# ayutaz/F5-TTS

Hardware: AMD Instinct MI355X
Metric: mel-frames/s (RTF alongside), F5TTS_v1_Base NFE=16 CFM.sample (higher is better)
Workload: dtype bf16; 1 GPU; C2: F5TTS_v1_Base CFM.sample, NFE 16 EPSS + sway -1, CFG 2.0, 1 utterance per GPU, 938 prompt + 938 generated frames (1876), 300 tokens; batch_per_gpu=1, frames=1876, gen_frames_per_gpu=938, nfe=16, parallelism=dp1

## Files before the change

### f5-tts_amd/csrc/elementwise.hip

```cpp
#include "common.h"
#include "kernels.h"
#include "lnrow.h"

#include <algorithm>

namespace f5h {

static inline unsigned nblk(int64_t n, int t) { return (unsigned)((n + t - 1) / t); }

struct TVals {
  float t[513];
};
__global__ void time_sinus_kernel(TVals tv, int n, float* out) {
  int i = blockIdx.x * blockDim.x + threadIdx.x;
  if (i >= n * 128) return;
  int r = i / 128, j = i % 128;
  const float k = logf(10000.f) / 127.f;
  float f = expf((float)j * -k);
  float e = (1000.f * tv.t[r]) * f;
  out[r * 256 + j] = sinf(e);
  out[r * 256 + 128 + j] = cosf(e);
}
hipError_t time_sinus(const float* t_host, int n, float* out, hipStream_t st) {
  if (n <= 0 || n > 512) return hipErrorInvalidValue;
  TVals tv{};
  for (int i = 0; i < n; ++i) tv.t[i] = t_host[i];
  hipLaunchKernelGGL(time_sinus_kernel, dim3(nblk(n * 128, 256)), dim3(256), 0, st, tv, n, out);
  return hipGetLastError();
}

__global__ void time_sinus_dev_kernel(const float* tg, int n, float* out) {
  int i = blockIdx.x * blockDim.x + threadIdx.x;
  if (i >= n * 128) return;
  int r = i / 128, j = i % 128;
  const float k = logf(10000.f) / 127.f;
  float f = expf((float)j * -k);
  float e = (1000.f * tg[r]) * f;
  out[r * 256 + j] = sinf(e);
  out[r * 256 + 128 + j] = cosf(e);
}
hipError_t time_sinus_dev(const float* tg, int n, float* out, hipStream_t st) {
  if (n <= 0 || n > 512) return hipErrorInvalidValue;
  hipLaunchKernelGGL(time_sinus_dev_kernel, dim3(nblk(n * 128, 256)), dim3(256), 0, st, tg, n, out);
  return hipGetLastError();
}

__global__ void grid_upload_kernel(TVals tv, int n, float* out) {
  int i = blockIdx.x * blockDim.x + threadIdx.x;
  if (i < n) out[i] = tv.t[i];
}
__global__ void ptr_upload_kernel(float* p, float** slot) {
  if (threadIdx.x == 0) slot[0] = p;
}
hipError_t ptr_upload(float* p, float** slot, hipStream_t st) {
  hipLaunchKernelGGL(ptr_upload_kernel, dim3(1), dim3(64), 0, st, p, slot);
  return hipGetLastError();
}
hipError_t grid_upload(const float* t_host, int n, float* out, hipStream_t st) {
  if (n <= 0 || n > 513) return hipErrorInvalidValue;
  TVals tv{};
  for (int i = 0; i < n; ++i) tv.t[i] = t_host[i];
  hipLaunchKernelGGL(grid_upload_kernel, dim3(nblk(n, 256)), dim3(256), 0, st, tv, n, out);
  return hipGetLastError();
}
struct IVals {
  int32_t v[512];
};
__global__ void seg_upload_kernel(IVals iv, int n, int32_t* out) {
  const int i = blockIdx.x * blockDim.x + threadIdx.x;
  if (i < n) out[i] = iv.v[i];
}
hipError_t seg_upload(const int32_t* host, int64_t n, int32_t* out, hipStream_t st) {
  if (n <= 0 || !host || !out) return hipErrorInvalidValue;
  for (int64_t o = 0; o < n; o += 512) {
    const int m = (int)(n - o < 512 ? n - o : 512);
    IVals iv{};
    for (int i = 0; i < m; ++i) iv.v[i] = host[o + i];
    hipLaunchKernelGGL(seg_upload_kernel, dim3(nblk(m, 256)), dim3(256), 0, st, iv, m, out + o);
  }
  return hipGetLastError();
}

__global__ void step_begin_kernel(const int* kstep, const float* src, int64_t stride, int n, float* dst) {
  const int k = *kstep;
  const int i = blockIdx.x * blockDim.x + threadIdx.x;
// ... 53 lines not shown
    const float xv[8] = {p0.x, p0.y, p0.z, p0.w, p1.x, p1.y, p1.z, p1.w};
#pragma unroll
    for (int e = 0; e < 8; ++e) {
      const float x = one + xv[e];
      hi[e] = from_f32<T>(x);
      lo[e] = from_f32<T>(x - to_f32(hi[e]));
    }
  };
  for (int k0 = 0; k0 < d; k0 += 64) {
    float4 xs[2][2], xh[2][2];
    v8 b[2][4];
#pragma unroll
    for (int u = 0; u < 2; ++u) {
      const int k = k0 + 32 * u;
      xs[u][0] = *reinterpret_cast<const float4*>(ar + sc_off + k);
      xs[u][1] = *reinterpret_cast<const float4*>(ar + sc_off + k + 4);
      xh[u][0] = *reinterpret_cast<const float4*>(ar + sh_off + k);
      xh[u][1] = *reinterpret_cast<const float4*>(ar + sh_off + k + 4);
#pragma unroll
      for (int t = 0; t < 4; ++t) b[u][t] = *reinterpret_cast<const v8*>(wr + (int64_t)t * 16 * d + k);
    }
#pragma unroll
    for (int u = 0; u < 2; ++u) {
      v8 shi, slo, hhi, hlo;
      parts(xs[u][0], xs[u][1], 1.f, shi, slo);
      parts(xh[u][0], xh[u][1], 0.f, hhi, hlo);
#pragma unroll
      for (int t = 0; t < 4; ++t) {
        acc[0][t] = Op16<T>::mma16(shi, b[u][t], acc[0][t]);
        acc[1][t] = Op16<T>::mma16(hhi, b[u][t], acc[1][t]);
        acc[0][t] = Op16<T>::mma16(slo, b[u][t], acc[0][t]);
        acc[1][t] = Op16<T>::mma16(hlo, b[u][t], acc[1][t]);
      }
    }
  }
  const int64_t LW = 2 * (int64_t)F + 6 * (int64_t)d;
  const int64_t u_off = a.out_off + l * LW + (ff ? 0 : 2 * (int64_t)F), v_off = u_off + (ff ? F : 3 * d);
#pragma unroll
  for (int t = 0; t < 4; ++t)
#pragma unroll
    for (int r = 0; r < 4; ++r) {
      const int s = g * 16 + 4 * (lane >> 4) + r;
      if (s < a.nfe) {
        float* o = a.table + (int64_t)s * a.stride + n0 + 16 * t + (lane & 15);
        o[u_off] = acc[0][t][r];
        o[v_off] = acc[1][t][r];
      }
    }
}
hipError_t lnfold_uv(int compute, const LnFoldArgs& a, hipStream_t st) {
  if (a.d % 64 || a.F % 64 || a.nfe <= 0 || a.depth <= 0) return hipErrorInvalidValue;
  const dim3 grid((a.depth * (a.F / 64 + 3 * a.d / 64) * ((a.nfe + 15) / 16) + 3) / 4), block(256);
  if (compute == F5H_C_BF16)
    hipLaunchKernelGGL(lnfold_uv_kernel<bf16>, grid, block, 0, st, a);
  else if (compute == F5H_C_FP16)
    hipLaunchKernelGGL(lnfold_uv_kernel<f16>, grid, block, 0, st, a);
  else
    return hipErrorInvalidValue;
  return hipGetLastError();
}

__global__ void zero_words_kernel(uint4* p, int64_t n4) {
  for (int64_t i = (int64_t)blockIdx.x * blockDim.x + threadIdx.x; i < n4; i += (int64_t)gridDim.x * blockDim.x)
    p[i] = uint4{0u, 0u, 0u, 0u};
}
hipError_t zero_words(unsigned* p, int64_t n, hipStream_t st) {
  if (n % 4 || ((uintptr_t)p & 15)) return hipErrorInvalidValue;
  const int64_t n4 = n / 4;
  hipLaunchKernelGGL(zero_words_kernel, dim3((unsigned)std::min<int64_t>(64, nblk(n4, 256))), dim3(256), 0, st,
                     reinterpret_cast<uint4*>(p), n4);
  return hipGetLastError();
}

template <typename TO>
__global__ void silu_kernel(const float* x, TO* y, int64_t n) {
  int64_t i = (int64_t)blockIdx.x * blockDim.x + threadIdx.x;
  if (i < n) y[i] = from_f32<TO>(silu(x[i]));
}
hipError_t silu_to_op(int compute, const float* x, void* y, int64_t n, hipStream_t st) {
  F5H_OP_DISPATCH(compute, T, hipLaunchKernelGGL(silu_kernel<T>, dim3(nblk(n, 256)), dim3(256), 0, st, x, (T*)y, n););
  return hipGetLastError();
}

constexpr int MAXV = 8;

template <typename TO, int NV, typename TI = float>
__global__ __launch_bounds__(256) void ln_mod_kernel(const TI* h, int M, int d, const float* shift,
                                                     const float* scale, TO* out) {
  constexpr bool FIXED = NV > 0;
  constexpr int V = FIXED ? NV : MAXV;
  const int row = blockIdx.x * 4 + (threadIdx.x >> 6), lane = threadIdx.x & 63;
  if (row >= M) return;
  const TI* x = h + (int64_t)row * d;
  const float4* sh = reinterpret_cast<const float4*>(shift);
  const float4* sc = reinterpret_cast<const float4*>(scale);
  const int n4 = FIXED ? 64 * NV : d >> 2;
  float4 v[V], a[V], b[V];
#pragma unroll
  for (int k = 0; k < V; ++k) {
    const int i = lane + 64 * k;
    const bool ok = FIXED || i < n4;
    v[k] = ok ? load4f<TI>(x + 4 * i) : make_float4(0, 0, 0, 0);
    a[k] = ok ? sc[i] : make_float4(0, 0, 0, 0);
    b[k] = ok ? sh[i] : make_float4(0, 0, 0, 0);
  }
  ln_mod_row<TO, V, FIXED>(v, a, b, lane, n4, d, out + (int64_t)row * d);
}
template <typename T>
__global__ __launch_bounds__(256) void ln_mod16_kernel(const T* h, int M, const float* shift, const float* scale,
                                                       T* out) {
  constexpr int d = 1024;
  const int row = blockIdx.x * 4 + (threadIdx.x >> 6), lane = threadIdx.x & 63;
  if (row >= M) return;
  const uint4* x = reinterpret_cast<const uint4*>(h + (int64_t)row * d);
  const float4* sh = reinterpret_cast<const float4*>(shift);
  const float4* sc = reinterpret_cast<const float4*>(scale);
  uint4 xv[2], o[2];
  float4 a[2][2], b[2][2];
#pragma unroll
  for (int k = 0; k < 2; ++k) {
    const int c = lane + 64 * k;
    xv[k] = x[c];
    a[k][0] = sc[2 * c];
    a[k][1] = sc[2 * c + 1];
    b[k][0] = sh[2 * c];
    b[k][1] = sh[2 * c + 1];
  }
  ln16_row<T>(xv, a, b, o);
  uint4* op = reinterpret_cast<uint4*>(out + (int64_t)row * d);
#pragma unroll
  for (int k = 0; k < 2; ++k) op[lane + 64 * k] = o[k];
}

hipError_t ln_modulate(int compute, const void* hv, int h16, int M, int d, const float* shift, const float* scale,
                       void* out, hipStream_t st) {
  if (d % 4 || d > 4 * 64 * MAXV) return hipErrorInvalidValue;
  const dim3 g(nblk(M, 4)), b(256);
  if (h16) {
    if (compute != F5H_C_BF16 && compute != F5H_C_FP16) return hipErrorInvalidValue;
    auto run = [&](auto tag) {
      typedef decltype(tag) T;
      const T* x = (const T*)hv;
      switch (d) {
        case 1024: hipLaunchKernelGGL((ln_mod16_kernel<T>), g, b, 0, st, x, M, shift, scale, (T*)out); break;
        case 768: hipLaunchKernelGGL((ln_mod_kernel<T, 3, T>), g, b, 0, st, x, M, d, shift, scale, (T*)out); break;
        case 512: hipLaunchKernelGGL((ln_mod_kernel<T, 2, T>), g, b, 0, st, x, M, d, shift, scale, (T*)out); break;
        default: hipLaunchKernelGGL((ln_mod_kernel<T, 0, T>), g, b, 0, st, x, M, d, shift, scale, (T*)out);
      }
    };
    if (compute == F5H_C_BF16)
      run(bf16{});
    else
      run(f16{});
    return hipGetLastError();
  }
  const float* h = (const float*)hv;
  switch (d) {
    case 1024: F5H_OP_DISPATCH(compute, T, hipLaunchKernelGGL((ln_mod_kernel<T, 4>), g, b, 0, st, h, M, d, shift, scale, (T*)out);); break;
    case 768: F5H_OP_DISPATCH(compute, T, hipLaunchKernelGGL((ln_mod_kernel<T, 3>), g, b, 0, st, h, M, d, shift, scale, (T*)out);); break;
    case 512: F5H_OP_DISPATCH(compute, T, hipLaunchKernelGGL((ln_mod_kernel<T, 2>), g, b, 0, st, h, M, d, shift, scale, (T*)out);); break;
    default: F5H_OP_DISPATCH(compute, T, hipLaunchKernelGGL((ln_mod_kernel<T, 0>), g, b, 0, st, h, M, d, shift, scale, (T*)out););
  }
  return hipGetLastError();
}

template <typename TO, int NV, typename TI = float>
__global__ __launch_bounds__(256) void rms_kernel(const TI* h, int M, int d, const float* g, TO* out) {
  constexpr bool FIXED = NV > 0;
  constexpr int V = FIXED ? NV : MAXV;
  const int row = blockIdx.x * 4 + (threadIdx.x >> 6), lane = threadIdx.x & 63;
  if (row >= M) return;
  const TI* x = h + (int64_t)row * d;
  const float4* gg = reinterpret_cast<const float4*>(g);
  const int n4 = FIXED ? 64 * NV : d >> 2;
  float4 v[V], a[V];
  float q = 0.f;
#pragma unroll
  for (int k = 0; k < V; ++k) {
    const int i = lane + 64 * k;
    const bool ok = FIXED || i < n4;
    v[k] = ok ? load4f<TI>(x + 4 * i) : make_float4(0, 0, 0, 0);
    a[k] = ok ? gg[i] : make_float4(0, 0, 0, 0);
  }
#pragma unroll
  for (int k = 0; k < V; ++k) q += v[k].x * v[k].x + v[k].y * v[k].y + v[k].z * v[k].z + v[k].w * v[k].w;
  const float nrm = fmaxf(sqrtf(wave_sum_dpp(q)), 1e-12f);
  const float f = sqrtf((float)d);
#pragma unroll
  for (int k = 0; k < V; ++k) {
// ... 340 lines not shown
  }
  partial[((int64_t)z * S + s) * C + c] = acc;
}
template <typename TO>
__global__ void grn_apply_ragged_kernel(const float* x, const int* off, int S, int C, const float* nx,
                                        const float* gamma, const float* beta, TO* out, int64_t total) {
  int64_t i = (int64_t)blockIdx.x * blockDim.x + threadIdx.x;
  if (i >= total) return;
  int c = (int)(i % C);
  int s = seg_find(off, S, (int)(i / C));
  float v = x[i];
  out[i] = from_f32<TO>(gamma[c] * (v * nx[(int64_t)s * C + c]) + beta[c] + v);
}
hipError_t grn_ragged(int compute, const float* x, const int32_t* off, int S, int R, int Lmax, int C,
                      const float* gamma, const float* beta, float* scratch, void* out, hipStream_t st) {
  if (S <= 0 || R <= 0 || Lmax <= 0 || C <= 0 || !off) return hipErrorInvalidValue;
  const int nz = (int)nblk(Lmax, 64);
  float* nx = scratch + (size_t)nz * S * C;
  hipLaunchKernelGGL(grn_sumsq_ragged_kernel, dim3(nblk(C, 256), S, nz), dim3(256), 0, st, x, off, S, C, scratch);
  hipLaunchKernelGGL(grn_norm_kernel, dim3(S), dim3(1024), 0, st, scratch, nz, S, C, nx);
  const int64_t total = (int64_t)R * C;
  F5H_OP_DISPATCH(compute, T, hipLaunchKernelGGL(grn_apply_ragged_kernel<T>, dim3(nblk(total, 256)), dim3(256), 0, st, x, off, S, C, nx, gamma, beta, (T*)out, total););
  return hipGetLastError();
}
__global__ void rowtab_kernel(const int* off, int S, int R, int2* rowtab, int32_t* len) {
  const int m = blockIdx.x * blockDim.x + threadIdx.x;
  if (m < S && len) len[m] = off[m + 1] - off[m];
  if (m >= R) return;
  const int s = seg_find(off, S, m);
  rowtab[m] = make_int2(s, m - off[s]);
}
hipError_t build_rowtab(const int32_t* off, int S, int R, int2* rowtab, int32_t* len, hipStream_t st) {
  if (S <= 0 || R < S || !off || !rowtab) return hipErrorInvalidValue;
  hipLaunchKernelGGL(rowtab_kernel, dim3(nblk(R, 256)), dim3(256), 0, st, off, S, R, rowtab, len);
  return hipGetLastError();
}

template <typename TO>
__global__ void build_ct_kernel(const float* cond, const uint8_t* cmask, const float* tc, const float* tu, int B,
                                int N, int td, int tdp, int S, int drop_audio, int drop_text, TO* out) {
  const int64_t K = 128 + tdp;
  int64_t i = (int64_t)blockIdx.x * blockDim.x + threadIdx.x;
  if (i >= (int64_t)S * N * K) return;
  const int64_t row = i / K;
  const int col = (int)(i - row * K);
  const int s = (int)(row / N), n = (int)(row - (int64_t)s * N);
  const int b = s % B;
  float v = 0.f;
  if (col < 128) {
    if (col < 100 && s < B && !drop_audio && cmask[(int64_t)b * N + n]) v = cond[((int64_t)b * N + n) * 100 + col];
  } else if (col - 128 < td) {
    const float* t = (s < B && !drop_text) ? tc : tu;
    v = t[((int64_t)b * N + n) * td + (col - 128)];
  }
  out[i] = from_f32<TO>(v);
}
hipError_t build_ct(int compute, const float* cond, const uint8_t* cond_mask, const float* text_c,
                    const float* text_u, int B, int N, int td, int S, int drop_audio, int drop_text, void* out,
                    hipStream_t st) {
  const int tdp = (td + 63) / 64 * 64;
  const int64_t total = (int64_t)S * N * (128 + tdp);
  F5H_OP_DISPATCH(compute, T, hipLaunchKernelGGL(build_ct_kernel<T>, dim3(nblk(total, 256)), dim3(256), 0, st, cond, cond_mask, text_c, text_u, B, N, td, tdp, S, drop_audio, drop_text, (T*)out););
  return hipGetLastError();
}

template <typename TO>
__global__ void pack_y_kernel(const float* y, int rows, int mel, TO* yp) {
  int64_t i = (int64_t)blockIdx.x * blockDim.x + threadIdx.x;
  if (i >= (int64_t)rows * 128) return;
  int64_t r = i >> 7;
  int c = (int)(i & 127);
  yp[i] = from_f32<TO>(c < mel ? y[r * mel + c] : 0.f);
}
hipError_t pack_y(int compute, const float* y, int rows, int mel, void* ypad, hipStream_t st) {
  const int64_t total = (int64_t)rows * 128;
  F5H_OP_DISPATCH(compute, T, hipLaunchKernelGGL(pack_y_kernel<T>, dim3(nblk(total, 256)), dim3(256), 0, st, y, rows, mel, (T*)ypad););
  return hipGetLastError();
}

template <typename TO>
__global__ __launch_bounds__(256) void cfg_euler_kernel(EulerArgs a, TO* ypad) {
  int64_t i = (int64_t)blockIdx.x * blockDim.x + threadIdx.x;
  const int64_t total = (int64_t)a.B * a.N * a.mel;
  const int k = a.kstep ? __hip_atomic_load(a.kstep, __ATOMIC_RELAXED, __HIP_MEMORY_SCOPE_AGENT) : 0;
  if (a.kstep && a.next_dst) {
    if (k + 1 < a.nfe) {
      const float4* src = reinterpret_cast<const float4*>(a.next_src + (int64_t)(k + 1) * a.next_stride);
      float4* dst = reinterpret_cast<float4*>(a.next_dst);
      for (int64_t j = i; j < a.next_n / 4; j += (int64_t)gridDim.x * blockDim.x) dst[j] = src[j];
    }
  }
  float dt = a.dt;
  float* traj = a.traj;
  if (a.kstep) {
    dt = sub_nc(a.tgrid[k + 1], a.tgrid[k]);
    traj = a.trajp ? *a.trajp : nullptr;
    if (traj) traj += (int64_t)(k + 1) * total;
  }
  for (; i < total; i += (int64_t)gridDim.x * blockDim.x) {
    const int c = (int)(i % a.mel);
    const int64_t bn = i / a.mel;
    const int b = (int)(bn / a.N), n = (int)(bn - (int64_t)b * a.N);
    const float pc = a.p[(int64_t)b * a.p_seq_stride + (int64_t)(a.p_row_off + n) * a.p_ld + c];
    float v = pc;
    if (a.use_cfg) {
      const float pu = a.p[(int64_t)(a.B + b) * a.p_seq_stride + (int64_t)(a.p_row_off + n) * a.p_ld + c];
      v = add_nc(pc, mul_nc(sub_nc(pc, pu), a.cfg));
    }
    const float y = add_nc(a.y[i], mul_nc(dt, v));
    a.y[i] = y;
    if (ypad) ypad[bn * 128 + c] = from_f32<TO>(y);
    if (traj) traj[i] = y;
  }
  if (a.kstep && a.arrive) {
    __syncthreads();
    if (threadIdx.x == 0) {
      const unsigned old = __hip_atomic_fetch_add(a.arrive, 1u, __ATOMIC_RELAXED, __HIP_MEMORY_SCOPE_AGENT);
      if (old == gridDim.x - 1) {
        __hip_atomic_store(a.arrive, 0u, __ATOMIC_RELAXED, __HIP_MEMORY_SCOPE_AGENT);
        __hip_atomic_store(const_cast<int*>(a.kstep), k + 1, __ATOMIC_RELAXED, __HIP_MEMORY_SCOPE_AGENT);
        if (a.tick) __hip_atomic_fetch_add(a.tick, 1, __ATOMIC_RELAXED, __HIP_MEMORY_SCOPE_AGENT);
      }
    }
  }
}
hipError_t cfg_euler(const EulerArgs& a, hipStream_t st) {
  const int64_t total = (int64_t)a.B * a.N * a.mel;
  const unsigned blocks = std::min<unsigned>(128, std::max<unsigned>(1, nblk(total, 256)));
  F5H_OP_DISPATCH(a.compute, T, hipLaunchKernelGGL(cfg_euler_kernel<T>, dim3(blocks), dim3(256), 0, st, a, (T*)a.ypad););
  return hipGetLastError();
}

template <typename TO, int METHOD>
__global__ __launch_bounds__(256) void cfg_rk_kernel(RkArgs a, TO* ypad) {
  constexpr OdeTableau T = ode_tableau(METHOD);
  constexpr int STAGES = T.stages;
  static_assert(METHOD == 1 || METHOD == 2, "midpoint or rk4");
  static_assert(METHOD != 1 || (T.a[4] == T.c[1] && T.b[0] == 0.f && T.b[1] == 1.f), "midpoint tableau");
  static_assert(METHOD != 2 || (T.a[4] == T.c[1] && T.a[8] == -T.c[1] && T.a[9] == 1.f && T.a[12] == 1.f &&
                                T.a[13] == -1.f && T.a[14] == 1.f && T.b[1] == 3.f * T.b[0] &&
                                T.b[2] == T.b[1] && T.b[3] == T.b[0]),
                "3/8-rule tableau");
  int64_t i = (int64_t)blockIdx.x * blockDim.x + threadIdx.x;
  const int64_t total = (int64_t)a.B * a.N * a.mel;
  const int e = __hip_atomic_load(a.keval, __ATOMIC_RELAXED, __HIP_MEMORY_SCOPE_AGENT);
  const int k = e / STAGES, s = e - k * STAGES;
  if (a.next_dst && e + 1 < a.neval) {
    const float4* src = reinterpret_cast<const float4*>(a.next_src + (int64_t)(e + 1) * a.next_stride);
    float4* dst = reinterpret_cast<float4*>(a.next_dst);
    for (int64_t j = i; j < a.next_n / 4; j += (int64_t)gridDim.x * blockDim.x) dst[j] = src[j];
  }
  const float dt = sub_nc(a.sgrid[k + 1], a.sgrid[k]);
  const bool last = s == STAGES - 1;
  float* traj = (last && a.trajp) ? *a.trajp : nullptr;
  if (traj) traj += (int64_t)(k + 1) * total;
  for (; i < total; i += (int64_t)gridDim.x * blockDim.x) {
    const int c = (int)(i % a.mel);
    const int64_t bn = i / a.mel;
    const int b = (int)(bn / a.N), n = (int)(bn - (int64_t)b * a.N);
    const float pc = a.p[(int64_t)b * a.p_seq_stride + (int64_t)(a.p_row_off + n) * a.p_ld + c];
    float v = pc;
    if (a.use_cfg) {
      const float pu = a.p[(int64_t)(a.B + b) * a.p_seq_stride + (int64_t)(a.p_row_off + n) * a.p_ld + c];
      v = add_nc(pc, mul_nc(sub_nc(pc, pu), a.cfg));
    }
    const float y0 = a.y[i];
    float yn;
    if constexpr (METHOD == 1) {
      yn = s == 0 ? add_nc(y0, mul_nc(v, mul_nc(T.c[1], dt))) : add_nc(y0, mul_nc(dt, v));
    } else {
      constexpr float c3 = T.c[1];
      const float* K0 = a.kbuf;
      const float* K1 = K0 + total;
      const float* K2 = K1 + total;
      if (s == 0) {
        yn = add_nc(y0, mul_nc(mul_nc(dt, v), c3));
      } else if (s == 1) {
        yn = add_nc(y0, mul_nc(dt, sub_nc(v, mul_nc(K0[i], c3))));
      } else if (s == 2) {
        yn = add_nc(y0, mul_nc(dt, add_nc(sub_nc(K0[i], K1[i]), v)));
      } else {
        const float sum = add_nc(add_nc(K0[i], mul_nc(T.b[1] / T.b[0], add_nc(K1[i], K2[i]))), v);
        yn = add_nc(y0, mul_nc(mul_nc(sum, dt), T.b[0]));
      }
      if (!last) a.kbuf[(int64_t)s * total + i] = v;
    }
    if (last) a.y[i] = yn;
    ypad[bn * 128 + c] = from_f32<TO>(yn);
    if (traj) traj[i] = yn;
  }
  if (a.arrive) {
    __syncthreads();
    if (threadIdx.x == 0) {
      const unsigned old = __hip_atomic_fetch_add(a.arrive, 1u, __ATOMIC_RELAXED, __HIP_MEMORY_SCOPE_AGENT);
      if (old == gridDim.x - 1) {
        __hip_atomic_store(a.arrive, 0u, __ATOMIC_RELAXED, __HIP_MEMORY_SCOPE_AGENT);
        __hip_atomic_store(a.keval, e + 1, __ATOMIC_RELAXED, __HIP_MEMORY_SCOPE_AGENT);
        if (a.tick) __hip_atomic_fetch_add(a.tick, 1, __ATOMIC_RELAXED, __HIP_MEMORY_SCOPE_AGENT);
      }
    }
  }
}
hipError_t cfg_rk(const RkArgs& a, hipStream_t st) {
  if ((a.method != 1 && a.method != 2) || !a.keval || !a.sgrid || !a.ypad) return hipErrorInvalidValue;
  if (ode_kept_slopes(a.method) > 0 && !a.kbuf) return hipErrorInvalidValue;
  const int64_t total = (int64_t)a.B * a.N * a.mel;
  const unsigned blocks = std::min<unsigned>(128, std::max<unsigned>(1, nblk(total, 256)));
// ... 176 lines not shown
```

### f5-tts_amd/csrc/engine.cpp

```cpp
#include "engine_internal.h"

static bool adaln_bb(const f5h_arch& a) { return a.backbone != F5H_UNETT; }
static size_t mm_ada_x(const f5h_arch& a, int l) { return (size_t)l * 12 * a.dim; }
static size_t mm_ada_c(const f5h_arch& a, int l) { return mm_ada_x(a, l) + (size_t)6 * a.dim; }
static size_t mm_ada_fin(const f5h_arch& a) { return mm_ada_c(a, a.depth - 1) + (size_t)2 * a.dim; }

static void layout(const f5h_engine* e, WS& ws, Bufs& b, int B, int N, int nfe, int use_cfg, int method = 0,
                   int steps = 0, int nt = 0, int rgB = 0, int rgL = 0) {
  const f5h_arch& a = e->a;
  const int d = a.dim, td = a.text_dim, S = use_cfg ? 2 * B : B;
  const bool mm = a.backbone == F5H_MMDIT;
  const int L = adaln_bb(a) ? N : N + 1;
  const size_t rows = (size_t)S * L, es = e->esz;
  const size_t jrows = mm ? (size_t)S * (N + nt) : rows;
  const int inner = a.heads * 64;
  b.tsin = ws.take<float>((size_t)nfe * 256);
  b.th = ws.take<float>((size_t)nfe * d);
  b.temb = ws.take<float>((size_t)nfe * d);
  b.tin_op = ws.take<char>((size_t)nfe * std::max(256, d) * es);
  b.ada = adaln_bb(a) ? ws.take<float>((size_t)nfe * e->ada_row) : nullptr;
  b.te = ws.take<float>((size_t)2 * B * (mm ? nt : N) * td);
  b.keepfill = ws.take<uint8_t>((size_t)2 * B * N);
  if (a.conv_layers > 0) {
    b.dwln = ws.take<char>((size_t)2 * B * N * td * es);
// ... 169 lines not shown
    TextEmbArgs t{};
    t.text = text;
    t.B = c.B;
    t.nt = c.nt;
    t.N = c.nt;
    t.td = d;
    t.table = e->text_table;
    t.freqs = e->freqs;
    t.freq_rows = kMMTextPos;
    t.mask_padding = a.text_mask_padding;
    t.out_c = b.te;
    t.out_u = b.te + (size_t)c.B * c.nt * d;
    KCK(text_embed(t, st));
    if (bf) KCK(f32_to_op(bf, b.te, (int64_t)2 * c.B * c.nt * d, b.c0, st));
  } else if (!text_cached) {
    TextEmbArgs t{};
    t.text = text;
    t.B = c.rag_B ? c.rag_B : c.B;
    t.nt = c.nt;
    t.N = c.N;
    t.td = td;
    t.seg_off = b.rg_off;
    t.seq_len = (a.backbone == F5H_DIT && c.batch_mask) ? duration : nullptr;
    t.table = e->text_table;
    t.freqs = a.conv_layers > 0 ? e->freqs : nullptr;
    t.mask_padding = a.text_mask_padding;
    t.out_c = b.te;
    t.out_u = b.te + (size_t)c.B * c.N * td;
    t.keep = b.keepfill;
    KCK(text_embed(t, st));
    const int S2 = 2 * c.B, R2 = S2 * c.N;
    const int32_t* tl = c.isolate ? duration : nullptr;
    for (int i = 0; i < a.conv_layers; ++i) {
      CNX& x = e->cnx[i];
      if (c.rag_B)
        KCK(dwconv_ln_ragged(bf, b.te, b.rg_off, 2 * c.rag_B, R2, td, x.dw_w, x.dw_b, x.ln_w, x.ln_b, b.dwln, st));
      else
        KCK(dwconv_ln(bf, b.te, S2, c.N, td, x.dw_w, x.dw_b, x.ln_w, x.ln_b, b.dwln, st, tl, c.B));
      GemmArgs g = gargs(b.dwln, td, x.pw1, R2, b.pw1o, 2 * td);
      KCK(gemm(bf, EPI_GELU_ERF, g, st));
      if (c.rag_B)
        KCK(grn_ragged(bf, b.pw1o, b.rg_off, 2 * c.rag_B, R2, c.rag_L, 2 * td, x.gamma, x.beta, b.grn_scr, b.grno, st));
      else
        KCK(grn(bf, b.pw1o, S2, c.N, 2 * td, x.gamma, x.beta, b.grn_scr, b.grno, st, tl, c.B));
      g = gargs(b.grno, 2 * td, x.pw2, R2, b.te, td);
      g.rowkeep = a.text_mask_padding ? b.keepfill : nullptr;
      KCK(gemm(bf, EPI_RESID_FILL, g, st));
    }
    if (a.text_average_upsampling) {
      TextUpArgs u{};
      u.text = text;
      u.B = c.B;
      u.nt = c.nt;
      u.N = c.N;
      u.td = td;
      u.seq_len = t.seq_len;
      u.in_c = t.out_c;
      u.in_u = t.out_u;
      u.out_c = b.te_up;
      u.out_u = b.te_up + (size_t)c.B * c.N * td;
      KCK(text_upsample(u, st));
    }
  }
  if (c.isolate && b.rowkeep_n) KCK(build_rowkeep(duration, c.B, c.S, c.N, 0, b.rowkeep_n, st));
  const float* te = a.text_average_upsampling ? b.te_up : b.te;
  KCK(build_ct(bf, cond, cond_mask, te, te + (size_t)c.B * c.N * td, c.B, c.N, mm ? 0 : td, c.S, c.drop_audio,
               c.drop_text, b.act, st));
  GemmArgs g = gargs(b.act, 128 + e->tdp, e->in_ct, c.S * c.N, b.P, d);
  KCK(gemm(bf, EPI_STORE, g, st));
  return 0;
}

constexpr int kArrive = 16;

static int step_prep(Ctx& c) {
  f5h_engine* e = c.e;
  if (adaln_bb(e->a))
    KCK(step_begin(c.b.kstep, c.b.ada, e->ada_row, e->ada_row, c.b.ada_cur, c.st));
  else
    KCK(step_begin(c.b.kstep, c.b.temb, e->a.dim, e->a.dim, c.b.temb_cur, c.st));
  return 0;
}

static int backbone_part(Ctx& c, int s0, int ns, hipStream_t st) {
  f5h_engine* e = c.e;
  const f5h_arch& a = e->a;
  const int d = a.dim, bf = e->bf, H = a.heads, inner = H * 64;
  const bool dit = a.backbone == F5H_DIT;
  const size_t es = e->esz;
  Bufs& b = c.b;
  const int BN = c.B * c.N;
  const int rows = ns * c.L;
  const size_t ro = (size_t)s0 * c.L;
  const size_t no = (size_t)s0 * c.N;
  auto op = [&](void* base, size_t row, size_t width) -> void* { return (char*)base + row * width * es; };
  const uint8_t* keep = c.batch_mask ? b.rowkeep + ro : nullptr;
  static const bool res32 = [] {
    const char* v = getenv("F5H_RES32");
    return v && *v == '1';
  }();
  const bool r16 = bf != 0 && (!dit || !res32);
  static const bool skip_ln = [] {
    const char* v = getenv("F5H_DIAG_SKIP_LN");
    const bool on = v && *v == '1';
    if (on) std::fprintf(stderr, "[f5h] F5H_DIAG_SKIP_LN=1: LayerNorm launches skipped, results are WRONG (timing only)\n");
    return on;
  }();
  const bool do_ln = !(skip_ln && r16);
  const size_t hsz = r16 ? es : sizeof(float);
  auto res = [&](void* base) -> void* { return (char*)base + ro * d * hsz; };
  void* bh = dit ? res(b.h) : res(b.xs[0]);
  void* aop = op(b.aop, ro, d);
  void* q = op(b.q, ro, inner);
  void* k = op(b.k, ro, inner);
  void* v = op(b.v, ro, inner);
  void* o = op(b.o, ro, inner);
  void* f = op(b.f, ro, a.ff_dim);
  {
    GemmArgs g = gargs(b.ypad, 128, e->in_x, BN, b.h0 + no * d, d);
    g.bias = nullptr;
    g.add = b.P + no * d;
    g.ld_add = d;
    g.dual_rows = ns == 2 * c.B ? BN : 0;
    KCK(gemm(bf, EPI_INPROJ, g, st));
    ConvArgs cv{};
    cv.S = ns;
    cv.L = c.N;
    cv.d = d;
    cv.rowkeep = dit ? keep : (c.isolate ? b.rowkeep_n + no : nullptr);
    cv.x = b.h0 + no * d;
    cv.x_f32 = 1;
    cv.w = e->conv_w[0];
    cv.bias = e->conv_b[0];
    cv.mode = 0;
    cv.y = op(b.c1, no, d);
    if (c.rag_B) {
      cv.ragged = 1;
      cv.S = ns * c.rag_B;
      cv.L = c.rag_L;
      cv.rowkeep = reinterpret_cast<const uint8_t*>(b.rg_off);
    }
    {
      ProbeScope ps(e, KC_CONV, st, &c.site);
      KCK(conv_pos(bf, cv, st));
    }
    cv.x = op(b.c1, no, d);
    cv.x_f32 = bf ? 0 : 1;
    cv.w = e->conv_w[1];
    cv.bias = e->conv_b[1];
    cv.mode = r16 ? 2 : 1;
    cv.y = bh;
    cv.y_seq_stride = c.L;
    cv.y_row_off = dit ? 0 : 1;
    cv.resid = b.h0 + no * d;
    KCK(conv_pos(bf, cv, st));
  }
  if (!dit) KCK(write_time_token(bf, r16, b.temb_cur, ns, c.L, d, bh, st));
  void* hkeep = a.long_skip_connection ? (char*)b.hkeep + ro * d * hsz : nullptr;
  if (hkeep) {
    if (bf != 0 && !r16)
      return fail(F5H_EINVAL, "long_skip_connection: F5H_RES32 (fp32 residual under 16-bit operands) is not supported");
    KCK(hipMemcpyAsync(hkeep, bh, (size_t)rows * d * hsz, hipMemcpyDeviceToDevice, st));
  }

  const float* ada_k = dit ? b.ada_cur : nullptr;
  const int epi_resid = r16 ? EPI_RESID16 : EPI_RESID;
  void* h = bh;
  const void* h_in = nullptr;
  auto qkv_args = [&](const Layer& Lq) {
    GemmArgs g = gargs(aop, d, Lq.qkv, rows, nullptr, 0);
    g.rope = b.rope;
    g.seq_len = c.L;
    g.heads = H;
    g.rope_heads = a.pe_attn_head > 0 ? a.pe_attn_head : H;
    g.q = q;
    g.k = k;
    g.v = v;
    g.q_scale = 0.125f * 1.4426950408889634f;
    g.q_norm_w = Lq.q_norm_w;
    g.k_norm_w = Lq.k_norm_w;
    g.qk_norm_eps = 1e-6f;
    if (c.rag_B) {
      g.add = reinterpret_cast<const float*>(b.rg_tab);
      g.seq_len = c.rag_L;
      g.qkv_dst_len = c.rag_L;
    }
    return g;
  };
  const bool chain_on = c.chain && dit && r16 && do_ln && !keep && d == 1024 && b.chain && s0 == 0 && ns == c.S &&
                        (e->probe_class < 0 || e->probe_class == KC_ATTN || e->probe_class == KC_CONV ||
                         e->probe_class == KC_CHAIN);
  static const bool zero_memset = [] {
    const char* v = getenv("F5H_CHAIN_ZERO");
    return v && !strcmp(v, "memset");
  }();
  if (chain_on) {
    if (zero_memset)
      KCK(hipMemsetAsync(b.chain, 0, (size_t)a.depth * 5 * b.chain_g4 * sizeof(unsigned), st));
    else
      KCK(zero_words(b.chain, (int64_t)a.depth * 5 * b.chain_g4, st));
  }
  bool qkv_done = false;
  bool final_done = false;
  const bool fold_on = c.lnfold && dit && r16 && do_ln && !keep && !chain_on && b.lnp && e->lnf_ok;
  const bool rms_on = c.lnfold && !dit && r16 && b.lnp && e->rmsf_ok;
  const int64_t lnf_lw = 2 * (int64_t)a.ff_dim + 6 * (int64_t)d;
  auto lnf = [&](int l) { return ada_k + e->ada.Npad + (int64_t)l * lnf_lw; };
// ... 76 lines not shown
        at.kv_len = at.q_len = b.rg_len;
        at.o_split = kAttnRagged;
        at.o2 = b.rg_off;
      }
      at.store_wt = attention_store_wt(bf, at, store_want(c.store, KC_ATTN));
      count_store(e, at.store_wt);
      ProbeScope ps(e, KC_ATTN, st, &c.site, &at.probe);
      KCK(attention(bf, at, st));
    }
    if (chain_on) {
      ChainArgs ca{};
      ca.out = gargs(o, inner, Ly.out, rows, h, d);
      ca.out.gate = ad + 2 * d;
      ca.ln1 = LnArgs{h, aop, ad + 3 * d , ad + 4 * d };
      ca.ff1 = gargs(aop, d, Ly.ff1, rows, f, a.ff_dim);
      ca.ff2 = gargs(f, a.ff_dim, Ly.ff2, rows, h, d);
      ca.ff2.gate = ad + 5 * d;
      if (l + 1 < a.depth) {
        const float* an = ada_k + (size_t)(l + 1) * 6 * d;
        ca.ln2 = LnArgs{h, aop, an , an + d };
        ca.qkv = qkv_args(e->layers[l + 1]);
      } else {
        const float* fin = ada_k + (size_t)a.depth * 6 * d;
        ca.ln2 = LnArgs{h, aop, fin + d, fin};
      }
      ca.cnt = b.chain + (size_t)l * 5 * b.chain_g4;
      ca.groups = (rows + kChainRows - 1) / kChainRows;
      ca.fault = e->chain_fault;
      ProbeScope ps(e, KC_CHAIN, st, &c.site, &ca.probe);
      const hipError_t ce = chain_launch(bf, ca, st);
      if (ce == hipSuccess) {
        e->n_chain.fetch_add(1, std::memory_order_relaxed);
        qkv_done = l + 1 < a.depth;
        final_done = l + 1 == a.depth;
        continue;
      }
      if (ce != hipErrorInvalidValue) KCK(ce);
    }
    {
      GemmArgs g = gargs(o, inner, Ly.out, rows, h, d);
      g.resid = h_in;
      g.gate = ad ? ad + 2 * d : nullptr;
      g.rowkeep = keep;
      if (keep && !h_in && e->pad_skip && !rms_on) {
        g.live_len = b.kvlen + s0;
        g.live_seq = c.L;
      }
      if (fold_on) fold_producer(g, ad + 4 * d );
      if (rms_on) rms_producer(g);
      gemm_policy(c, g, epi_resid, KC_OUT);
      ProbeScope ps(e, KC_OUT, st, &c.site, &g.probe);
      KCK(gemm(bf, epi_resid, g, st));
    }
    if (!fold_on && !rms_on) {
      ProbeScope ps(e, KC_NORM, st, &c.site);
      if (dit) {
        if (do_ln) KCK(ln_modulate(bf, h, r16, rows, d, ad + 3 * d , ad + 4 * d , aop, st));
      }
      else
        KCK(rms_norm_g(bf, h, r16, rows, d, Ly.g_ff, aop, st));
    }
    {
      GemmArgs g = gargs(aop, d, Ly.ff1, rows, f, a.ff_dim);
      if (fold_on) fold_consumer(g, lnf(l), lnf(l) + a.ff_dim);
      if (rms_on) {
        g.A = h;
        g.W = Ly.ff1_g.w;
        rms_consumer(g);
      }
      gemm_policy(c, g, EPI_GELU_TANH, KC_FFN1);
      ProbeScope ps(e, KC_FFN1, st, &c.site, &g.probe);
      KCK(gemm(bf, EPI_GELU_TANH, g, st));
    }
    {
      GemmArgs g = gargs(f, a.ff_dim, Ly.ff2, rows, h, d);
      g.gate = ad ? ad + 5 * d : nullptr;
      if (fold_on && l + 1 < a.depth) fold_producer(g, ada_k + (size_t)(l + 1) * 6 * d + d);
      if (rms_on && l + 1 < a.depth / 2) rms_producer(g);
      gemm_policy(c, g, epi_resid, KC_FFN2);
      ProbeScope ps(e, KC_FFN2, st, &c.site, &g.probe);
      KCK(gemm(bf, epi_resid, g, st));
    }
  }
  if (dit) {
    const float* fin = ada_k + (size_t)a.depth * 6 * d;
    if (hkeep) {
      void* hl = (char*)b.c1 + no * d * hsz;
      GemmArgs g = gargs(h, d, e->long_skip, rows, hl, d);
      g.A2 = hkeep;
      g.k_split = d;
      KCK(gemm(bf, r16 ? EPI_STORE16 : EPI_STORE, g, st));
      h = hl;
    }
    if (!final_done) KCK(ln_modulate(bf, h, r16, rows, d, fin + d, fin, aop, st));
  } else {
    KCK(rms_norm_g(bf, h, r16, rows, d, e->norm_out_g, aop, st));
  }
  const int pld = e->proj_out.Npad;
  GemmArgs g = gargs(aop, d, e->proj_out, rows, b.p + ro * pld, pld);
  g.N = pld;
  KCK(gemm(bf, EPI_STORE, g, st));
  return 0;
}

static int backbone_mmdit(Ctx& c, hipStream_t st) {
  f5h_engine* e = c.e;
  const f5h_arch& a = e->a;
  const int d = a.dim, bf = e->bf, H = a.heads, inner = H * 64, F = a.ff_dim;
  const size_t es = e->esz;
  Bufs& b = c.b;
  const int BN = c.B * c.N, rows = c.S * c.N, crows = c.S * c.nt, Lj = c.N + c.nt;
  const bool r16 = bf != 0;
  const int epi_resid = r16 ? EPI_RESID16 : EPI_RESID;
  const uint8_t* keep = c.batch_mask ? b.rowkeep : nullptr;
  {
    GemmArgs g = gargs(b.ypad, 128, e->in_x, BN, b.h0, d);
    g.bias = nullptr;
    g.add = b.P;
    g.ld_add = d;
    g.dual_rows = c.S == 2 * c.B ? BN : 0;
    KCK(gemm(bf, EPI_INPROJ, g, st));
    ConvArgs cv{};
    cv.S = c.S;
    cv.L = c.N;
    cv.d = d;
    cv.x = b.h0;
    cv.x_f32 = 1;
    cv.w = e->conv_w[0];
    cv.bias = e->conv_b[0];
    cv.mode = 0;
    cv.y = b.c1;
    cv.rowkeep = c.isolate ? keep : nullptr;
    {
      ProbeScope ps(e, KC_CONV, st, &c.site);
      KCK(conv_pos(bf, cv, st));
    }
    cv.x = b.c1;
    cv.x_f32 = bf ? 0 : 1;
    cv.w = e->conv_w[1];
    cv.bias = e->conv_b[1];
    cv.mode = r16 ? 2 : 1;
    cv.y = b.h;
    cv.y_seq_stride = c.N;
    cv.y_row_off = 0;
    cv.resid = b.h0;
    KCK(conv_pos(bf, cv, st));
  }
  const char* te0 = r16 ? (const char*)b.c0 : (const char*)b.te;
  const size_t hsz = r16 ? es : sizeof(float);
  const void* c0 = te0 + ((c.S == c.B && c.drop_text) ? (size_t)c.B * c.nt * d * hsz : 0);
  const float* ada_k = b.ada_cur;
  auto qkv = [&](const void* A, const Lin& W, int M, int seq, size_t row0, const float* qn, const float* kn) -> int {
    GemmArgs g = gargs(A, d, W, M, nullptr, 0);
    g.rope = b.rope;
    g.seq_len = seq;
    g.qkv_dst_len = Lj;
    g.heads = H;
    g.rope_heads = H;
    g.q = (char*)b.q + row0 * 64 * es;
    g.k = (char*)b.k + row0 * 64 * es;
    g.v = (char*)b.v + row0 * 64 * es;
    g.q_scale = 0.125f * 1.4426950408889634f;
    g.q_norm_w = qn;
    g.k_norm_w = kn;
    g.qk_norm_eps = 1e-6f;
    gemm_policy(c, g, EPI_QKV, KC_QKV);
// ... 84 lines not shown
  KCK(hipEventRecord(e->ev_fork, c.st));
  KCK(hipStreamWaitEvent(c.st2, e->ev_fork, 0));
  RC(backbone_part(c, 0, c.B, c.st));
  RC(backbone_part(c, c.B, c.B, c.st2));
  KCK(hipEventRecord(e->ev_join, c.st2));
  KCK(hipStreamWaitEvent(c.st, e->ev_join, 0));
  return 0;
}

static float round_to(int compute, float x) {
  if (compute == F5H_FP16) return (float)(_Float16)x;
  if (compute != F5H_BF16 || x != x) return x;
  uint32_t u;
  std::memcpy(&u, &x, 4);
  u = (u + 0x7fffu + ((u >> 16) & 1u)) & 0xffff0000u;
  std::memcpy(&x, &u, 4);
  return x;
}
void ode_eval_times(int method, int compute, const float* t, int steps, float* out) {
#pragma clang fp contract(off)
  const OdeTableau T = ode_tableau(method);
  for (int i = 0; i <= steps; ++i)
    if (round_to(compute, t[i]) != t[i]) compute = F5H_FP32;
  for (int k = 0; k < steps; ++k) {
    const float t0 = t[k], t1 = t[k + 1];
    const float dt = round_to(compute, t1 - t0);
    for (int s = 0; s < T.stages; ++s) {
      float v = t0;
      if (s > 0) v = T.c[s] == 1.f ? t1 : round_to(compute, t0 + round_to(compute, dt * T.c[s]));
      out[k * T.stages + s] = v;
    }
  }
}

extern "C" {

size_t f5h_workspace_size_ode(const f5h_engine* e, int32_t B, int32_t N, int32_t nt, int32_t steps, int32_t use_cfg,
                             int32_t method) {
  if (!e || B <= 0 || N <= 0 || steps <= 0 || method < 0 || method >= kOdeMethods) return 0;
  if (e->a.backbone == F5H_MMDIT && nt < 0) return 0;
  WS ws;
  Bufs b;
  layout(e, ws, b, B, N, steps * ode_tableau(method).stages + 1, use_cfg, method, steps,
         e->a.backbone == F5H_MMDIT ? nt : 0);
  return ws.off;
}
size_t f5h_workspace_size(const f5h_engine* e, int32_t B, int32_t N, int32_t nt, int32_t nfe, int32_t use_cfg) {
  return f5h_workspace_size_ode(e, B, N, nt, nfe, use_cfg, F5H_EULER);
}

static int check_ws(Ctx& c, void* w, size_t bytes) {
  WS ws;
  layout(c.e, ws, c.b, c.B, c.N, c.nfe + 1, c.use_cfg, c.method, c.steps, c.nt, c.rag_B, c.rag_L);
  if (bytes < ws.off)
    return fail(F5H_ENOMEM, "workspace too small: need " + std::to_string(ws.off) + " have " + std::to_string(bytes));
  ws.off = 0;
  ws.base = reinterpret_cast<char*>(w);
  layout(c.e, ws, c.b, c.B, c.N, c.nfe + 1, c.use_cfg, c.method, c.steps, c.nt, c.rag_B, c.rag_L);
  return 0;
}
static int check_mmdit_call(const f5h_engine* e, int nt, int batch_mask, int isolate) {
  if (e->a.backbone != F5H_MMDIT) return 0;
  if (nt <= 0) return fail(F5H_EINVAL, "MMDiT needs nt >= 1 text tokens");
  if (e->a.attn_mask_enabled && batch_mask && !isolate)
    return fail(F5H_EINVAL,
                "MMDiT: attn_mask_enabled with a batch mask is not supported: the valid keys [0, dur) and [N, N + "
                "text length) are not a prefix of the joint sequence, and the reference's masked mode is not wired to "
                "the two-range attention (use_batch_mask 2 masks both ranges and isolates the batch)");
  return 0;
}

static GraphKey graph_key(const Ctx& c, const void* ws, int kind) {
  GraphKey key{};
  key.ws = ws;
  key.kind = kind;
  key.B = c.B;
  key.N = c.N;
  key.nt = c.nt;
  key.nfe = c.nfe;
  key.use_cfg = c.use_cfg;
  key.batch_mask = c.batch_mask + c.isolate;
  key.lnfold = c.lnfold;
  key.store = c.store;
  key.method = c.method;
  key.rag_B = c.rag_B;
  key.rag_L = c.rag_L;
  key.kernel_epoch = g_kernel_epoch.load();
  return key;
}

static int prologue_graph(Ctx& c, const f5h_sample_args* a, const GraphKey& key) {
  f5h_engine* e = c.e;
  const size_t bn = (size_t)c.B * c.N;
  HIPCK(hipMemcpyAsync(c.b.in_cond, a->cond, bn * e->a.mel_dim * sizeof(float), hipMemcpyDeviceToDevice, c.st));
  HIPCK(hipMemcpyAsync(c.b.in_mask, a->cond_mask, bn, hipMemcpyDeviceToDevice, c.st));
  if (c.nt > 0)
    HIPCK(hipMemcpyAsync(c.b.in_text, a->text, (size_t)c.B * c.nt * sizeof(int64_t), hipMemcpyDeviceToDevice, c.st));
  HIPCK(hipMemcpyAsync(c.b.in_dur, a->duration, (size_t)c.B * sizeof(int32_t), hipMemcpyDeviceToDevice, c.st));
  const Bufs& b = c.b;
  std::shared_ptr<GraphEntry> hold;
  RC(graph_get(c, key, false,
               [&](Ctx& cc) { return prologue(cc, nullptr, cc.nfe, b.in_cond, b.in_mask, b.in_text, b.in_dur); },
               hold, 1));
  HIPCK(hipGraphLaunch(hold->exec, c.st));
  return note_replays(e, hold.get(), c.st);
}

static int enqueue_step(Ctx& c, const f5h_sample_args* a) {
  f5h_engine* e = c.e;
  c.site = 0;
  RC(backbone_step(c));
  const bool dit = adaln_bb(e->a);
  auto common = [&](auto& u) {
    u.y = c.b.y;
    u.B = c.B;
    u.N = c.N;
    u.mel = e->a.mel_dim;
    u.p = c.b.p;
    u.p_seq_stride = (int64_t)c.L * e->proj_out.Npad;
    u.p_row_off = dit ? 0 : 1;
    u.p_ld = e->proj_out.Npad;
    u.use_cfg = c.use_cfg;
    u.cfg = a->cfg_strength;
    u.ypad = c.b.ypad;
    u.compute = e->bf;
    u.trajp = c.b.trajp;
    u.next_src = dit ? c.b.ada : c.b.temb;
    u.next_stride = dit ? e->ada_row : e->a.dim;
    u.next_n = dit ? (int)e->ada_row : e->a.dim;
    u.next_dst = dit ? c.b.ada_cur : c.b.temb_cur;
    u.arrive = reinterpret_cast<unsigned*>(c.b.kstep + kArrive);
    u.tick = e->ptick;
  };
  if (c.method != F5H_EULER) {
    RkArgs r{};
    common(r);
    r.method = c.method;
    r.kbuf = c.b.kbuf;
    r.keval = c.b.kstep;
    r.sgrid = c.b.sgrid;
    r.neval = c.nfe;
    KCK(cfg_rk(r, c.st));
    return 0;
  }
  EulerArgs u{};
  common(u);
  u.dt = 0.f;
  u.kstep = c.b.kstep;
  u.tgrid = c.b.tgrid;
  u.traj = nullptr;
  u.nfe = c.nfe;
  KCK(cfg_euler(u, c.st));
  return 0;
}

static int run_steps(Ctx& c, const f5h_sample_args* a, const void* ws) {
  f5h_engine* e = c.e;
  if (!e->graph_mode) {
    for (int k = 0; k < c.nfe; ++k) RC(enqueue_step(c, a));
    return 0;
  }
  GraphKey key = graph_key(c, ws, 0);
  if (e->a.backbone != F5H_MMDIT) key.nt = 0;
  key.probe = e->probe_class;
  const bool split = e->split_cfg == 1 && !c.rag_B;
  key.split = split;
  key.pad_skip = e->pad_skip;
  key.chain = c.chain;
  std::memcpy(&key.cfg_bits, &a->cfg_strength, 4);
  std::shared_ptr<GraphEntry> hold;
  RC(graph_get(c, key, split, [&](Ctx& cc) { return enqueue_step(cc, a); }, hold, c.nfe));
  int rc = 0, k = 0;
  for (; k < c.nfe; ++k) {
    const hipError_t le = hipGraphLaunch(hold->exec, c.st);
    if (le != hipSuccess) {
      rc = fail(F5H_EHIP, std::string("hipGraphLaunch: ") + hipGetErrorString(le));
      break;
    }
  }
  if (k > 0) {
    const int r2 = note_replays(e, hold.get(), c.st);
    if (!rc) rc = r2;
  }
  return rc;
}

struct RagCall {
  int B, Lmax;
  const int32_t* dur;
};
struct CallShape {
  int B, N, nt;
  int nfe;
  int use_cfg, use_batch_mask;
  int method, steps;
};
static int call_begin(f5h_engine* e, hipStream_t st, const CallShape& sh, void* ws, size_t bytes, const RagCall* rg,
                      Ctx& c, ChainTicket& ticket) {
  c.e = e;
  c.st = st;
  c.B = sh.B;
  c.N = sh.N;
  c.nt = sh.nt;
  c.method = sh.method;
  c.steps = sh.steps;
  c.nfe = sh.nfe;
  c.use_cfg = sh.use_cfg;
  c.S = c.use_cfg ? 2 * c.B : c.B;
  c.L = adaln_bb(e->a) ? c.N : c.N + 1;
  if (sh.use_batch_mask < 0 || sh.use_batch_mask > 2) return fail(F5H_EINVAL, "use_batch_mask must be 0, 1 or 2");
  c.batch_mask = sh.use_batch_mask ? 1 : 0;
  c.isolate = sh.use_batch_mask == 2 ? 1 : 0;
  c.rag_B = rg ? rg->B : 0;
  c.rag_L = rg ? rg->Lmax : 0;
  RC(check_mmdit_call(e, c.nt, c.batch_mask, c.isolate));
  RC(check_ws(c, ws, bytes));
  RC(chain_fault_check(e, c.st));
  c.chain = rg ? 0 : chain_for_call(e, c, ticket);
  c.lnfold = !rg && e->lnfold && !c.chain && ((e->lnf_ok && !c.batch_mask) || e->rmsf_ok);
  c.store = e->store_policy;
  return 0;
}
static int sample_impl(f5h_engine* e, void* stream, const f5h_sample_args* a, int method, void* workspace,
                       size_t workspace_bytes, const RagCall* rg = nullptr) {
  if (!e || !a) return fail(F5H_EINVAL, "null engine/args");
  if (a->B <= 0 || a->N <= 0 || a->nt < 0 || a->nfe <= 0 || a->nfe > 512)
    return fail(F5H_EINVAL, "bad B/N/nt/nfe");
  const int stages = ode_tableau(method).stages;
  if (a->nfe * stages > 512)
    return fail(F5H_EINVAL, std::to_string(a->nfe) + " steps x " + std::to_string(stages) + " stages = " +
                                std::to_string(a->nfe * stages) +
                                " backbone evaluations exceed the 512 rows of the per-call time tables");
  if (!a->cond || !a->cond_mask || (!a->duration && !rg) || !a->y0 || !a->t_grid || !a->out || (a->nt > 0 && !a->text))
    return fail(F5H_EINVAL, "null tensor argument");
  if (e->a.backbone == F5H_DIT && (rg ? rg->Lmax : a->N) > 8192)
    return fail(F5H_EINVAL, "N exceeds the text position table (8192)");
  HIPCK(hipSetDevice(e->dev));
  UseNote used{e->uses, reinterpret_cast<hipStream_t>(stream)};
  ChainTicket ticket;
  Ctx c{};
  const CallShape sh{a->B, a->N, a->nt, a->nfe * stages, a->cfg_strength >= 1e-5f, a->use_batch_mask, method, a->nfe};
  RC(call_begin(e, reinterpret_cast<hipStream_t>(stream), sh, workspace, workspace_bytes, rg, c, ticket));
  if (rg) {
    std::vector<int32_t> off((size_t)2 * rg->B + 1);
    off[0] = 0;
    for (int s = 0; s < 2 * rg->B; ++s) off[s + 1] = off[s] + rg->dur[s % rg->B];
    HIPCK(seg_upload(off.data(), (int64_t)off.size(), c.b.rg_off, c.st));
  }
  double hp[kHostPhases] = {};
  c.hp = hp;
  const double h0 = host_ms();
  static const bool pro_graph = [] {
    const char* v = getenv("F5H_PROLOGUE_GRAPH");
    return !(v && *v == '0');
  }();
  std::vector<float> evt;
  const float* t_rows = a->t_grid;
  if (method == F5H_EULER) {
    HIPCK(grid_upload(a->t_grid, c.nfe + 1, c.b.tgrid, c.st));
  } else {
    evt.resize(c.nfe);
    ode_eval_times(method, e->bf, a->t_grid, c.steps, evt.data());
    t_rows = evt.data();
    HIPCK(grid_upload(t_rows, c.nfe, c.b.tgrid, c.st));
    HIPCK(grid_upload(a->t_grid, c.steps + 1, c.b.sgrid, c.st));
  }
  const GraphKey pkey = graph_key(c, workspace, 1);
  if (pro_graph && e->graph_mode && !rg && c.nt <= c.N && prologue_repeats(e, pkey))
    RC(prologue_graph(c, a, pkey));
  else
    RC(prologue(c, t_rows, c.nfe, a->cond, a->cond_mask, a->text, a->duration));
  const double h1 = host_ms();
  const size_t ysz = (size_t)c.B * c.N * e->a.mel_dim;
  HIPCK(hipMemcpyAsync(c.b.y, a->y0, ysz * sizeof(float), hipMemcpyDeviceToDevice, c.st));
  if (a->trajectory)
    HIPCK(hipMemcpyAsync(a->trajectory, a->y0, ysz * sizeof(float), hipMemcpyDeviceToDevice, c.st));
  HIPCK(pack_y(e->bf, c.b.y, c.B * c.N, e->a.mel_dim, c.b.ypad, c.st));
  HIPCK(ptr_upload(a->trajectory, c.b.trajp, c.st));
  HIPCK(hipMemsetAsync(c.b.kstep, 0, 64 * sizeof(int), c.st));
  RC(step_prep(c));
  const double h2 = host_ms();
  const double g2 = hp[HP_LOCK] + hp[HP_REAP] + hp[HP_CAPTURE] + hp[HP_INSTANTIATE];
  RC(run_steps(c, a, workspace));
  const double h3 = host_ms();
  HIPCK(final_where_out(a->cond, a->cond_mask, c.b.y, a->out, c.B, c.N, e->a.mel_dim,
                        c.chain ? e->chain_fault : nullptr, c.st));
  if (c.chain) RC(chain_fault_note(e, c.st));
  const double h4 = host_ms();
  hp[HP_TOTAL] = h4 - h0;
  hp[HP_PROLOGUE] = h1 - h0;
  hp[HP_LAUNCH] = (h3 - h2) - (hp[HP_LOCK] + hp[HP_REAP] + hp[HP_CAPTURE] + hp[HP_INSTANTIATE] - g2);
  hp[HP_FINAL] = h4 - h3;
  {
    std::lock_guard<std::mutex> g(e->hm);
    std::memcpy(e->last_host, hp, sizeof(hp));
  }
  return 0;
}

int f5h_sample(f5h_engine* e, void* stream, const f5h_sample_args* a, void* workspace, size_t workspace_bytes) {
  return sample_impl(e, stream, a, F5H_EULER, workspace, workspace_bytes);
}
int f5h_sample_ode(f5h_engine* e, void* stream, const f5h_sample_args* a, int32_t method, void* workspace,
                   size_t workspace_bytes) {
  if (method < 0 || method >= kOdeMethods) return fail(F5H_EINVAL, "ode method must be 0 (euler), 1 (midpoint) or 2 (rk4)");
  return sample_impl(e, stream, a, method, workspace, workspace_bytes);
}

static int check_ragged_call(const f5h_engine* e, int B, int64_t R, int Lmax, const int32_t* dur) {
  if (!e) return fail(F5H_EINVAL, "null engine");
  if (e->a.backbone != F5H_DIT)
    return fail(F5H_EINVAL, "ragged sampling serves the DiT backbone only (UNetT's time-token row and MMDiT's joint "
                            "sequence are not packed)");
  if (e->a.text_average_upsampling)
    return fail(F5H_EINVAL, "ragged sampling does not serve text_embedding_average_upsampling");
  if (B <= 0 || R <= 0 || Lmax <= 0) return fail(F5H_EINVAL, "ragged sampling: bad B / R / Lmax");
  if (2 * R >= (int64_t)1 << 24) return fail(F5H_EINVAL, "ragged sampling: 2 R must stay below 2^24 rows");
  if (dur) {
    int64_t sum = 0;
    for (int b = 0; b < B; ++b) {
      if (dur[b] < 1) return fail(F5H_EINVAL, "ragged sampling: duration[" + std::to_string(b) + "] is below 1");
      if (dur[b] > Lmax)
        return fail(F5H_EINVAL, "ragged sampling: duration[" + std::to_string(b) + "] exceeds Lmax");
      sum += dur[b];
    }
    if (sum != R) return fail(F5H_EINVAL, "ragged sampling: the durations add up to " + std::to_string(sum) + ", not R");
  }
  return 0;
}
size_t f5h_workspace_size_ragged(const f5h_engine* e, int32_t B, int64_t R, int32_t Lmax, int32_t nt, int32_t steps,
                                 int32_t use_cfg, int32_t method) {
  (void)nt;
  if (!e || steps <= 0 || method < 0 || method >= kOdeMethods || R > INT32_MAX) return 0;
  if (check_ragged_call(e, B, R, Lmax, nullptr)) return 0;
  WS ws;
  Bufs b;
  layout(e, ws, b, 1, (int)R, steps * ode_tableau(method).stages + 1, use_cfg, method, steps, 0, B, Lmax);
  return ws.off;
}
int f5h_sample_ragged(f5h_engine* e, void* stream, const f5h_ragged_args* r, int32_t method, void* workspace,
                      size_t workspace_bytes) {
  if (!e || !r) return fail(F5H_EINVAL, "null engine/args");
  if (method < 0 || method >= kOdeMethods) return fail(F5H_EINVAL, "ode method must be 0 (euler), 1 (midpoint) or 2 (rk4)");
  if (!r->duration) return fail(F5H_EINVAL, "null tensor argument");
  if (r->R > INT32_MAX) return fail(F5H_EINVAL, "ragged sampling: R too large");
  RC(check_ragged_call(e, r->B, r->R, r->Lmax, r->duration));
  f5h_sample_args a{};
  a.B = 1;
  a.N = (int32_t)r->R;
  a.nt = r->nt;
  a.nfe = r->nfe;
  a.cond = r->cond;
  a.cond_mask = r->cond_mask;
  a.text = r->text;
  a.duration = nullptr;
  a.y0 = r->y0;
  a.t_grid = r->t_grid;
  a.cfg_strength = r->cfg_strength;
  a.use_batch_mask = 0;
  a.out = r->out;
  a.trajectory = r->trajectory;
  const RagCall rg{r->B, r->Lmax, r->duration};
  return sample_impl(e, stream, &a, method, workspace, workspace_bytes, &rg);
// ... 57 lines not shown
```

### f5-tts_amd/csrc/engine_ctl.cpp

```cpp
#include "engine_internal.h"
#include "capi_util.h"

thread_local std::string g_err;
int fail(int code, const std::string& msg) {
  g_err = msg;
  return code;
}
int f5h_internal_fail(int code, const std::string& msg) { return fail(code, msg); }

extern "C" {

const char* f5h_last_error(void) { return g_err.c_str(); }
const char* f5h_version(void) { return "f5h 0.1 gfx950"; }

int f5h_probe_enable(f5h_engine* e, int32_t kclass, int32_t enable) {
  if (!e) return fail(F5H_EINVAL, "null engine");
  std::lock_guard<std::mutex> g(e->pm);
  e->probe_class = enable ? kclass : -1;
  if (e->pstamp) {
    HIPCK(hipSetDevice(e->dev));
    HIPCK(hipDeviceSynchronize());
    HIPCK(hipMemset(e->pstamp, 0, 64 * sizeof(unsigned long long)));
    HIPCK(hipMemset(e->pslots, 0xff, (size_t)kProbeEnd * sizeof(unsigned long long)));
    HIPCK(hipMemset(e->pslots + kProbeEnd, 0, (size_t)kProbeEnd * sizeof(unsigned long long)));
// ... 5 lines not shown

int f5h_probe_timeline(f5h_engine* e, uint64_t* stamps, int32_t max_wg, int32_t* n_wg, double* tick_khz) {
  if (!e || !stamps || max_wg <= 0) return fail(F5H_EINVAL, "null engine / buffer");
  std::lock_guard<std::mutex> g(e->pm);
  HIPCK(hipSetDevice(e->dev));
  HIPCK(hipDeviceSynchronize());
  const int n = std::min<int>(max_wg, kTimelineWG);
  HIPCK(hipMemcpy(stamps, e->ptl, (size_t)n * 4 * sizeof(unsigned long long), hipMemcpyDeviceToHost));
  int last = 0;
  for (int i = 0; i < n; ++i)
    if (stamps[4 * i]) last = i + 1;
  if (n_wg) *n_wg = last;
  if (tick_khz) *tick_khz = e->wall_khz;
  return 0;
}

int f5h_probe_read(f5h_engine* e, int64_t* launches, double* total_ms) {
  if (!e) return fail(F5H_EINVAL, "null engine");
  std::lock_guard<std::mutex> g(e->pm);
  double ms = 0.0;
  int64_t n = 0;
  if (e->pstamp && e->wall_khz > 0.0) {
    HIPCK(hipSetDevice(e->dev));
    HIPCK(hipDeviceSynchronize());
    std::vector<unsigned long long> h(2 * (size_t)kProbeEnd);
    HIPCK(hipMemcpy(h.data(), e->pslots, h.size() * sizeof(unsigned long long), hipMemcpyDeviceToHost));
    unsigned long long ticks = 0;
    for (int64_t i = 0; i < kProbeEnd; i += (int64_t)kProbeLanes * kProbeStride) {
      unsigned long long t0 = ~0ull, t1 = 0;
      for (int l = 0; l < kProbeLanes; ++l) {
        t0 = std::min(t0, h[i + l * kProbeStride]);
        t1 = std::max(t1, h[kProbeEnd + i + l * kProbeStride]);
      }
      if (t1 == 0 || t0 == ~0ull || t1 < t0) continue;
      ticks += t1 - t0;
      ++n;
    }
    ms = (double)ticks / e->wall_khz;
  }
  if (launches) *launches = n;
  if (total_ms) *total_ms = ms;
  return 0;
}

int f5h_set_graph_mode(f5h_engine* e, int32_t mode) {
  if (!e) return fail(F5H_EINVAL, "null engine");
  if (mode != 0 && mode != 1) return fail(F5H_EINVAL, "graph mode must be 0 (eager) or 1 (step graph)");
  std::lock_guard<std::mutex> g(e->gm);
  e->graph_mode = mode;
  return 0;
}

int f5h_set_cfg_streams(f5h_engine* e, int32_t n) {
  if (!e) return fail(F5H_EINVAL, "null engine");
  if (n < 0 || n > 2) return fail(F5H_EINVAL, "cfg streams must be 0 (auto), 1 or 2");
  std::lock_guard<std::mutex> g(e->gm);
  e->split_cfg = n == 0 ? 2 : (n == 2 ? 1 : 0);
  return 0;
}

int f5h_set_pad_skip(f5h_engine* e, int32_t enable) {
  if (!e) return fail(F5H_EINVAL, "null engine");
  if (enable != 0 && enable != 1) return fail(F5H_EINVAL, "pad skip must be 0 or 1");
  std::lock_guard<std::mutex> g(e->gm);
  e->pad_skip = enable;
  return 0;
}

int f5h_set_ln_fold(f5h_engine* e, int32_t enable) {
  if (!e) return fail(F5H_EINVAL, "null engine");
  if (enable != 0 && enable != 1) return fail(F5H_EINVAL, "ln fold must be 0 or 1");
  std::lock_guard<std::mutex> g(e->gm);
  e->lnfold = enable;
  return 0;
}

int f5h_ln_fold_stats(f5h_engine* e, int32_t* supported, int64_t* passes) {
  if (!e) return fail(F5H_EINVAL, "null engine");
  if (supported) *supported = (e->lnf_ok || e->rmsf_ok) ? 1 : 0;
  if (passes) *passes = e->n_lnfold.load(std::memory_order_relaxed);
  return 0;
}

int f5h_set_store_policy(f5h_engine* e, int32_t mode) {
  if (!e) return fail(F5H_EINVAL, "null engine");
  if (mode != -1 && mode != 0 && mode != 1 && (mode < 0x100 || mode > 0x11F))
    return fail(F5H_EINVAL, "store policy must be -1 (auto), 0 (plain), 1 (write-through) or 0x100 | class mask");
  std::lock_guard<std::mutex> g(e->gm);
  e->store_policy = mode;
  return 0;
}

int f5h_store_policy_stats(f5h_engine* e, int64_t* write_through, int64_t* plain) {
  if (!e) return fail(F5H_EINVAL, "null engine");
  if (write_through) *write_through = e->n_store_wt.load(std::memory_order_relaxed);
  if (plain) *plain = e->n_store_plain.load(std::memory_order_relaxed);
  return 0;
}

int f5h_store_policy_force(int32_t mode) {
  if (mode < -1 || mode > 1) return fail(F5H_EINVAL, "forced store policy must be -1 (off), 0 (plain) or 1 (write-through)");
  store_policy_force(mode);
  g_kernel_epoch.fetch_add(1);
  return 0;
}

int f5h_last_call_host_ms(f5h_engine* e, double* ms, int32_t n) {
  if (!e || !ms || n <= 0) return fail(F5H_EINVAL, "null engine / buffer");
  std::lock_guard<std::mutex> g(e->hm);
  for (int i = 0; i < n; ++i) ms[i] = i < kHostPhases ? e->last_host[i] : 0.0;
  return 0;
}

int f5h_graph_stats(f5h_engine* e, int64_t* captures, int64_t* replays, int32_t* cached) {
  if (!e) return fail(F5H_EINVAL, "null engine");
  std::lock_guard<std::mutex> g(e->gm);
  if (captures) *captures = e->n_captures;
  if (replays) *replays = e->n_replays;
  if (cached) *cached = (int32_t)e->graphs.size();
  return 0;
}

int f5h_gemm_force_config(int32_t cfg) {
  if (cfg != -1 && cfg != 0 && cfg != 1 && cfg != 5 && cfg != 11 && cfg != 12 && cfg != 13)
    return fail(F5H_EINVAL, "gemm config must be -1, 0, 1, 5, 11, 12 or 13");
  gemm_force_config(cfg);
  g_kernel_epoch.fetch_add(1);
  return 0;
}

int f5h_attn_force_safe(int32_t on) {
  attention_force_safe(on);
  g_kernel_epoch.fetch_add(1);
  return 0;
}

}
```

### f5-tts_amd/csrc/engine_internal.h

```cpp
#pragma once
#include <hip/hip_runtime.h>

#include <cmath>
#include <cstring>
#include <algorithm>
#include <atomic>
#include <chrono>
#include <cstdio>
#include <memory>
#include <functional>
#include <mutex>
#include <string>
#include <type_traits>
#include <unordered_map>
#include <vector>

#include "../../include/f5h.h"
#include "kernels.h"
#include "reaper.h"

using namespace f5h;

#pragma GCC visibility push(hidden)

extern thread_local std::string g_err;
int fail(int code, const std::string& msg);
#define HIPCK(x)                                                                               \
  do {                                                                                         \
    hipError_t _e = (x);                                                                       \
    if (_e != hipSuccess) return fail(F5H_EHIP, std::string(#x) + ": " + hipGetErrorString(_e)); \
  } while (0)

#define RC(x)              \
  do {                     \
    int _r = (x);          \
    if (_r) return _r;     \
  } while (0)

#define KCK(x) HIPCK(x)

struct Lin {
  void* w = nullptr;
  float* b = nullptr;
  int N = 0, K = 0, Npad = 0;
};

struct CNX {
  float *dw_w = nullptr, *dw_b = nullptr, *ln_w = nullptr, *ln_b = nullptr, *gamma = nullptr, *beta = nullptr;
  Lin pw1, pw2;
};

struct Layer {
  Lin qkv, out, ff1, ff2, skip;
  float *g_attn = nullptr, *g_ff = nullptr;
  Lin qkv_g, ff1_g;
  float *q_norm_w = nullptr, *k_norm_w = nullptr;
  Lin qkv_c, out_c, ff1_c, ff2_c;
  float *cq_norm_w = nullptr, *ck_norm_w = nullptr;
};
constexpr int kMMTextPos = 1024;

struct GraphKey {
  const void* ws;
  uint64_t kernel_epoch;
  int32_t kind;
  int32_t B, N, nt, nfe, use_cfg, batch_mask, probe, split, pad_skip, chain, lnfold, store;
  int32_t method;
  int32_t drop_text;
  int32_t rag_B, rag_L;
  uint32_t cfg_bits;
};
static_assert(std::has_unique_object_representations_v<GraphKey>, "GraphKey is compared as bytes: no padding");
inline bool operator==(const GraphKey& a, const GraphKey& b) { return std::memcmp(&a, &b, sizeof(GraphKey)) == 0; }

struct f5h_engine {
  f5h_arch a{};
  int dev = 0;
  int bf = 0;
  size_t esz = 4;
  int tdp = 0;
  std::vector<void*> allocs;
  hipStream_t mstream = nullptr;
  Lin t1, t2, ada, in_x, in_ct, proj_out;
  Lin long_skip;
  float* text_table = nullptr;
  float* freqs = nullptr;
  std::vector<CNX> cnx;
  void* conv_w[2] = {nullptr, nullptr};
  float* conv_b[2] = {nullptr, nullptr};
  std::vector<Layer> layers;
  float* norm_out_g = nullptr;
  std::mutex gm;
  std::vector<std::shared_ptr<struct GraphEntry>> graphs;
  std::vector<std::shared_ptr<struct GraphEntry>> graveyard;
  std::vector<hipEvent_t> ev_pool;
  std::vector<struct GraphKey> pro_seen;
  int64_t n_evicted = 0, n_reaped = 0;
  std::mutex hm;
  double last_host[8] = {};
  hipStream_t cap = nullptr;
  hipStream_t cap2 = nullptr;
  hipEvent_t ev_fork = nullptr, ev_join = nullptr;
  int graph_mode = 1;
  int split_cfg = 2;
  int pad_skip = 1;
  int chain = 0;
  int lnfold = 1;
  bool lnf_ok = false, rmsf_ok = false;
  const void** lnf_w = nullptr;
  int64_t ada_row = 0;
  std::atomic<int64_t> n_lnfold{0};
  int store_policy = -1;
  std::atomic<int64_t> n_store_wt{0}, n_store_plain{0};
  unsigned* chain_fault = nullptr;
  volatile unsigned* fault_host = nullptr;
  int fault_slot = -1;
  std::atomic<int64_t> n_chain{0};
  uint64_t use_ctr = 0;
  int64_t n_captures = 0, n_replays = 0;
  std::mutex pm;
  int probe_class = -1;
  unsigned long long* pstamp = nullptr;
  unsigned long long* pslots = nullptr;
  unsigned long long* ptl = nullptr;
  int* ptick = nullptr;
  double wall_khz = 0.0;
  UseLog uses;
};

struct GraphEntry {
  GraphKey key{};
  hipGraphExec_t exec = nullptr;
  uint64_t stamp = 0;
  std::vector<hipEvent_t> inflight;
  ~GraphEntry() {
    if (exec) (void)hipGraphExecDestroy(exec);
    for (hipEvent_t ev : inflight) (void)hipEventDestroy(ev);
  }
};

struct WS {
  size_t off = 0;
  char* base = nullptr;
  template <typename T>
  T* take(size_t n) {
    size_t o = off;
    off = (off + n * sizeof(T) + 255) / 256 * 256;
    return base ? reinterpret_cast<T*>(base + o) : nullptr;
  }
};

struct Bufs {
  float *tsin, *th, *temb, *ada;
  void* tin_op;
  float *te, *pw1o, *grn_scr;
  void *dwln, *grno;
  uint8_t* keepfill;
  void* act;
  float* P;
  void* ypad;
  float *h0, *h, *p;
  void *c1, *aop, *q, *k, *v, *o, *f;
  float2* rope;
  uint8_t* rowkeep;
  int32_t* kvlen;
  float* lnp;
  unsigned* chain;
  int chain_g4;
  float *ada_cur, *temb_cur, *tgrid;
  int* kstep;
  float* y;
  float** trajp;
  float *sgrid, *kbuf;
  void* hkeep;
  float* te_up;
  void *c0, *ch, *caop, *co, *cf;
  uint8_t* ckeep;
  int32_t* tlen;
  uint8_t* rowkeep_n;
  std::vector<void*> xs;
  void* pp[2];
  float* in_cond;
  uint8_t* in_mask;
  int64_t* in_text;
  int32_t* in_dur;
  int32_t *rg_off, *rg_len;
  int2* rg_tab;
};

struct Ctx {
  f5h_engine* e;
  hipStream_t st;
  Bufs b;
  int B, N, nt, S, L, nfe, use_cfg, batch_mask;
  int isolate;
  int method, steps;
  int drop_audio, drop_text;
  hipStream_t st2;
  int site;
  int chain;
  int lnfold;
  int store;
  double* hp;
  int rag_B, rag_L;
};
enum { HP_TOTAL = 0, HP_PROLOGUE, HP_LOCK, HP_REAP, HP_CAPTURE, HP_INSTANTIATE, HP_LAUNCH, HP_FINAL, kHostPhases };
inline double host_ms() {
  return std::chrono::duration<double, std::milli>(std::chrono::steady_clock::now().time_since_epoch()).count();
}

constexpr size_t kConvPackElems = (size_t)16 * 31 * 64 * 64;
int pack_conv_weight(const void* src, int src_dt, int d, void* dst, int dst_dt, hipStream_t st);
extern std::atomic<uint64_t> g_kernel_epoch;
int graph_get(Ctx& c, const GraphKey& key, bool split, const std::function<int(Ctx&)>& body,
              std::shared_ptr<GraphEntry>& hold, int64_t replays);
int note_replays(f5h_engine* e, GraphEntry* g, hipStream_t st);
bool prologue_repeats(f5h_engine* e, const GraphKey& key);
int fault_slot_take(volatile unsigned** host);
void fault_slot_give(int i);
struct ChainTicket {
  int dev = 0;
  hipStream_t st = nullptr;
  bool held = false;
  ~ChainTicket();
};
int chain_for_call(f5h_engine* e, const Ctx& c, ChainTicket& t);
int chain_fault_check(f5h_engine* e, hipStream_t st);
int chain_fault_note(f5h_engine* e, hipStream_t st);
void ode_eval_times(int method, int compute, const float* t, int steps, float* out);

#pragma GCC visibility pop
```

### f5-tts_amd/csrc/engine_ops.cpp

```cpp
#include "engine_internal.h"

extern "C" {

static bool op_compute_ok(int32_t compute) { return compute >= F5H_FP32 && compute <= F5H_FP16; }
struct OpWs {
  WS ws;
  size_t bytes;
  size_t end = 0;
  OpWs(void* base, size_t n) : bytes(n) { ws.base = reinterpret_cast<char*>(base); }
  void* take(size_t n) {
    end = ws.off + n;
    return ws.take<char>(n);
  }
  bool fits() const { return ws.off == 0 || (ws.base && ws.off <= bytes); }
};
#define OPWS_CHECK(w, what)                                                                       \
  do {                                                                                            \
    if (!(w).fits()) return fail(F5H_ENOMEM, std::string("workspace too small for ") + (what));  \
  } while (0)

static int op_seg_check(const char* what, const int32_t* off, int S, int64_t R, int Lmax) {
  if (!off || S <= 0 || R <= 0 || Lmax <= 0) return fail(F5H_EINVAL, std::string(what) + ": bad segment table");
  if (off[0] != 0 || off[S] != R) return fail(F5H_EINVAL, std::string(what) + ": seg_off must run from 0 to R");
  for (int s = 0; s < S; ++s)
// ... 509 lines not shown
  g.N = N;
  g.K = K;
  g.bias = a->bias;
  g.C = a->C;
  g.ldc = N;
  g.gate = a->gate;
  g.rowkeep = a->rowkeep;
  g.resid = a->resid;
  g.live_len = a->live_len;
  g.live_seq = a->live_len ? a->live_seq : 0;
  g.add = a->add;
  g.ld_add = a->ld_add;
  g.dual_rows = dual;
  if (rq) {
    HIPCK(seg_upload(a->seg_off, a->n_seq + 1, rq_off, st));
    HIPCK(build_rowtab(rq_off, a->n_seq, M, rq_tab, nullptr, st));
    g.add = reinterpret_cast<const float*>(rq_tab);
  }
  if (cop) {
    if (inout) HIPCK(f32_to_op(compute, a->C, nC, cop, st));
    g.C = cop;
  }
  if (rop) {
    HIPCK(f32_to_op(compute, a->resid, nC, rop, st));
    g.resid = rop;
  }
  if (epi == EPI_QKV) {
    HIPCK(rope_table(a->seq_len, rope, st));
    if (a->rope_out)
      HIPCK(hipMemcpyAsync(a->rope_out, rope, (size_t)a->seq_len * 32 * sizeof(float2), hipMemcpyDeviceToDevice, st));
    g.rope = rope;
    g.seq_len = a->seq_len;
    g.heads = a->heads;
    g.rope_heads = a->rope_heads > 0 ? a->rope_heads : a->heads;
    g.q_scale = a->q_scale;
    g.q = compute ? qop : (void*)a->q;
    g.k = compute ? kop : (void*)a->k;
    g.v = compute ? vop : (void*)a->v;
    g.C = nullptr;
    g.ldc = 0;
    g.q_norm_w = a->q_norm_w;
    g.k_norm_w = a->k_norm_w;
    g.qk_norm_eps = a->qk_norm_eps;
    g.qkv_dst_len = a->qkv_dst_len;
    if (a->qkv_dst_len && compute) {
      HIPCK(f32_to_op(compute, a->q, nqkv, qop, st));
      HIPCK(f32_to_op(compute, a->k, nqkv, kop, st));
      HIPCK(f32_to_op(compute, a->v, nqkv, vop, st));
    }
  }
  if (fold_prod) {
    const int live_fill = a->poison ? 0xFF : 0;
    HIPCK(hipMemsetAsync(a->ln_part_out, live_fill, lp_live, st));
    HIPCK(hipMemsetAsync(reinterpret_cast<char*>(a->ln_part_out) + lp_live, 0xFF, lp_all - lp_live, st));
    g.ln_part = a->ln_part_out;
    if (hsop) {
      HIPCK(hipMemsetAsync(hsop, live_fill, hs_live, st));
      HIPCK(hipMemsetAsync(reinterpret_cast<char*>(hsop) + hs_live, 0xFF, hs_all - hs_live, st));
      g.hs = hsop;
      g.hs_scale = a->hs_scale;
    }
  }
  if (fold_cons) {
    g.ln_part_in = a->ln_part_in;
    g.ln_u = a->ln_u;
    g.ln_v = a->ln_v;
  }
  if (fold) {
    g.ln_nparts = a->ln_nparts;
    g.ln_rms = a->ln_rms;
    g.ln_eps = a->ln_eps;
  }
  HIPCK(gemm(compute, epi, g, st));
  if (hsop) HIPCK(op_to_f32(compute, hsop, (int64_t)(M + F5H_OP_GUARD_ROWS) * N, a->hs_out, st));
  if (cop) HIPCK(op_to_f32(compute, cop, nC, a->C, st));
  if (epi == EPI_QKV && compute) {
    HIPCK(op_to_f32(compute, qop, nqkv, a->q, st));
    HIPCK(op_to_f32(compute, kop, nqkv, a->k, st));
    HIPCK(op_to_f32(compute, vop, nqkv, a->v, st));
  }
  return 0;
}

int f5h_op_text_upsample(void* stream, int32_t B, int32_t nt, int32_t N, int32_t td, const int64_t* text,
                         const int32_t* seq_len, const float* in, float* out) {
  if (B <= 0 || nt < 0 || N <= 0 || N > 8192 || td <= 0 || td % 4)
    return fail(F5H_EINVAL, "op_text_upsample needs B > 0, nt >= 0, 0 < N <= 8192 and td % 4 == 0");
  if ((nt > 0 && !text) || !in || !out || in == out) return fail(F5H_EINVAL, "op_text_upsample: null or aliased tensor");
  TextUpArgs u{};
  u.text = text;
  u.B = B;
  u.nt = nt;
  u.N = N;
  u.td = td;
  u.seq_len = seq_len;
  u.in_c = in;
  u.out_c = out;
  HIPCK(text_upsample(u, reinterpret_cast<hipStream_t>(stream)));
  return 0;
}

int f5h_op_lnfold_uv(void* stream, int32_t compute, int32_t nfe, int32_t depth, int32_t d, int32_t F, float* table,
                     int64_t stride, int64_t out_off, const float* W1, const float* Wqkv, void* workspace,
                     size_t workspace_bytes) {
  if (compute != F5H_BF16 && compute != F5H_FP16) return fail(F5H_EINVAL, "op_lnfold_uv needs a 16-bit compute mode");
  if (nfe <= 0 || depth <= 0 || d <= 0 || F <= 0 || d % 64 || F % 64)
    return fail(F5H_EINVAL, "op_lnfold_uv needs nfe, depth > 0 and d % 64 == 0, F % 64 == 0");
  const int64_t LW = 2 * (int64_t)F + 6 * (int64_t)d;
  if (stride % 4 || out_off < 6 * (int64_t)d * depth || stride < out_off + depth * LW)
    return fail(F5H_EINVAL, "op_lnfold_uv: stride % 4 == 0, u / v blocks past the modulation rows and inside the row");
  if (!table || !W1 || !Wqkv) return fail(F5H_EINVAL, "op_lnfold_uv: null tensor");
  hipStream_t st = reinterpret_cast<hipStream_t>(stream);
  const int64_t n1 = (int64_t)F * d, nq = 3 * (int64_t)d * d;
  OpWs ws(workspace, workspace_bytes);
  void* w1op = ws.take((size_t)depth * n1 * 2);
  void* wqop = ws.take((size_t)depth * nq * 2);
  const void** ptrs = reinterpret_cast<const void**>(ws.take(2 * (size_t)depth * sizeof(void*)));
  OPWS_CHECK(ws, "op_lnfold_uv");
  HIPCK(f32_to_op(compute, W1, depth * n1, w1op, st));
  HIPCK(f32_to_op(compute, Wqkv, depth * nq, wqop, st));
  std::vector<const void*> host(2 * (size_t)depth);
  for (int l = 0; l < depth; ++l) {
    host[l] = reinterpret_cast<const char*>(w1op) + (size_t)l * n1 * 2;
    host[depth + l] = reinterpret_cast<const char*>(wqop) + (size_t)l * nq * 2;
  }
  HIPCK(hipMemcpyAsync(ptrs, host.data(), host.size() * sizeof(void*), hipMemcpyHostToDevice, st));
  HIPCK(hipStreamSynchronize(st));
  LnFoldArgs la{};
  la.table = table;
  la.stride = stride;
  la.out_off = out_off;
  la.nfe = nfe;
  la.depth = depth;
  la.d = d;
  la.F = F;
  la.w1 = ptrs;
  la.wqkv = ptrs + depth;
  HIPCK(lnfold_uv(compute, la, st));
  return 0;
}

int f5h_op_scale_cols(void* stream, int32_t compute, int64_t rows, int32_t K, const float* W, const float* g,
                      float* out, void* workspace, size_t workspace_bytes) {
  if (compute != F5H_BF16 && compute != F5H_FP16) return fail(F5H_EINVAL, "op_scale_cols needs a 16-bit compute mode");
  if (rows <= 0 || K <= 0 || K % 8) return fail(F5H_EINVAL, "op_scale_cols needs rows > 0 and K % 8 == 0");
  if (!W || !g || !out) return fail(F5H_EINVAL, "op_scale_cols: null tensor");
  hipStream_t st = reinterpret_cast<hipStream_t>(stream);
  const int64_t n = rows * K;
  OpWs ws(workspace, workspace_bytes);
  void* wop = ws.take((size_t)n * 2);
  void* oop = ws.take((size_t)n * 2);
  OPWS_CHECK(ws, "op_scale_cols");
  HIPCK(f32_to_op(compute, W, n, wop, st));
  HIPCK(scale_cols(compute, wop, rows, K, g, oop, st));
  HIPCK(op_to_f32(compute, oop, n, out, st));
  return 0;
}

}
```

### f5-tts_amd/csrc/engine_pack.cpp

```cpp
#include "engine_internal.h"

static constexpr size_t kProbeBytes = (64 + 2 * (size_t)kProbeEnd) * sizeof(unsigned long long);

struct WView {
  const void* p;
  int dt;
  int64_t numel;
};
struct WMap {
  std::unordered_map<std::string, WView> m;
  const WView* get(const std::string& n, int64_t numel, std::string* err) const {
    auto it = m.find(n);
    if (it == m.end()) {
      *err = "missing weight " + n;
      return nullptr;
    }
    if (it->second.numel != numel) {
      *err = "weight " + n + " has " + std::to_string(it->second.numel) + " elements, expected " +
             std::to_string(numel);
      return nullptr;
    }
    return &it->second;
  }
};
// ... 316 lines not shown
    const WView* nw = W.get("norm_out.linear.weight", (int64_t)2 * d * d, &err);
    const WView* nb = nw ? W.get("norm_out.linear.bias", 2 * d, &err) : nullptr;
    if (!nw || !nb) return fail(F5H_ENOWEIGHT, err);
    ada_blocks.push_back(Block{nw, 2 * d, d, 0, d, 0});
    ada_bias.push_back(nb);
    RC(make_lin(e, ada_blocks, d, ada_bias, &e->ada));
    if (a.long_skip_connection) {
      const WView* sw = W.get("long_skip_connection.weight", (int64_t)d * 2 * d, &err);
      if (!sw) return fail(F5H_EINVAL, "long_skip_connection: " + err);
      RC(make_lin(e, {Block{sw, d, 2 * d, 0, 2 * d, 0}}, 2 * d, {}, &e->long_skip));
    }
  } else {
    RC(vec_upload(e, W, "norm_out.g", d, &e->norm_out_g, &err));
  }
  RC(lin_simple(e, W, "proj_out.weight", "proj_out.bias", mel, d, &e->proj_out, &err));
  return 0;
}

static int check_arch(const f5h_arch* a) {
  if (!a) return fail(F5H_EINVAL, "null arch");
  if (a->backbone != F5H_DIT && a->backbone != F5H_UNETT && a->backbone != F5H_MMDIT)
    return fail(F5H_EINVAL, "backbone must be DiT, UNetT or MMDiT");
  if (a->backbone == F5H_MMDIT) {
    if (a->text_dim != a->dim) return fail(F5H_EINVAL, "MMDiT: text_dim must equal dim");
    if (a->conv_layers != 0) return fail(F5H_EINVAL, "MMDiT: conv_layers must be 0");
    if (a->pe_attn_head != 0) return fail(F5H_EINVAL, "MMDiT: pe_attn_head must be 0");
    if (a->long_skip_connection != 0) return fail(F5H_EINVAL, "MMDiT: long_skip_connection must be 0");
    if (a->text_average_upsampling != 0) return fail(F5H_EINVAL, "MMDiT: text_average_upsampling must be 0");
    if (a->depth < 1) return fail(F5H_EINVAL, "MMDiT: depth must be >= 1");
  }
  if (a->dim_head != 64) return fail(F5H_EINVAL, "dim_head must be 64");
  if (a->dim % 128 || a->dim <= 0 || a->dim > 1024) return fail(F5H_EINVAL, "dim must be a multiple of 128, <= 1024");
  if (a->heads * 64 != a->dim) return fail(F5H_EINVAL, "heads*dim_head must equal dim");
  if (a->ff_dim % 64 || a->ff_dim <= 0) return fail(F5H_EINVAL, "ff_dim must be a positive multiple of 64");
  if (a->mel_dim != 100) return fail(F5H_EINVAL, "mel_dim must be 100");
  if (a->backbone != F5H_MMDIT && (a->text_dim <= 0 || a->text_dim % 4 || a->text_dim > 512))
    return fail(F5H_EINVAL, "text_dim must be <= 512, % 4");
  if (a->depth <= 0 || (a->backbone == F5H_UNETT && a->depth % 2)) return fail(F5H_EINVAL, "bad depth");
  if (a->backbone == F5H_UNETT && a->conv_layers != 0) return fail(F5H_EINVAL, "UNetT with conv_layers unsupported");
  if (a->compute != F5H_FP32 && a->compute != F5H_BF16 && a->compute != F5H_FP16)
    return fail(F5H_EINVAL, "compute must be FP32, BF16 or FP16");
  if (a->qk_norm != 0 && a->qk_norm != 1) return fail(F5H_EINVAL, "qk_norm must be 0 (none) or 1 (rms_norm)");
  if ((a->long_skip_connection != 0 && a->long_skip_connection != 1) ||
      (a->text_average_upsampling != 0 && a->text_average_upsampling != 1))
    return fail(F5H_EINVAL, "long_skip_connection and text_average_upsampling must be 0 or 1");
  if (a->backbone != F5H_DIT && (a->long_skip_connection || a->text_average_upsampling))
    return fail(F5H_EINVAL, "long_skip_connection and text_average_upsampling are DiT options");
  if (a->text_average_upsampling && !a->text_mask_padding)
    return fail(F5H_EINVAL, "text_embedding_average_upsampling requires text_mask_padding to be True");
  return 0;
}

extern "C" {

int f5h_engine_create_views(const f5h_arch* arch, const f5h_tensor_view* weights, int32_t n_weights, int32_t device,
                            f5h_engine** out) {
  if (!out) return fail(F5H_EINVAL, "null out");
  *out = nullptr;
  RC(check_arch(arch));
  if (n_weights < 0 || (n_weights > 0 && !weights)) return fail(F5H_EINVAL, "null weights");
  for (int i = 0; i < n_weights; ++i) {
    const f5h_tensor_view& v = weights[i];
    if (!v.name || (!v.data && v.numel > 0) || v.numel < 0) return fail(F5H_EINVAL, "bad weight view");
    if (v.dtype != F5H_DT_F32 && v.dtype != F5H_DT_BF16 && v.dtype != F5H_DT_F16)
      return fail(F5H_EINVAL, std::string("weight ") + v.name + ": dtype must be F5H_DT_F32, _BF16 or _F16");
    if (v.on_device != 0 && v.on_device != 1)
      return fail(F5H_EINVAL, std::string("weight ") + v.name + ": on_device must be 0 or 1");
  }
  HIPCK(hipSetDevice(device));
  f5h_engine* e = new f5h_engine();
  if (hipStreamCreateWithFlags(&e->mstream, hipStreamNonBlocking) != hipSuccess) {
    delete e;
    return fail(F5H_EHIP, "engine stream");
  }
  e->a = *arch;
  e->dev = device;
  e->bf = arch->compute;
  e->esz = e->bf ? 2 : 4;
  e->tdp = arch->backbone == F5H_MMDIT ? 0 : (arch->text_dim + 63) / 64 * 64;
  if (const char* gv = getenv("F5H_GRAPH")) e->graph_mode = atoi(gv) ? 1 : 0;
  if (const char* sv = getenv("F5H_SPLIT_CFG")) e->split_cfg = std::min(2, std::max(0, atoi(sv)));
  if (const char* pv = getenv("F5H_NO_PAD_SKIP")) e->pad_skip = (*pv == '1') ? 0 : 1;
  if (const char* cv = getenv("F5H_CHAIN")) e->chain = (*cv == '1') ? 1 : 0;
  {
    hipEvent_t ev = nullptr;
    if (hipEventCreateWithFlags(&ev, hipEventDisableTiming) == hipSuccess) {
      if (hipEventRecord(ev, nullptr) != hipSuccess || hipStreamWaitEvent(e->mstream, ev, 0) != hipSuccess)
        (void)hipGetLastError();
      (void)hipEventDestroy(ev);
    } else {
      (void)hipGetLastError();
    }
  }
  WMap W;
  std::vector<void*> staged;
  int rc = 0;
  for (int i = 0; i < n_weights && !rc; ++i) {
    const f5h_tensor_view& v = weights[i];
    const size_t bytes = (size_t)v.numel * (v.dtype == F5H_DT_F32 ? 4 : 2);
    const void* dp = v.data;
    if (!v.on_device && bytes) {
      void* t = dev_alloc(device, bytes, e->mstream);
      if (!t) {
        rc = fail(F5H_EHIP, "weight staging allocation");
        break;
      }
      staged.push_back(t);
      if (hipMemcpyAsync(t, v.data, bytes, hipMemcpyHostToDevice, e->mstream) != hipSuccess) {
        rc = fail(F5H_EHIP, std::string("weight staging copy: ") + v.name);
        break;
      }
      dp = t;
    } else if (v.on_device && bytes) {
      hipPointerAttribute_t at{};
      if (hipPointerGetAttributes(&at, v.data) != hipSuccess || at.device != device) {
        (void)hipGetLastError();
        rc = fail(F5H_EINVAL, std::string("weight ") + v.name + ": on_device view is not memory of device " +
                                  std::to_string(device));
        break;
      }
    }
    W.m[v.name] = WView{dp, v.dtype, v.numel};
  }
  if (!rc) rc = pack_all(e, W);
  if (!rc && arch->backbone == F5H_DIT) {
    e->lnf_ok = e->bf != 0 && arch->dim % 64 == 0 && arch->dim <= 1024 && arch->ff_dim % 64 == 0;
    e->ada_row = e->ada.Npad + (e->lnf_ok ? (int64_t)arch->depth * (2 * (int64_t)arch->ff_dim + 6 * (int64_t)arch->dim) : 0);
    if (e->lnf_ok) {
      std::vector<const void*> wp;
      for (const Layer& L : e->layers) wp.push_back(L.ff1.w);
      for (const Layer& L : e->layers) wp.push_back(L.qkv.w);
      if (upload(e, wp, &e->lnf_w)) e->lnf_ok = false;
    }
  }
  if (!rc && arch->backbone == F5H_MMDIT) e->ada_row = e->ada.Npad;
  if (!rc && arch->backbone == F5H_UNETT && e->bf != 0 && arch->dim % 64 == 0 && arch->dim <= 1024) {
    e->rmsf_ok = true;
    for (Layer& L : e->layers) {
      L.qkv_g = L.qkv;
      L.ff1_g = L.ff1;
      if (dalloc(e, (size_t)L.qkv.Npad * L.qkv.K * e->esz, &L.qkv_g.w) ||
          dalloc(e, (size_t)L.ff1.Npad * L.ff1.K * e->esz, &L.ff1_g.w) ||
          scale_cols(e->bf, L.qkv.w, L.qkv.Npad, L.qkv.K, L.g_attn, L.qkv_g.w, e->mstream) != hipSuccess ||
          scale_cols(e->bf, L.ff1.w, L.ff1.Npad, L.ff1.K, L.g_ff, L.ff1_g.w, e->mstream) != hipSuccess) {
        e->rmsf_ok = false;
        break;
      }
    }
  }
  e->lnfold = arch->backbone == F5H_DIT ? 1 : 0;
  if (const char* lv = getenv("F5H_LNFOLD")) e->lnfold = (*lv == '0') ? 0 : 1;
  if (!rc && hipStreamSynchronize(e->mstream) != hipSuccess) rc = fail(F5H_EHIP, "weight packing");
  for (void* t : staged) dev_free(t, e->mstream);
  if (rc) {
    f5h_engine_destroy(e);
    return rc;
  }
  {
    void* p = nullptr;
    int khz = 0;
    void* tl = nullptr;
    if (dalloc(e, kProbeBytes, &p) || dalloc(e, (size_t)kTimelineWG * 4 * sizeof(unsigned long long), &tl) ||
        hipStreamSynchronize(e->mstream) != hipSuccess) {
      f5h_engine_destroy(e);
      return fail(F5H_EHIP, "probe buffers");
    }
// ... 60 lines not shown
```

### f5-tts_amd/csrc/kernels.h

```cpp
#pragma once
#include <hip/hip_runtime.h>
#include <stddef.h>
#include <stdint.h>

namespace f5h {

enum ComputeMode { F5H_C_FP32 = 0, F5H_C_BF16 = 1, F5H_C_FP16 = 2 };

enum Epi {
  EPI_STORE = 0,
  EPI_SILU = 1,
  EPI_GELU_TANH = 2,
  EPI_GELU_ERF = 3,
  EPI_RESID = 4,
  EPI_RESID_FILL = 5,
  EPI_INPROJ = 6,
  EPI_QKV = 7,
  EPI_GELU_ERF_OP = 8,
  EPI_RESID16 = 9,
  EPI_STORE16 = 10,
};

constexpr int kProbeTicks = 512, kProbeSites = 64, kProbeLanes = 16, kProbeStride = 16, kProbeEvery = 4;
constexpr int64_t kProbeRow = (int64_t)kProbeTicks * kProbeLanes * kProbeStride;
// ... 70 lines not shown

constexpr float kAttnScale = 0.125f;
struct AttnArgs {
  const void* q; const void* k; const void* v; void* o;
  int S, H, L;
  int kv_start2;
  const int32_t* kv_len;
  const int32_t* q_len;
  int prescaled;
  int o_split;
  DevProbe probe;
  int force_safe;
  int store_wt;
  void* o2;
  const int32_t* kv_len2;
};
constexpr int kAttnRagged = -1;
static_assert(sizeof(AttnArgs) == 120, "AttnArgs: keep the kernel argument's size (see the layout note)");
hipError_t attention(int compute, const AttnArgs& a, hipStream_t st);
int attention_store_wt(int compute, const AttnArgs& a, int want);
void attention_force_safe(int on);

struct ConvArgs {
  const void* x; int x_f32;
  int ragged;
  const void* w;
  const float* bias;
  const uint8_t* rowkeep;
  int S, L, d;
  int mode;
  void* y; int64_t y_seq_stride; int64_t y_row_off;
  const float* resid;
};
hipError_t conv_pos(int compute, const ConvArgs& a, hipStream_t st);

hipError_t time_sinus(const float* t_host, int n, float* out, hipStream_t st);
hipError_t time_sinus_dev(const float* tg, int n, float* out, hipStream_t st);
hipError_t silu_to_op(int compute, const float* x, void* y, int64_t n, hipStream_t st);
hipError_t ln_modulate(int compute, const void* h, int h16, int M, int d, const float* shift, const float* scale,
                       void* out, hipStream_t st);
hipError_t rms_norm_g(int compute, const void* h, int h16, int M, int d, const float* g, void* out, hipStream_t st);
hipError_t scale_cols(int compute, const void* W, int64_t rows, int K, const float* g, void* out, hipStream_t st);
hipError_t rope_table(int L, float2* out, hipStream_t st);
struct TextEmbArgs {
  const int64_t* text; int B, nt, N, td;
  const int32_t* seq_len;
  const float* table;
  const float* freqs;
  int freq_rows;
  int mask_padding;
  float* out_c; float* out_u;
  uint8_t* keep;
  const int32_t* seg_off;
};
hipError_t text_embed(const TextEmbArgs& a, hipStream_t st);
struct TextUpArgs {
  const int64_t* text; int B, nt, N, td;
  const int32_t* seq_len;
  const float* in_c; const float* in_u;
  float* out_c; float* out_u;
};
hipError_t text_upsample(const TextUpArgs& a, hipStream_t st);
hipError_t dwconv_ln(int compute, const float* x, int S, int L, int C, const float* dw_w, const float* dw_b,
                     const float* ln_w, const float* ln_b, void* out, hipStream_t st, const int32_t* len = nullptr,
                     int len_mod = 1);
hipError_t grn(int compute, const float* x, int S, int L, int C, const float* gamma, const float* beta,
               float* scratch , void* out, hipStream_t st, const int32_t* len = nullptr,
               int len_mod = 1);
hipError_t build_ct(int compute, const float* cond, const uint8_t* cond_mask, const float* text_c,
                    const float* text_u, int B, int N, int td, int S, int drop_audio, int drop_text, void* out,
                    hipStream_t st);
hipError_t pack_y(int compute, const float* y, int rows, int mel, void* ypad, hipStream_t st);
struct EulerArgs {
  float* y; int B, N, mel;
  const float* p; int64_t p_seq_stride; int p_row_off; int64_t p_ld;
  int use_cfg; float cfg; float dt;
  void* ypad; int compute;
  float* traj;
  const int* kstep; const float* tgrid; float* const* trajp;
  const float* next_src; int64_t next_stride; int next_n; float* next_dst; int nfe;
  unsigned* arrive; int* tick;
};
hipError_t cfg_euler(const EulerArgs& a, hipStream_t st);
constexpr int kOdeMethods = 3;
struct OdeTableau {
  int stages;
  float c[4], a[16], b[4];
};
constexpr float kOneThird = (float)(1.0 / 3.0), kTwoThirds = (float)(2.0 / 3.0);
constexpr OdeTableau ode_tableau(int method) {
  return method == 1   ? OdeTableau{2, {0.f, 0.5f}, {0.f, 0.f, 0.f, 0.f, 0.5f}, {0.f, 1.f}}
         : method == 2 ? OdeTableau{4,
                                    {0.f, kOneThird, kTwoThirds, 1.f},
                                    {0.f, 0.f, 0.f, 0.f, kOneThird, 0.f, 0.f, 0.f, -kOneThird, 1.f, 0.f, 0.f, 1.f, -1.f, 1.f, 0.f},
                                    {0.125f, 0.375f, 0.375f, 0.125f}}
                       : OdeTableau{1, {0.f}, {0.f}, {1.f}};
}
constexpr int ode_kept_slopes(int method) { return method == 2 ? 3 : 0; }
struct RkArgs {
  float* y; int B, N, mel;
  const float* p; int64_t p_seq_stride; int p_row_off; int64_t p_ld;
  int use_cfg; float cfg;
  void* ypad; int compute;
  int method;
  float* kbuf;
  int* keval; const float* sgrid; float* const* trajp;
  const float* next_src; int64_t next_stride; int next_n; float* next_dst; int neval;
  unsigned* arrive; int* tick;
};
hipError_t cfg_rk(const RkArgs& a, hipStream_t st);
hipError_t grid_upload(const float* t_host, int n, float* out, hipStream_t st);
hipError_t step_begin(const int* kstep, const float* src, int64_t stride, int n, float* dst, hipStream_t st);
hipError_t stamp_begin(unsigned long long* slots, const int* tick, hipStream_t st);
hipError_t stamp_end(unsigned long long* slots, const int* tick, hipStream_t st);
hipError_t step_advance(int* kstep, int* tick, hipStream_t st);
hipError_t zero_words(unsigned* p, int64_t n, hipStream_t st);
hipError_t final_where(const float* cond, const uint8_t* cond_mask, float* y, int B, int N, int mel,
                       hipStream_t st);
hipError_t final_where_out(const float* cond, const uint8_t* cond_mask, const float* y, float* out, int B, int N,
                           int mel, const unsigned* fault, hipStream_t st);
hipError_t ptr_upload(float* p, float** slot, hipStream_t st);
hipError_t build_rowkeep(const int32_t* dur, int B, int S, int L, int off, uint8_t* keep, hipStream_t st);
hipError_t build_textkeep(const int64_t* text, int B, int S, int nt, uint8_t* keep, hipStream_t st);
hipError_t build_kvlen(const int32_t* dur, int B, int S, int off, int32_t* kv, hipStream_t st);
hipError_t build_textlen(const int64_t* text, int B, int S, int nt, int32_t* len, hipStream_t st);
hipError_t write_time_token(int compute, int h16, const float* temb, int S, int L, int d, void* h, hipStream_t st);
hipError_t copy_pred(const float* p, int S, int L, int row_off, int mel, int64_t p_ld, float* dst,
                     const unsigned* fault, hipStream_t st);
hipError_t vocos_im2col(int compute, const float* mel, int B, int T, int C, int Kp, void* out, hipStream_t st);
hipError_t vocos_spec(float* x, int64_t rows, int bins, int ld, hipStream_t st);
hipError_t vocos_ola(const float* frames, const float* win, int B, int T, int n_fft, int hop, float* y,
                     hipStream_t st);
hipError_t mel_frames(const float* wav, int B, int L, int T, int n_fft, int hop, float* frames, hipStream_t st);
hipError_t mel_mag(const float* spec, int64_t rows, int bins, int ld_spec, int ld_mag, float* mag, hipStream_t st);
hipError_t mel_log(const float* mel, int B, int T, int n_mels, float* out, hipStream_t st);
hipError_t seg_upload(const int32_t* host, int64_t n, int32_t* out, hipStream_t st);
hipError_t dwconv_ln_ragged(int compute, const float* x, const int32_t* off, int B, int R, int C, const float* dw_w,
                            const float* dw_b, const float* ln_w, const float* ln_b, void* out, hipStream_t st);
hipError_t vocos_im2col_ragged(int compute, const float* src, int64_t row_st, int64_t frame_st, int64_t chan_st,
                               const int32_t* off, const int32_t* start, int B, int R, int C, int Kp, void* out,
                               hipStream_t st);
hipError_t vocos_ola_ragged(const float* frames, const float* win, const int32_t* off, int B, int R, int n_fft,
                            int hop, float* y, hipStream_t st);
hipError_t mel_frames_ragged(const float* wav, int64_t wav_st, const int32_t* off, const int32_t* len, int B, int R,
                             int n_fft, int hop, float* frames, hipStream_t st);
hipError_t mel_log_ragged(const float* mel, const int32_t* off, int B, int T_out, int n_mels, float* out,
                          hipStream_t st);
hipError_t grn_ragged(int compute, const float* x, const int32_t* off, int S, int R, int Lmax, int C,
                      const float* gamma, const float* beta, float* scratch, void* out, hipStream_t st);
hipError_t build_rowtab(const int32_t* off, int S, int R, int2* rowtab, int32_t* len, hipStream_t st);
hipError_t f32_to_op(int compute, const float* x, int64_t n, void* out, hipStream_t st);
hipError_t op_to_f32(int compute, const void* x, int64_t n, float* out, hipStream_t st);
struct PackArgs {
  const void* src; int src_dt; int64_t src_st[4];
  void* dst; int dst_dt; int64_t dst_st[3];
  int n[4];
};
hipError_t pack_strided(const PackArgs& a, hipStream_t st);

constexpr int kChainRows = 64;
struct ChainDep {
  const unsigned* wait;
  int wait_mult, wait_unit;
  unsigned* pub;
  unsigned* err;
  unsigned spin_limit;
// ... 32 lines not shown
```

### f5-tts_amd/csrc/lnrow.h

```cpp
#pragma once
#include "common.h"

namespace f5h {

template <typename T> F5H_DEV void store4(T* p, float a, float b, float c, float d);
template <> F5H_DEV void store4<float>(float* p, float a, float b, float c, float d) {
  *reinterpret_cast<float4*>(p) = make_float4(a, b, c, d);
}
template <> F5H_DEV void store4<bf16>(bf16* p, float a, float b, float c, float d) {
  bf16x4 v = {f2bf(a), f2bf(b), f2bf(c), f2bf(d)};
  *reinterpret_cast<bf16x4*>(p) = v;
}
template <> F5H_DEV void store4<f16>(f16* p, float a, float b, float c, float d) {
  f16x4 v = {(f16)a, (f16)b, (f16)c, (f16)d};
  *reinterpret_cast<f16x4*>(p) = v;
}

template <typename TI> F5H_DEV float4 load4f(const TI* p);
template <> F5H_DEV float4 load4f<float>(const float* p) { return *reinterpret_cast<const float4*>(p); }
template <> F5H_DEV float4 load4f<bf16>(const bf16* p) {
  const bf16x4 v = *reinterpret_cast<const bf16x4*>(p);
  return make_float4((float)v[0], (float)v[1], (float)v[2], (float)v[3]);
}
template <> F5H_DEV float4 load4f<f16>(const f16* p) {
  const f16x4 v = *reinterpret_cast<const f16x4*>(p);
  return make_float4((float)v[0], (float)v[1], (float)v[2], (float)v[3]);
}

F5H_DEV float wave_sum_dpp(float v) {
  auto dpp = [](float x, int ctrl) -> float {
    switch (ctrl) {
      case 0xB1: return __int_as_float(__builtin_amdgcn_update_dpp(0, __float_as_int(x), 0xB1, 0xF, 0xF, false));
      case 0x4E: return __int_as_float(__builtin_amdgcn_update_dpp(0, __float_as_int(x), 0x4E, 0xF, 0xF, false));
      case 0x141: return __int_as_float(__builtin_amdgcn_update_dpp(0, __float_as_int(x), 0x141, 0xF, 0xF, false));
      default: return __int_as_float(__builtin_amdgcn_update_dpp(0, __float_as_int(x), 0x140, 0xF, 0xF, false));
    }
  };
  v += dpp(v, 0xB1);
  v += dpp(v, 0x4E);
  v += dpp(v, 0x141);
  v += dpp(v, 0x140);
  const float r0 = __int_as_float(__builtin_amdgcn_readlane(__float_as_int(v), 0));
  const float r1 = __int_as_float(__builtin_amdgcn_readlane(__float_as_int(v), 16));
  const float r2 = __int_as_float(__builtin_amdgcn_readlane(__float_as_int(v), 32));
  const float r3 = __int_as_float(__builtin_amdgcn_readlane(__float_as_int(v), 48));
  return (r0 + r1) + (r2 + r3);
}

template <typename TO, int V, bool FIXED>
F5H_DEV void ln_mod_row(const float4 (&v)[V], const float4 (&a)[V], const float4 (&b)[V], int lane, int n4, int d,
                        TO* orow) {
  float s = 0.f;
#pragma unroll
  for (int k = 0; k < V; ++k) s += v[k].x + v[k].y + v[k].z + v[k].w;
  const float mean = wave_sum_dpp(s) / d;
  float q = 0.f;
#pragma unroll
  for (int k = 0; k < V; ++k) {
    const int i = lane + 64 * k;
    if (FIXED || i < n4) {
      float p0 = v[k].x - mean, p1 = v[k].y - mean, p2 = v[k].z - mean, p3 = v[k].w - mean;
      q += p0 * p0 + p1 * p1 + p2 * p2 + p3 * p3;
    }
  }
  const float rstd = rsqrtf(wave_sum_dpp(q) / d + 1e-6f);
#pragma unroll
  for (int k = 0; k < V; ++k) {
    const int i = lane + 64 * k;
    if (FIXED || i < n4)
      store4<TO>(orow + 4 * i, (v[k].x - mean) * rstd * (1.f + a[k].x) + b[k].x,
                 (v[k].y - mean) * rstd * (1.f + a[k].y) + b[k].y, (v[k].z - mean) * rstd * (1.f + a[k].z) + b[k].z,
                 (v[k].w - mean) * rstd * (1.f + a[k].w) + b[k].w);
  }
}

template <typename T>
F5H_DEV void ln16_row(const uint4 (&x)[2], const float4 (&a)[2][2], const float4 (&b)[2][2], uint4 (&o)[2]) {
  typedef typename Op16<T>::v8 v8;
  constexpr int d = 1024;
  float v[2][8];
#pragma unroll
  for (int k = 0; k < 2; ++k) {
    const v8 w = __builtin_bit_cast(v8, x[k]);
#pragma unroll
    for (int e = 0; e < 8; ++e) v[k][e] = to_f32(w[e]);
  }
  float s = 0.f;
#pragma unroll
  for (int k = 0; k < 2; ++k)
#pragma unroll
    for (int e = 0; e < 8; ++e) s += v[k][e];
  const float mean = wave_sum_dpp(s) / d;
  float q = 0.f;
#pragma unroll
  for (int k = 0; k < 2; ++k)
#pragma unroll
    for (int e = 0; e < 8; ++e) {
      const float p = v[k][e] - mean;
      q += p * p;
    }
  const float rstd = rsqrtf(wave_sum_dpp(q) / d + 1e-6f);
#pragma unroll
  for (int k = 0; k < 2; ++k) {
    const float av[8] = {a[k][0].x, a[k][0].y, a[k][0].z, a[k][0].w, a[k][1].x, a[k][1].y, a[k][1].z, a[k][1].w};
    const float bv[8] = {b[k][0].x, b[k][0].y, b[k][0].z, b[k][0].w, b[k][1].x, b[k][1].y, b[k][1].z, b[k][1].w};
    v8 w;
#pragma unroll
    for (int e = 0; e < 8; ++e) w[e] = from_f32<T>((v[k][e] - mean) * rstd * (1.f + av[e]) + bv[e]);
    o[k] = __builtin_bit_cast(uint4, w);
  }
}

}
```

### f5-tts_amd/f5_tts_amd/_lib.py

```python

from __future__ import annotations

import ctypes
import os

import torch

_HERE = os.path.dirname(os.path.abspath(__file__))
LIB_PATH = os.environ.get("F5H_LIB", os.path.join(_HERE, "lib", "libf5h.so"))

F5H_DIT, F5H_UNETT, F5H_MMDIT = 0, 1, 2
BACKBONE = {"DiT": F5H_DIT, "UNetT": F5H_UNETT, "MMDiT": F5H_MMDIT}
F5H_FP32, F5H_BF16, F5H_FP16 = 0, 1, 2
COMPUTE = {"fp32": F5H_FP32, "bf16": F5H_BF16, "fp16": F5H_FP16}
F5H_DT_F32, F5H_DT_BF16, F5H_DT_F16 = 0, 1, 2
F5H_EULER, F5H_MIDPOINT, F5H_RK4 = 0, 1, 2
ODE_METHOD = {"euler": F5H_EULER, "midpoint": F5H_MIDPOINT, "rk4": F5H_RK4}

EXPORTS = (
    "f5h_engine_create_views",
    "f5h_engine_create",
    "f5h_engine_destroy",
    "f5h_release_pending",
    "f5h_workspace_size",
    "f5h_sample",
    "f5h_workspace_size_ode",
    "f5h_sample_ode",
    "f5h_workspace_size_ragged",
    "f5h_sample_ragged",
    "f5h_debug_ode_tableau",
    "f5h_debug_ode_eval_times",
    "f5h_forward",
    "f5h_probe_enable",
    "f5h_probe_read",
    "f5h_probe_timeline",
    "f5h_set_graph_mode",
    "f5h_set_cfg_streams",
    "f5h_graph_stats",
    "f5h_last_call_host_ms",
    "f5h_set_pad_skip",
    "f5h_set_chain",
    "f5h_chain_stats",
    "f5h_chain_debug_spin_limit",
    "f5h_set_ln_fold",
    "f5h_ln_fold_stats",
    "f5h_set_store_policy",
    "f5h_store_policy_stats",
    "f5h_store_policy_force",
    "f5h_op_linear",
    "f5h_op_attention",
    "f5h_op_attention_qlen",
    "f5h_op_attention_split",
    "f5h_op_attention_ranges",
    "f5h_op_conv_pos",
    "f5h_op_norm",
    "f5h_op_dwconv_ln",
    "f5h_op_dwconv_ln_len",
    "f5h_op_grn",
    "f5h_op_grn_len",
    "f5h_op_attention_ragged",
    "f5h_op_conv_pos_ragged",
    "f5h_op_grn_ragged",
    "f5h_op_gemm_epi",
    "f5h_op_text_upsample",
    "f5h_op_lnfold_uv",
    "f5h_op_scale_cols",
    "f5h_gemm_force_config",
    "f5h_attn_force_safe",
    "f5h_debug_tile_live",
    "f5h_vocos_create",
    "f5h_vocos_destroy",
    "f5h_vocos_workspace_size",
    "f5h_vocos_decode",
    "f5h_vocos_ragged_workspace_size",
    "f5h_vocos_decode_ragged",
    "f5h_mel_create",
    "f5h_mel_destroy",
    "f5h_mel_workspace_size",
    "f5h_mel_forward",
    "f5h_mel_ragged_workspace_size",
    "f5h_mel_forward_ragged",
    "f5h_last_error",
    "f5h_version",
)

KCLASS = {"ffn1": 0, "attention": 1, "qkv": 2, "ffn2": 3, "conv": 4, "out": 5, "norm": 6, "chain": 7}


class Arch(ctypes.Structure):
    _fields_ = [(n, ctypes.c_int32) for n in (
        "backbone", "dim", "depth", "heads", "dim_head", "ff_dim", "text_dim", "text_num_embeds", "mel_dim",
        "conv_layers", "text_mask_padding", "pe_attn_head", "attn_mask_enabled", "compute",
        "qk_norm", "long_skip_connection", "text_average_upsampling")]


class VocosArch(ctypes.Structure):
    _fields_ = [(n, ctypes.c_int32) for n in (
        "input_channels", "dim", "intermediate_dim", "num_layers", "n_fft", "hop_length", "compute")]


class MelArch(ctypes.Structure):
    _fields_ = [(n, ctypes.c_int32) for n in ("n_fft", "hop_length", "n_mels", "sample_rate")]


class Weight(ctypes.Structure):
    _fields_ = [("name", ctypes.c_char_p), ("data", ctypes.c_void_p), ("numel", ctypes.c_int64)]


class TensorView(ctypes.Structure):
    _fields_ = [("name", ctypes.c_char_p), ("data", ctypes.c_void_p), ("dtype", ctypes.c_int32),
                ("on_device", ctypes.c_int32), ("numel", ctypes.c_int64)]


class SampleArgs(ctypes.Structure):
    _fields_ = [
        ("B", ctypes.c_int32), ("N", ctypes.c_int32), ("nt", ctypes.c_int32), ("nfe", ctypes.c_int32),
        ("cond", ctypes.c_void_p), ("cond_mask", ctypes.c_void_p), ("text", ctypes.c_void_p),
        ("duration", ctypes.c_void_p), ("y0", ctypes.c_void_p), ("t_grid", ctypes.c_void_p),
        ("cfg_strength", ctypes.c_float), ("use_batch_mask", ctypes.c_int32),
        ("out", ctypes.c_void_p), ("trajectory", ctypes.c_void_p),
    ]


class ForwardArgs(ctypes.Structure):
    _fields_ = [
        ("B", ctypes.c_int32), ("N", ctypes.c_int32), ("nt", ctypes.c_int32),
        ("x", ctypes.c_void_p), ("cond", ctypes.c_void_p), ("cond_mask", ctypes.c_void_p),
        ("text", ctypes.c_void_p), ("duration", ctypes.c_void_p), ("t", ctypes.c_float),
        ("use_batch_mask", ctypes.c_int32), ("pred", ctypes.c_void_p),
        ("cfg_infer", ctypes.c_int32), ("drop_audio_cond", ctypes.c_int32), ("drop_text", ctypes.c_int32),
        ("t_dev", ctypes.c_void_p), ("text_cache", ctypes.c_int32),
    ]


class OpGemmArgs(ctypes.Structure):
    _fields_ = [
        ("compute", ctypes.c_int32), ("epi", ctypes.c_int32), ("M", ctypes.c_int32), ("N", ctypes.c_int32),
        ("K", ctypes.c_int32), ("k_split", ctypes.c_int32),
        ("A", ctypes.c_void_p), ("A2", ctypes.c_void_p), ("W", ctypes.c_void_p), ("bias", ctypes.c_void_p),
        ("C", ctypes.c_void_p), ("resid", ctypes.c_void_p), ("gate", ctypes.c_void_p), ("rowkeep", ctypes.c_void_p),
        ("live_len", ctypes.c_void_p), ("live_seq", ctypes.c_int32),
        ("seq_len", ctypes.c_int32), ("heads", ctypes.c_int32), ("rope_heads", ctypes.c_int32),
        ("q_scale", ctypes.c_float),
        ("add", ctypes.c_void_p), ("ld_add", ctypes.c_int64), ("dual_rows", ctypes.c_int64),
        ("q", ctypes.c_void_p), ("k", ctypes.c_void_p), ("v", ctypes.c_void_p), ("rope_out", ctypes.c_void_p),
        ("hs_scale", ctypes.c_void_p), ("hs_out", ctypes.c_void_p), ("ln_part_out", ctypes.c_void_p),
        ("ln_part_in", ctypes.c_void_p), ("ln_u", ctypes.c_void_p), ("ln_v", ctypes.c_void_p),
        ("ln_nparts", ctypes.c_int32), ("ln_rms", ctypes.c_int32), ("ln_eps", ctypes.c_float),
        ("poison", ctypes.c_int32),
        ("q_norm_w", ctypes.c_void_p), ("k_norm_w", ctypes.c_void_p), ("qk_norm_eps", ctypes.c_float),
        ("qkv_dst_len", ctypes.c_int32),
        ("seg_off", ctypes.c_void_p), ("n_seq", ctypes.c_int32),
    ]


class RaggedArgs(ctypes.Structure):
    _fields_ = [
        ("B", ctypes.c_int32), ("Lmax", ctypes.c_int32), ("nt", ctypes.c_int32), ("nfe", ctypes.c_int32),
        ("R", ctypes.c_int64),
        ("cond", ctypes.c_void_p), ("cond_mask", ctypes.c_void_p), ("text", ctypes.c_void_p),
        ("duration", ctypes.c_void_p), ("y0", ctypes.c_void_p), ("t_grid", ctypes.c_void_p),
        ("cfg_strength", ctypes.c_float),
        ("out", ctypes.c_void_p), ("trajectory", ctypes.c_void_p),
    ]


OP_GUARD_ROWS = 4


_lib = None
_load_error = None


def lib():
    global _lib, _load_error
    if _lib is not None:
        return _lib
    if _load_error is not None:
        raise RuntimeError(_load_error)
    if not os.path.exists(LIB_PATH):
        _load_error = (f"libf5h.so not found at {LIB_PATH}: build it with `python -c \"import __graft_entry__ as g; "
                       f"g.build()\"` or `make -C f5-tts_amd/csrc`")
        raise RuntimeError(_load_error)
    L = ctypes.CDLL(LIB_PATH)
    vp, i32, i64, sz = ctypes.c_void_p, ctypes.c_int32, ctypes.c_int64, ctypes.c_size_t
    L.f5h_engine_create.argtypes = [ctypes.POINTER(Arch), ctypes.POINTER(Weight), i32, i32, ctypes.POINTER(vp)]
    L.f5h_engine_create.restype = ctypes.c_int
    L.f5h_engine_create_views.argtypes = [ctypes.POINTER(Arch), ctypes.POINTER(TensorView), i32, i32,
                                          ctypes.POINTER(vp)]
    L.f5h_engine_create_views.restype = ctypes.c_int
    L.f5h_engine_destroy.argtypes = [vp]
    L.f5h_engine_destroy.restype = None
    L.f5h_release_pending.argtypes = [i32]
    L.f5h_release_pending.restype = ctypes.c_int
    L.f5h_workspace_size.argtypes = [vp, i32, i32, i32, i32, i32]
    L.f5h_workspace_size.restype = sz
    L.f5h_sample.argtypes = [vp, vp, ctypes.POINTER(SampleArgs), vp, sz]
    L.f5h_sample.restype = ctypes.c_int
    if hasattr(L, "f5h_sample_ode"):
        L.f5h_workspace_size_ode.argtypes = [vp, i32, i32, i32, i32, i32, i32]
        L.f5h_workspace_size_ode.restype = sz
        L.f5h_sample_ode.argtypes = [vp, vp, ctypes.POINTER(SampleArgs), i32, vp, sz]
        L.f5h_sample_ode.restype = ctypes.c_int
        fp = ctypes.POINTER(ctypes.c_float)
        L.f5h_debug_ode_tableau.argtypes = [i32, ctypes.POINTER(i32), fp, fp, fp]
        L.f5h_debug_ode_tableau.restype = ctypes.c_int
        L.f5h_debug_ode_eval_times.argtypes = [i32, i32, fp, i32, fp]
        L.f5h_debug_ode_eval_times.restype = ctypes.c_int
    L.f5h_forward.argtypes = [vp, vp, ctypes.POINTER(ForwardArgs), vp, sz]
    L.f5h_forward.restype = ctypes.c_int
    L.f5h_probe_enable.argtypes = [vp, i32, i32]
    L.f5h_probe_enable.restype = ctypes.c_int
    L.f5h_probe_read.argtypes = [vp, ctypes.POINTER(i64), ctypes.POINTER(ctypes.c_double)]
    L.f5h_probe_read.restype = ctypes.c_int
    L.f5h_probe_timeline.argtypes = [vp, ctypes.POINTER(ctypes.c_uint64), i32, ctypes.POINTER(i32),
                                     ctypes.POINTER(ctypes.c_double)]
    L.f5h_probe_timeline.restype = ctypes.c_int
    L.f5h_set_graph_mode.argtypes = [vp, i32]
    L.f5h_set_graph_mode.restype = ctypes.c_int
    L.f5h_set_cfg_streams.argtypes = [vp, i32]
    L.f5h_set_cfg_streams.restype = ctypes.c_int
    L.f5h_graph_stats.argtypes = [vp, ctypes.POINTER(i64), ctypes.POINTER(i64), ctypes.POINTER(i32)]
    L.f5h_graph_stats.restype = ctypes.c_int
    if hasattr(L, "f5h_last_call_host_ms"):
        L.f5h_last_call_host_ms.argtypes = [vp, ctypes.POINTER(ctypes.c_double), i32]
        L.f5h_last_call_host_ms.restype = ctypes.c_int
    L.f5h_set_pad_skip.argtypes = [vp, i32]
    L.f5h_set_pad_skip.restype = ctypes.c_int
    L.f5h_op_linear.argtypes = [vp, i32, i32, i32, i32, vp, vp, vp, vp, vp, sz]
    L.f5h_op_linear.restype = ctypes.c_int
    L.f5h_op_attention.argtypes = [vp, i32, i32, i32, i32, vp, vp, vp, vp, i32, vp, vp, sz]
    L.f5h_op_attention.restype = ctypes.c_int
    if hasattr(L, "f5h_op_gemm_epi"):
        L.f5h_op_attention_qlen.argtypes = [vp, i32, i32, i32, i32, vp, vp, vp, vp, vp, i32, vp, vp, sz]
        L.f5h_op_attention_qlen.restype = ctypes.c_int
        L.f5h_op_conv_pos.argtypes = [vp, i32, i32, i32, i32, vp, vp, vp, vp, i32, vp, i32, i64, i64, vp, vp, sz]
        L.f5h_op_conv_pos.restype = ctypes.c_int
        L.f5h_op_norm.argtypes = [vp, i32, i32, i32, i32, i32, vp, vp, vp, vp, vp, sz]
        L.f5h_op_norm.restype = ctypes.c_int
        L.f5h_op_dwconv_ln.argtypes = [vp, i32, i32, i32, i32, vp, vp, vp, vp, vp, vp, vp, sz]
        L.f5h_op_dwconv_ln.restype = ctypes.c_int
        L.f5h_op_grn.argtypes = [vp, i32, i32, i32, i32, vp, vp, vp, vp, vp, sz]
        L.f5h_op_grn.restype = ctypes.c_int
        L.f5h_op_gemm_epi.argtypes = [vp, ctypes.POINTER(OpGemmArgs), vp, sz]
        L.f5h_op_gemm_epi.restype = ctypes.c_int
        if hasattr(L, "f5h_op_lnfold_uv"):
            L.f5h_op_lnfold_uv.argtypes = [vp, i32, i32, i32, i32, i32, vp, i64, i64, vp, vp, vp, sz]
            L.f5h_op_lnfold_uv.restype = ctypes.c_int
            L.f5h_op_scale_cols.argtypes = [vp, i32, i64, i32, vp, vp, vp, vp, sz]
            L.f5h_op_scale_cols.restype = ctypes.c_int
    if hasattr(L, "f5h_op_attention_split"):
        L.f5h_op_attention_split.argtypes = [vp, i32, i32, i32, i32, vp, vp, vp, vp, vp, i32, i32, vp, vp, vp, sz]
        L.f5h_op_attention_split.restype = ctypes.c_int
    if hasattr(L, "f5h_op_attention_ranges"):
        L.f5h_op_attention_ranges.argtypes = [vp, i32, i32, i32, i32, vp, vp, vp, vp, i32, vp, vp, i32, vp, vp, sz]
        L.f5h_op_attention_ranges.restype = ctypes.c_int
        L.f5h_op_dwconv_ln_len.argtypes = [vp, i32, i32, i32, i32, vp, vp, vp, vp, vp, vp, vp, vp, sz]
        L.f5h_op_dwconv_ln_len.restype = ctypes.c_int
        L.f5h_op_grn_len.argtypes = [vp, i32, i32, i32, i32, vp, vp, vp, vp, vp, vp, sz]
        L.f5h_op_grn_len.restype = ctypes.c_int
    if hasattr(L, "f5h_op_text_upsample"):
        L.f5h_op_text_upsample.argtypes = [vp, i32, i32, i32, i32, vp, vp, vp, vp]
        L.f5h_op_text_upsample.restype = ctypes.c_int
    L.f5h_gemm_force_config.argtypes = [i32]
    L.f5h_gemm_force_config.restype = ctypes.c_int
    if hasattr(L, "f5h_attn_force_safe"):
        L.f5h_attn_force_safe.argtypes = [i32]
        L.f5h_attn_force_safe.restype = ctypes.c_int
    if hasattr(L, "f5h_set_chain"):
        L.f5h_set_chain.argtypes = [vp, i32]
        L.f5h_set_chain.restype = ctypes.c_int
        L.f5h_chain_stats.argtypes = [vp, ctypes.POINTER(i64), ctypes.POINTER(i32), ctypes.POINTER(i64)]
        L.f5h_chain_stats.restype = ctypes.c_int
    if hasattr(L, "f5h_set_ln_fold"):
        L.f5h_set_ln_fold.argtypes = [vp, i32]
        L.f5h_set_ln_fold.restype = ctypes.c_int
        L.f5h_ln_fold_stats.argtypes = [vp, ctypes.POINTER(i32), ctypes.POINTER(i64)]
        L.f5h_ln_fold_stats.restype = ctypes.c_int
    if hasattr(L, "f5h_set_store_policy"):
        L.f5h_set_store_policy.argtypes = [vp, i32]
        L.f5h_set_store_policy.restype = ctypes.c_int
        L.f5h_store_policy_stats.argtypes = [vp, ctypes.POINTER(i64), ctypes.POINTER(i64)]
        L.f5h_store_policy_stats.restype = ctypes.c_int
        L.f5h_store_policy_force.argtypes = [i32]
        L.f5h_store_policy_force.restype = ctypes.c_int
    if hasattr(L, "f5h_chain_debug_spin_limit"):
        L.f5h_chain_debug_spin_limit.argtypes = [i64]
        L.f5h_chain_debug_spin_limit.restype = ctypes.c_int
    if hasattr(L, "f5h_debug_tile_live"):
        L.f5h_debug_tile_live.argtypes = [vp, i32, i32, i32, i32]
        L.f5h_debug_tile_live.restype = ctypes.c_int
    L.f5h_vocos_create.argtypes = [ctypes.POINTER(VocosArch), ctypes.POINTER(Weight), i32, i32, ctypes.POINTER(vp)]
    L.f5h_vocos_create.restype = ctypes.c_int
    L.f5h_vocos_destroy.argtypes = [vp]
    L.f5h_vocos_destroy.restype = None
    L.f5h_vocos_workspace_size.argtypes = [vp, i32, i32]
    L.f5h_vocos_workspace_size.restype = sz
    L.f5h_vocos_decode.argtypes = [vp, vp, i32, i32, vp, vp, vp, sz]
    L.f5h_vocos_decode.restype = ctypes.c_int
    L.f5h_mel_create.argtypes = [ctypes.POINTER(MelArch), i32, ctypes.POINTER(vp)]
    L.f5h_mel_create.restype = ctypes.c_int
    L.f5h_mel_destroy.argtypes = [vp]
    L.f5h_mel_destroy.restype = None
    L.f5h_mel_workspace_size.argtypes = [vp, i32, i32]
    L.f5h_mel_workspace_size.restype = sz
    L.f5h_mel_forward.argtypes = [vp, vp, i32, i32, vp, vp, vp, sz]
    L.f5h_mel_forward.restype = ctypes.c_int
    if hasattr(L, "f5h_vocos_decode_ragged"):
        L.f5h_vocos_ragged_workspace_size.argtypes = [vp, i32, i64]
        L.f5h_vocos_ragged_workspace_size.restype = sz
        L.f5h_vocos_decode_ragged.argtypes = [vp, vp, i32, vp, i64, i64, i64, ctypes.POINTER(i32), ctypes.POINTER(i32),
                                              vp, vp, sz]
        L.f5h_vocos_decode_ragged.restype = ctypes.c_int
        L.f5h_mel_ragged_workspace_size.argtypes = [vp, i32, i64]
        L.f5h_mel_ragged_workspace_size.restype = sz
        L.f5h_mel_forward_ragged.argtypes = [vp, vp, i32, vp, i64, ctypes.POINTER(i32), i32, vp, vp, sz]
        L.f5h_mel_forward_ragged.restype = ctypes.c_int
    if hasattr(L, "f5h_sample_ragged"):
        L.f5h_workspace_size_ragged.argtypes = [vp, i32, i64, i32, i32, i32, i32, i32]
        L.f5h_workspace_size_ragged.restype = sz
        L.f5h_sample_ragged.argtypes = [vp, vp, ctypes.POINTER(RaggedArgs), i32, vp, sz]
        L.f5h_sample_ragged.restype = ctypes.c_int
        pi32 = ctypes.POINTER(i32)
        L.f5h_op_attention_ragged.argtypes = [vp, i32, i32, i32, i32, i32, pi32, vp, vp, vp, i32, vp, vp, sz]
        L.f5h_op_attention_ragged.restype = ctypes.c_int
        L.f5h_op_conv_pos_ragged.argtypes = [vp, i32, i32, i32, i32, i32, pi32, vp, vp, vp, i32, vp, i32, vp, vp, sz]
        L.f5h_op_conv_pos_ragged.restype = ctypes.c_int
        L.f5h_op_grn_ragged.argtypes = [vp, i32, i32, i32, i32, i32, pi32, vp, vp, vp, vp, vp, sz]
        L.f5h_op_grn_ragged.restype = ctypes.c_int
    L.f5h_last_error.argtypes = []
    L.f5h_last_error.restype = ctypes.c_char_p
    L.f5h_version.argtypes = []
    L.f5h_version.restype = ctypes.c_char_p
    _lib = L
    return L


def has_ode() -> bool:
    return hasattr(lib(), "f5h_sample_ode")


def has_dit_options() -> bool:
    return hasattr(lib(), "f5h_op_text_upsample")


def has_mmdit() -> bool:
    return hasattr(lib(), "f5h_op_attention_split")


def has_isolate() -> bool:
    return hasattr(lib(), "f5h_op_attention_ranges")


def has_ragged() -> bool:
    return hasattr(lib(), "f5h_vocos_decode_ragged")


def has_ragged_sampler() -> bool:
    return hasattr(lib(), "f5h_sample_ragged")


def check(rc: int, what: str = "f5h"):
    if rc != 0:
        msg = lib().f5h_last_error().decode(errors="replace")
        raise RuntimeError(f"{what} failed (status {rc}): {msg}")


def host_ints(x, n: int, what: str) -> "list[int]":
    if torch.is_tensor(x):
        if x.device.type != "cpu":
            raise ValueError(f"{what} must be host values (ints, a list or a CPU tensor), not a tensor on {x.device}: "
                             "reading it back would synchronise the device")
        x = x.reshape(-1).tolist()
    elif isinstance(x, int):
        x = [x] * n
    vals = [int(v) for v in x]
    if len(vals) != n:
        raise ValueError(f"{what} has {len(vals)} entries for {n} utterances")
    return vals


def ptr(t) -> int | None:
    return None if t is None else t.data_ptr()


def stream_handle(device=None) -> int:
    return torch.cuda.current_stream(device).cuda_stream
```

### f5-tts_amd/f5_tts_amd/engine.py

```python

from __future__ import annotations

import ctypes
import threading

import numpy as np
import torch

from . import _lib


_VIEW_DT = {torch.float32: _lib.F5H_DT_F32, torch.bfloat16: _lib.F5H_DT_BF16, torch.float16: _lib.F5H_DT_F16}


def _arch_struct(arch: dict, compute: str) -> _lib.Arch:
    if arch["backbone"] == "MMDiT":
        return _mmdit_arch_struct(arch, compute)
    a = _lib.Arch()
    a.backbone = _lib.F5H_DIT if arch["backbone"] == "DiT" else _lib.F5H_UNETT
    a.dim = arch["dim"]
    a.depth = arch["depth"]
    a.heads = arch["heads"]
    a.dim_head = arch.get("dim_head", 64)
    a.ff_dim = int(arch["dim"] * arch["ff_mult"])
# ... 98 lines not shown

    def __init__(self, arch: dict, weights: dict, compute: str = "bf16", device=None):
        L = _lib.lib()
        self.arch = dict(arch)
        self.compute = compute
        self.device = torch.device("cuda", torch.cuda.current_device() if device is None else
                                   torch.device(device).index or 0)
        keep, views = [], []
        for k, v in weights.items():
            k = k[len("transformer."):] if k.startswith("transformer.") else k
            t = v.detach() if isinstance(v, torch.Tensor) else torch.from_numpy(np.ascontiguousarray(v))
            if t.dtype not in _VIEW_DT:
                t = t.to(torch.float32)
            if t.is_cuda and t.device != self.device:
                t = t.to(self.device)
            t = t.contiguous()
            keep.append(t)
            views.append((k.encode(), t))
        arr = (_lib.TensorView * len(views))()
        for i, (name, t) in enumerate(views):
            arr[i].name = name
            arr[i].data = t.data_ptr()
            arr[i].dtype = _VIEW_DT[t.dtype]
            arr[i].on_device = int(t.is_cuda)
            arr[i].numel = t.numel()
        a = _arch_struct(self.arch, compute)
        h = ctypes.c_void_p()
        with torch.cuda.device(self.device):
            if any(t.is_cuda for t in keep):
                torch.cuda.current_stream(self.device).synchronize()
            _lib.check(L.f5h_engine_create_views(ctypes.byref(a), arr, len(views), self.device.index,
                                                 ctypes.byref(h)), "f5h_engine_create_views")
        del keep
        self._h = h
        self._lock = threading.Lock()
        self._ws_cache: dict = {}

    def __del__(self):
        h = getattr(self, "_h", None)
        if h is not None and h.value:
            try:
                _lib.lib().f5h_engine_destroy(h)
            except Exception:
                pass
            self._h = None

    def workspace_bytes(self, B, N, nt, nfe, use_cfg=True, method="euler") -> int:
        m = _ode_method(method)
        if not _lib.has_ode():
            return int(_lib.lib().f5h_workspace_size(self._h, B, N, nt, nfe, int(use_cfg)))
        return int(_lib.lib().f5h_workspace_size_ode(self._h, B, N, nt, nfe, int(use_cfg), m))

    def _workspace(self, nbytes):
        return torch.empty(max(nbytes, 256), dtype=torch.uint8, device=self.device)

    def _cached_workspace(self, nbytes, stream):
        with self._lock:
            ent = self._ws_cache.get((stream, nbytes))
            if ent is None:
                if len(self._ws_cache) >= 4:
                    self._ws_cache.pop(next(iter(self._ws_cache)))
                ent = (self._workspace(nbytes), threading.Lock())
                self._ws_cache[(stream, nbytes)] = ent
            return ent

    def set_graph_mode(self, on: bool):
        _lib.check(_lib.lib().f5h_set_graph_mode(self._h, int(bool(on))), "set_graph_mode")

    def set_cfg_streams(self, n: int):
        _lib.check(_lib.lib().f5h_set_cfg_streams(self._h, int(n)), "set_cfg_streams")

    def set_pad_skip(self, on: bool):
        _lib.check(_lib.lib().f5h_set_pad_skip(self._h, int(bool(on))), "set_pad_skip")

    def set_chain(self, on: bool):
        _lib.check(_lib.lib().f5h_set_chain(self._h, int(bool(on))), "set_chain")

    def set_ln_fold(self, on: bool):
        _lib.check(_lib.lib().f5h_set_ln_fold(self._h, int(bool(on))), "set_ln_fold")

    def ln_fold_stats(self):
        sup, n = ctypes.c_int32(), ctypes.c_int64()
        _lib.check(_lib.lib().f5h_ln_fold_stats(self._h, ctypes.byref(sup), ctypes.byref(n)), "ln_fold_stats")
        return bool(sup.value), int(n.value)

    STORE_CLASS_BITS = {"qkv": 1, "attn": 2, "out": 4, "ffn1": 8, "ffn2": 16}

    def set_store_policy(self, mode: int):
        _lib.check(_lib.lib().f5h_set_store_policy(self._h, int(mode)), "set_store_policy")

    def store_policy_stats(self):
        wt, plain = ctypes.c_int64(), ctypes.c_int64()
        _lib.check(_lib.lib().f5h_store_policy_stats(self._h, ctypes.byref(wt), ctypes.byref(plain)), "store_policy_stats")
        return int(wt.value), int(plain.value)

    def chain_stats(self):
        n, f, r = ctypes.c_int64(), ctypes.c_int32(), ctypes.c_int64()
        _lib.check(_lib.lib().f5h_chain_stats(self._h, ctypes.byref(n), ctypes.byref(f), ctypes.byref(r)),
                   "chain_stats")
        return int(n.value), int(f.value), int(r.value)

    HOST_PHASES = ("total", "prologue", "cache_lock", "reap", "capture", "instantiate", "launch", "final")

    def last_call_host_ms(self):
        buf = (ctypes.c_double * 8)()
        _lib.check(_lib.lib().f5h_last_call_host_ms(self._h, buf, 8), "last_call_host_ms")
        return {k: round(buf[i], 4) for i, k in enumerate(self.HOST_PHASES)}

    def graph_stats(self):
        cap, rep, n = ctypes.c_int64(), ctypes.c_int64(), ctypes.c_int32()
        _lib.check(_lib.lib().f5h_graph_stats(self._h, ctypes.byref(cap), ctypes.byref(rep), ctypes.byref(n)),
                   "graph_stats")
        return {"captures": cap.value, "replays": rep.value, "cached": n.value}

    def sample(self, cond, cond_mask, text, duration, y0, t_grid, cfg_strength, use_batch_mask,
               out=None, keep_trajectory=True, workspace=None, method="euler"):
        _refuse_mmdit_masked(self.arch, use_batch_mask)
        mode = _mask_mode(self.arch, use_batch_mask)
        B, N, mel = cond.shape
        nt = text.shape[1]
        tg = np.ascontiguousarray(np.asarray(t_grid, dtype=np.float32))
        nfe = tg.shape[0] - 1
        cond = cond.to(self.device, torch.float32).contiguous()
        cmask = cond_mask.to(self.device, torch.uint8).contiguous()
        text = text.to(self.device, torch.int64).contiguous()
        dur = duration.to(self.device, torch.int32).contiguous()
        y0 = y0.to(self.device, torch.float32).contiguous()
        if out is None:
            out = torch.empty(B, N, mel, dtype=torch.float32, device=self.device)
        traj = (torch.empty(nfe + 1, B, N, mel, dtype=torch.float32, device=self.device)
                if keep_trajectory else None)
        use_cfg = cfg_strength >= 1e-5
        m = _ode_method(method)
        need = self.workspace_bytes(B, N, nt, nfe, use_cfg, method)
        stream = _lib.stream_handle(self.device)
        if workspace is not None and workspace.numel() >= need:
            ws, wlock = workspace, threading.Lock()
        else:
            ws, wlock = self._cached_workspace(need, stream)
        a = _lib.SampleArgs()
        a.B, a.N, a.nt, a.nfe = B, N, nt, nfe
        a.cond, a.cond_mask, a.text, a.duration, a.y0 = (cond.data_ptr(), cmask.data_ptr(), text.data_ptr(),
                                                         dur.data_ptr(), y0.data_ptr())
        a.t_grid = tg.ctypes.data
        a.cfg_strength = float(cfg_strength)
        a.use_batch_mask = mode
        a.out = out.data_ptr()
        a.trajectory = traj.data_ptr() if traj is not None else None
        with torch.cuda.device(self.device), wlock:
            if _lib.has_ode():
                _lib.check(_lib.lib().f5h_sample_ode(self._h, stream, ctypes.byref(a), m, ws.data_ptr(), ws.numel()),
                           "f5h_sample_ode")
            else:
                _lib.check(_lib.lib().f5h_sample(self._h, stream, ctypes.byref(a), ws.data_ptr(), ws.numel()),
                           "f5h_sample")
        return out, traj

    def workspace_bytes_ragged(self, durations, nt, nfe, use_cfg=True, method="euler", lmax=None) -> int:
        _refuse_ragged(self.arch)
        dur = [int(d) for d in durations]
        return int(_lib.lib().f5h_workspace_size_ragged(self._h, len(dur), sum(dur), int(lmax or max(dur)), nt, nfe,
                                                        int(use_cfg), _ode_method(method)))

    def sample_ragged(self, cond, cond_mask, text, durations, y0, t_grid, cfg_strength, keep_trajectory=True,
                      workspace=None, method="euler", lmax=None):
        _refuse_ragged(self.arch)
# ... 179 lines not shown
def op_attention_ragged(Q, K, V, seg_off, compute="bf16", q_prescaled=False):
    if not _lib.has_ragged_sampler():
        raise RuntimeError("the loaded libf5h.so has no f5h_op_attention_ragged (an older build)")
    S, H, Lmax, D = Q.shape
    assert D == 64
    arr, off = _seg_array(seg_off)
    R = off[-1]
    O = torch.full((R, H * 64), float("nan"), dtype=torch.float32, device=Q.device)
    ws = torch.empty(Q.numel() * 6 + O.numel() * 2 + R * 8 + S * 8 + 4096, dtype=torch.uint8, device=Q.device)
    _lib.check(_lib.lib().f5h_op_attention_ragged(_lib.stream_handle(Q.device), _lib.COMPUTE[compute], S, H, Lmax, R,
                                                  arr, Q.contiguous().data_ptr(), K.contiguous().data_ptr(),
                                                  V.contiguous().data_ptr(), int(bool(q_prescaled)), O.data_ptr(),
                                                  ws.data_ptr(), ws.numel()), "f5h_op_attention_ragged")
    return O


def op_conv_pos_ragged(x, w, bias, seg_off, mode=0, resid=None, x_as_f32=True, compute="bf16"):
    if not _lib.has_ragged_sampler():
        raise RuntimeError("the loaded libf5h.so has no f5h_op_conv_pos_ragged (an older build)")
    R, d = x.shape
    dev = x.device
    x, w, bias, resid = _f32(x), _f32(w, dev), _f32(bias, dev), _f32(resid, dev)
    arr, off = _seg_array(seg_off)
    S, lmax = len(off) - 1, max(b - a for a, b in zip(off, off[1:]))
    y = torch.full((R, d), float("nan"), dtype=torch.float32, device=dev)
    ws = torch.empty(16 * 31 * 64 * 64 * 4 + x.numel() * 4 + S * 4 + 4096, dtype=torch.uint8, device=dev)
    _lib.check(_lib.lib().f5h_op_conv_pos_ragged(_lib.stream_handle(dev), _lib.COMPUTE[compute], S, lmax, R, d, arr,
                                                 x.data_ptr(), w.data_ptr(), bias.data_ptr(), int(mode),
                                                 _lib.ptr(resid), int(bool(x_as_f32)), y.data_ptr(), ws.data_ptr(),
                                                 ws.numel()), "f5h_op_conv_pos_ragged")
    return y


def op_grn_ragged(x, gamma, beta, seg_off, compute="bf16"):
    if not _lib.has_ragged_sampler():
        raise RuntimeError("the loaded libf5h.so has no f5h_op_grn_ragged (an older build)")
    R, C = x.shape
    dev = x.device
    x, gamma, beta = (_f32(t, dev) for t in (x, gamma, beta))
    arr, off = _seg_array(seg_off)
    S, lmax = len(off) - 1, max(b - a for a, b in zip(off, off[1:]))
    out = torch.full((R, C), float("nan"), dtype=torch.float32, device=dev)
    ws = torch.empty(((lmax + 63) // 64 + 1) * S * C * 4 + x.numel() * 2 + S * 4 + 4096, dtype=torch.uint8, device=dev)
    _lib.check(_lib.lib().f5h_op_grn_ragged(_lib.stream_handle(dev), _lib.COMPUTE[compute], S, lmax, R, C, arr,
                                            x.data_ptr(), gamma.data_ptr(), beta.data_ptr(), out.data_ptr(),
                                            ws.data_ptr(), ws.numel()), "f5h_op_grn_ragged")
    return out


def _f32(t, dev=None):
    return None if t is None else t.to(device=dev or t.device, dtype=torch.float32).contiguous()


def _u8(t, dev):
    return None if t is None else t.to(device=dev, dtype=torch.uint8).contiguous()


def op_conv_pos(x, w, bias, rowkeep=None, mode=0, resid=None, x_as_f32=True, y=None, y_row_off=0, compute="bf16"):
    S, L, d = x.shape
    dev = x.device
    x, w, bias, resid = _f32(x), _f32(w, dev), _f32(bias, dev), _f32(resid, dev)
    if y is None:
        y = torch.full((S, L + (y_row_off if mode else 0), d), float("nan"), dtype=torch.float32, device=dev)
    assert y.is_contiguous() and y.dtype == torch.float32
    keep = _u8(rowkeep, dev)
    ws = torch.empty(16 * 31 * 64 * 64 * 4 + x.numel() * 2 + y.numel() * 2 + 1024, dtype=torch.uint8, device=dev)
    _lib.check(_lib.lib().f5h_op_conv_pos(_lib.stream_handle(dev), _lib.COMPUTE[compute], S, L, d, x.data_ptr(),
                                          w.data_ptr(), bias.data_ptr(), _lib.ptr(keep), int(mode),
                                          _lib.ptr(resid), int(bool(x_as_f32)), y.shape[1], int(y_row_off),
                                          y.data_ptr(), ws.data_ptr(), ws.numel()), "f5h_op_conv_pos")
    return y


def op_norm(kind, h, p0, p1=None, h16=False, compute="bf16"):
    M, d = h.shape
    dev = h.device
    h, p0, p1 = _f32(h), _f32(p0, dev), _f32(p1, dev)
    out = torch.empty(M, d, dtype=torch.float32, device=dev)
    ws = torch.empty(h.numel() * 4 + 1024, dtype=torch.uint8, device=dev)
    _lib.check(_lib.lib().f5h_op_norm(_lib.stream_handle(dev), _lib.COMPUTE[compute], {"ln": 0, "rms": 1}[kind],
                                      int(bool(h16)), M, d, h.data_ptr(), p0.data_ptr(), _lib.ptr(p1),
                                      out.data_ptr(), ws.data_ptr(), ws.numel()), "f5h_op_norm")
    return out


def op_dwconv_ln(x, dw_w, dw_b, ln_w, ln_b, compute="bf16", seq_len=None):
    S, L, C = x.shape
    dev = x.device
    x, dw_w, dw_b, ln_w, ln_b = (_f32(t, dev) for t in (x, dw_w, dw_b, ln_w, ln_b))
    out = torch.empty(S, L, C, dtype=torch.float32, device=dev)
    ws = torch.empty(x.numel() * 2 + 1024, dtype=torch.uint8, device=dev)
    if seq_len is not None:
        if not _lib.has_isolate():
            raise RuntimeError("the loaded libf5h.so has no f5h_op_dwconv_ln_len (an older build)")
        ln = torch.as_tensor(seq_len).to(dev, torch.int32).contiguous()
        assert ln.numel() == S
        _lib.check(_lib.lib().f5h_op_dwconv_ln_len(_lib.stream_handle(dev), _lib.COMPUTE[compute], S, L, C,
                                                   x.data_ptr(), dw_w.data_ptr(), dw_b.data_ptr(), ln_w.data_ptr(),
                                                   ln_b.data_ptr(), ln.data_ptr(), out.data_ptr(), ws.data_ptr(),
                                                   ws.numel()), "f5h_op_dwconv_ln_len")
        return out
    _lib.check(_lib.lib().f5h_op_dwconv_ln(_lib.stream_handle(dev), _lib.COMPUTE[compute], S, L, C, x.data_ptr(),
                                           dw_w.data_ptr(), dw_b.data_ptr(), ln_w.data_ptr(), ln_b.data_ptr(),
                                           out.data_ptr(), ws.data_ptr(), ws.numel()), "f5h_op_dwconv_ln")
    return out


def op_grn(x, gamma, beta, compute="bf16", seq_len=None):
    S, L, C = x.shape
    dev = x.device
    x, gamma, beta = (_f32(t, dev) for t in (x, gamma, beta))
    out = torch.empty(S, L, C, dtype=torch.float32, device=dev)
    ws = torch.empty(((L + 63) // 64 + 1) * S * C * 4 + x.numel() * 2 + 1024, dtype=torch.uint8, device=dev)
    if seq_len is not None:
        if not _lib.has_isolate():
            raise RuntimeError("the loaded libf5h.so has no f5h_op_grn_len (an older build)")
        ln = torch.as_tensor(seq_len).to(dev, torch.int32).contiguous()
        assert ln.numel() == S
        _lib.check(_lib.lib().f5h_op_grn_len(_lib.stream_handle(dev), _lib.COMPUTE[compute], S, L, C, x.data_ptr(),
                                             gamma.data_ptr(), beta.data_ptr(), ln.data_ptr(), out.data_ptr(),
                                             ws.data_ptr(), ws.numel()), "f5h_op_grn_len")
        return out
    _lib.check(_lib.lib().f5h_op_grn(_lib.stream_handle(dev), _lib.COMPUTE[compute], S, L, C, x.data_ptr(),
                                     gamma.data_ptr(), beta.data_ptr(), out.data_ptr(), ws.data_ptr(), ws.numel()),
               "f5h_op_grn")
    return out


EPI = {"store": 0, "silu": 1, "gelu_tanh": 2, "gelu_erf": 3, "resid": 4, "resid_fill": 5, "inproj": 6, "qkv": 7,
       "gelu_erf_op": 8, "resid16": 9, "store16": 10}


def op_gemm_epi(epi, A, W, bias=None, C=None, compute="bf16", A2=None, k_split=0, resid=None, gate=None, rowkeep=None,
                live_len=None, live_seq=0, add=None, dual_rows=0, seq_len=0, heads=0, rope_heads=0, q_scale=0.0,
                hs_scale=None, ln_producer=False, ln_part_in=None, ln_u=None, ln_v=None, ln_rms=False, ln_eps=0.0,
                ln_nparts=None, poison=False, ws_fill=None, return_ws=False, q_norm_w=None, k_norm_w=None,
                qk_norm_eps=1e-6, qkv_dst_len=0, qkv_bufs=None, qkv_row0=0, seg_off=None):
    M, K = A.shape
    N = W.shape[0]
    dev = A.device
    A, A2, W, bias, resid, gate, add = (_f32(t, dev) for t in (A, A2, W, bias, resid, gate, add))
    keep = _u8(rowkeep, dev)
    ll = None if live_len is None else live_len.to(dev, torch.int32).contiguous()
    a = _lib.OpGemmArgs()
    a.compute, a.epi, a.M, a.N, a.K, a.k_split = _lib.COMPUTE[compute], EPI[epi], M, N, K, int(k_split)
    a.A, a.A2, a.W, a.bias = A.data_ptr(), _lib.ptr(A2), W.data_ptr(), _lib.ptr(bias)
    a.resid, a.gate, a.rowkeep, a.live_len, a.live_seq = _lib.ptr(resid), _lib.ptr(gate), _lib.ptr(keep), \
        _lib.ptr(ll), int(live_seq)
    a.add, a.ld_add, a.dual_rows = _lib.ptr(add), (0 if add is None else add.shape[1]), int(dual_rows)
    ws_bytes = ((N + 127) // 128 * 128) * K * 4 + 3 * M * K * 4 + 3 * (M + int(dual_rows)) * N * 4 + 4096
    hs_scale, ln_part_in, ln_u, ln_v = (_f32(t, dev) for t in (hs_scale, ln_part_in, ln_u, ln_v))
    hs = parts = None
    if ln_producer:
        G = _lib.OP_GUARD_ROWS
        a.ln_nparts = N // 64 if ln_nparts is None else int(ln_nparts)
        parts = torch.empty(M + G, max(a.ln_nparts, 1), 2, dtype=torch.float32, device=dev)
        a.ln_part_out = parts.data_ptr()
        if hs_scale is not None:
            hs = torch.empty(M + G, N, dtype=torch.float32, device=dev)
            a.hs_scale, a.hs_out = hs_scale.data_ptr(), hs.data_ptr()
            ws_bytes += (M + G) * N * 2 + 256
    elif ln_part_in is not None:
        a.ln_nparts = K // 64 if ln_nparts is None else int(ln_nparts)
        a.ln_part_in, a.ln_u, a.ln_v = ln_part_in.data_ptr(), _lib.ptr(ln_u), _lib.ptr(ln_v)
    a.ln_rms, a.ln_eps, a.poison = int(bool(ln_rms)), float(ln_eps), int(bool(poison))
    out = None
# ... 111 lines not shown
```

### include/f5h.h

```cpp
#ifndef F5H_H
#define F5H_H

#include <stddef.h>
#include <stdint.h>

#ifdef __cplusplus
extern "C" {
#endif

enum f5h_status {
  F5H_OK = 0,
  F5H_EINVAL = -1,
  F5H_EHIP = -2,
  F5H_ENOWEIGHT = -3,
  F5H_ENOMEM = -4,
};

enum f5h_backbone { F5H_DIT = 0, F5H_UNETT = 1, F5H_MMDIT = 2 };
enum f5h_compute { F5H_FP32 = 0, F5H_BF16 = 1, F5H_FP16 = 2 };

typedef struct f5h_arch {
  int32_t backbone;
  int32_t dim;
  int32_t depth;
// ... 37 lines not shown
                      int32_t device, f5h_engine** out);
void f5h_engine_destroy(f5h_engine* eng);
int f5h_release_pending(int32_t wait);

typedef struct f5h_sample_args {
  int32_t B, N, nt, nfe;
  const float* cond;
  const uint8_t* cond_mask;
  const int64_t* text;
  const int32_t* duration;
  const float* y0;
  const float* t_grid;
  float cfg_strength;
  int32_t use_batch_mask;
  float* out;
  float* trajectory;
} f5h_sample_args;

size_t f5h_workspace_size(const f5h_engine* eng, int32_t B, int32_t N, int32_t nt, int32_t nfe,
                          int32_t use_cfg);

int f5h_sample(f5h_engine* eng, void* stream, const f5h_sample_args* args, void* workspace,
               size_t workspace_bytes);

enum f5h_ode_method { F5H_EULER = 0, F5H_MIDPOINT = 1, F5H_RK4 = 2 };

size_t f5h_workspace_size_ode(const f5h_engine* eng, int32_t B, int32_t N, int32_t nt, int32_t steps,
                              int32_t use_cfg, int32_t method);
int f5h_sample_ode(f5h_engine* eng, void* stream, const f5h_sample_args* args, int32_t method, void* workspace,
                   size_t workspace_bytes);
typedef struct f5h_ragged_args {
  int32_t B, Lmax, nt, nfe;
  int64_t R;
  const float* cond;
  const uint8_t* cond_mask;
  const int64_t* text;
  const int32_t* duration;
  const float* y0;
  const float* t_grid;
  float cfg_strength;
  float* out;
  float* trajectory;
} f5h_ragged_args;
size_t f5h_workspace_size_ragged(const f5h_engine* eng, int32_t B, int64_t R, int32_t Lmax, int32_t nt, int32_t steps,
                                 int32_t use_cfg, int32_t method);
int f5h_sample_ragged(f5h_engine* eng, void* stream, const f5h_ragged_args* args, int32_t method, void* workspace,
                      size_t workspace_bytes);

int f5h_debug_ode_tableau(int32_t method, int32_t* stages, float* c, float* a, float* b);
int f5h_debug_ode_eval_times(int32_t method, int32_t compute, const float* t_grid, int32_t steps, float* out);

typedef struct f5h_forward_args {
  int32_t B, N, nt;
  const float* x;
  const float* cond;
  const uint8_t* cond_mask;
  const int64_t* text;
  const int32_t* duration;
  float t;
  int32_t use_batch_mask;
  float* pred;
  int32_t cfg_infer;
  int32_t drop_audio_cond;
  int32_t drop_text;
  const float* t_dev;
  int32_t text_cache;
} f5h_forward_args;
int f5h_forward(f5h_engine* eng, void* stream, const f5h_forward_args* args, void* workspace,
                size_t workspace_bytes);

int f5h_probe_enable(f5h_engine* eng, int32_t kclass, int32_t enable);
int f5h_probe_read(f5h_engine* eng, int64_t* launches, double* total_ms);
int f5h_probe_timeline(f5h_engine* eng, uint64_t* stamps, int32_t max_wg, int32_t* n_wg, double* tick_khz);

int f5h_set_graph_mode(f5h_engine* eng, int32_t mode);
int f5h_set_cfg_streams(f5h_engine* eng, int32_t n);
int f5h_graph_stats(f5h_engine* eng, int64_t* captures, int64_t* replays, int32_t* cached);
int f5h_last_call_host_ms(f5h_engine* eng, double* ms, int32_t n);
int f5h_set_pad_skip(f5h_engine* eng, int32_t enable);
int f5h_set_chain(f5h_engine* eng, int32_t enable);
int f5h_set_ln_fold(f5h_engine* eng, int32_t enable);
int f5h_ln_fold_stats(f5h_engine* eng, int32_t* supported, int64_t* passes);
int f5h_set_store_policy(f5h_engine* eng, int32_t mode);
int f5h_store_policy_stats(f5h_engine* eng, int64_t* write_through, int64_t* plain);
int f5h_store_policy_force(int32_t mode);
int f5h_chain_stats(f5h_engine* eng, int64_t* launches, int32_t* fault, int64_t* refused);
int f5h_chain_debug_spin_limit(int64_t limit);

int f5h_op_linear(void* stream, int32_t compute, int32_t M, int32_t N, int32_t K, const float* A,
                  const float* W, const float* bias, float* C, void* workspace, size_t workspace_bytes);
int f5h_op_attention(void* stream, int32_t compute, int32_t S, int32_t H, int32_t N, const float* Q,
                     const float* K, const float* V, const int32_t* kv_len, int32_t q_prescaled, float* O,
                     void* workspace, size_t workspace_bytes);
int f5h_op_attention_qlen(void* stream, int32_t compute, int32_t S, int32_t H, int32_t N, const float* Q,
                          const float* K, const float* V, const int32_t* kv_len, const int32_t* q_len,
                          int32_t q_prescaled, float* O, void* workspace, size_t workspace_bytes);

int f5h_op_attention_ranges(void* stream, int32_t compute, int32_t S, int32_t H, int32_t N, const float* Q,
                            const float* K, const float* V, const int32_t* kv_len, int32_t kv_start2,
                            const int32_t* kv_len2, const int32_t* q_len, int32_t q_prescaled, float* O,
                            void* workspace, size_t workspace_bytes);

int f5h_op_attention_split(void* stream, int32_t compute, int32_t S, int32_t H, int32_t N, const float* Q,
                           const float* K, const float* V, const int32_t* kv_len, const int32_t* q_len,
                           int32_t q_prescaled, int32_t o_split, float* O, float* O2, void* workspace,
                           size_t workspace_bytes);

int f5h_op_conv_pos(void* stream, int32_t compute, int32_t S, int32_t L, int32_t d, const float* x, const float* w,
                    const float* bias, const uint8_t* rowkeep, int32_t mode, const float* resid, int32_t x_as_f32,
                    int64_t y_seq_stride, int64_t y_row_off, float* y, void* workspace, size_t workspace_bytes);
int f5h_op_norm(void* stream, int32_t compute, int32_t kind, int32_t h16, int32_t M, int32_t d, const float* h,
                const float* shift_or_g, const float* scale, float* out, void* workspace, size_t workspace_bytes);
int f5h_op_dwconv_ln(void* stream, int32_t compute, int32_t S, int32_t L, int32_t C, const float* x,
                     const float* dw_w, const float* dw_b, const float* ln_w, const float* ln_b, float* out,
                     void* workspace, size_t workspace_bytes);
int f5h_op_grn(void* stream, int32_t compute, int32_t S, int32_t L, int32_t C, const float* x, const float* gamma,
               const float* beta, float* out, void* workspace, size_t workspace_bytes);
int f5h_op_dwconv_ln_len(void* stream, int32_t compute, int32_t S, int32_t L, int32_t C, const float* x,
                         const float* dw_w, const float* dw_b, const float* ln_w, const float* ln_b,
                         const int32_t* len, float* out, void* workspace, size_t workspace_bytes);
int f5h_op_grn_len(void* stream, int32_t compute, int32_t S, int32_t L, int32_t C, const float* x, const float* gamma,
                   const float* beta, const int32_t* len, float* out, void* workspace, size_t workspace_bytes);

typedef struct f5h_op_gemm_args {
  int32_t compute, epi, M, N, K, k_split;
  const float* A;
  const float* A2;
  const float* W;
  const float* bias;
  float* C;
  const float* resid;
  const float* gate;
  const uint8_t* rowkeep;
  const int32_t* live_len;
  int32_t live_seq;
  int32_t seq_len, heads, rope_heads;
  float q_scale;
  const float* add;
  int64_t ld_add;
  int64_t dual_rows;
  float* q;
  float* k;
  float* v;
  float* rope_out;
  const float* hs_scale;
  float* hs_out;
  float* ln_part_out;
  const float* ln_part_in;
  const float* ln_u;
  const float* ln_v;
  int32_t ln_nparts, ln_rms;
  float ln_eps;
  int32_t poison;
  const float* q_norm_w;
  const float* k_norm_w;
  float qk_norm_eps;
  int32_t qkv_dst_len;
  const int32_t* seg_off;
  int32_t n_seq;
} f5h_op_gemm_args;
#define F5H_OP_GUARD_ROWS 4
int f5h_op_gemm_epi(void* stream, const f5h_op_gemm_args* args, void* workspace, size_t workspace_bytes);
int f5h_op_text_upsample(void* stream, int32_t B, int32_t nt, int32_t N, int32_t td, const int64_t* text,
                         const int32_t* seq_len, const float* in, float* out);
int f5h_op_lnfold_uv(void* stream, int32_t compute, int32_t nfe, int32_t depth, int32_t d, int32_t F, float* table,
                     int64_t stride, int64_t out_off, const float* W1, const float* Wqkv, void* workspace,
                     size_t workspace_bytes);
int f5h_op_scale_cols(void* stream, int32_t compute, int64_t rows, int32_t K, const float* W, const float* g,
                      float* out, void* workspace, size_t workspace_bytes);

int f5h_op_attention_ragged(void* stream, int32_t compute, int32_t S, int32_t H, int32_t Lmax, int32_t R,
                            const int32_t* seg_off, const float* Q, const float* K, const float* V,
                            int32_t q_prescaled, float* O, void* workspace, size_t workspace_bytes);
int f5h_op_conv_pos_ragged(void* stream, int32_t compute, int32_t S, int32_t Lmax, int32_t R, int32_t d,
                           const int32_t* seg_off, const float* x, const float* w, const float* bias, int32_t mode,
                           const float* resid, int32_t x_as_f32, float* y, void* workspace, size_t workspace_bytes);
int f5h_op_grn_ragged(void* stream, int32_t compute, int32_t S, int32_t Lmax, int32_t R, int32_t C,
                      const int32_t* seg_off, const float* x, const float* gamma, const float* beta, float* out,
                      void* workspace, size_t workspace_bytes);

int f5h_gemm_force_config(int32_t cfg);
int f5h_attn_force_safe(int32_t on);
int f5h_debug_tile_live(const int32_t* live_len, int32_t live_seq, int32_t M, int32_t m0, int32_t BM);

typedef struct f5h_vocos_arch {
  int32_t input_channels;
  int32_t dim;
  int32_t intermediate_dim;
  int32_t num_layers;
  int32_t n_fft;
  int32_t hop_length;
  int32_t compute;
} f5h_vocos_arch;
// ... 38 lines not shown
```

Baseline: 19730 mel-frames/s.

## Fuse final norm, output projection, CFG Euler update and next-step input projection into one seam kernel

Adds a step_seam kernel that, at the boundary between ODE steps, does the final adaptive LayerNorm modulation, the mel output projection, the CFG Euler update, and the next step's input projection into h0, all in one launch. The backbone skips its input-projection head and output tail when the seam is active, and the first input projection moves into step setup. The aim is to remove several kernel launches and the intermediate round trips through global memory for each NFE step. The cost is one custom kernel with limited shape support (d up to a maximum, mel at most 128), which may run with lower parallelism than the separate GEMMs.

Measured after the change: 19790 mel-frames/s, median of 6. No clear change (+0.3%).

```diff
diff --git a/f5-tts_amd/csrc/elementwise.hip b/f5-tts_amd/csrc/elementwise.hip
--- a/f5-tts_amd/csrc/elementwise.hip
+++ b/f5-tts_amd/csrc/elementwise.hip
@@ -1,6 +1,7 @@
 #include "common.h"
 #include "kernels.h"
 #include "lnrow.h"
+#include "euler_step.h"
 
 #include <algorithm>
 
@@ -220,29 +221,14 @@
   return hipGetLastError();
 }
 
-constexpr int MAXV = 8;
+constexpr int MAXV = kLnMaxV;
 
 template <typename TO, int NV, typename TI = float>
 __global__ __launch_bounds__(256) void ln_mod_kernel(const TI* h, int M, int d, const float* shift,
                                                      const float* scale, TO* out) {
-  constexpr bool FIXED = NV > 0;
-  constexpr int V = FIXED ? NV : MAXV;
   const int row = blockIdx.x * 4 + (threadIdx.x >> 6), lane = threadIdx.x & 63;
   if (row >= M) return;
-  const TI* x = h + (int64_t)row * d;
-  const float4* sh = reinterpret_cast<const float4*>(shift);
-  const float4* sc = reinterpret_cast<const float4*>(scale);
-  const int n4 = FIXED ? 64 * NV : d >> 2;
-  float4 v[V], a[V], b[V];
-#pragma unroll
-  for (int k = 0; k < V; ++k) {
-    const int i = lane + 64 * k;
-    const bool ok = FIXED || i < n4;
-    v[k] = ok ? load4f<TI>(x + 4 * i) : make_float4(0, 0, 0, 0);
-    a[k] = ok ? sc[i] : make_float4(0, 0, 0, 0);
-    b[k] = ok ? sh[i] : make_float4(0, 0, 0, 0);
-  }
-  ln_mod_row<TO, V, FIXED>(v, a, b, lane, n4, d, out + (int64_t)row * d);
+  ln_mod_row_io<TO, NV, TI>(h + (int64_t)row * d, d, shift, scale, lane, out + (int64_t)row * d);
 }
 template <typename T>
 __global__ __launch_bounds__(256) void ln_mod16_kernel(const T* h, int M, const float* shift, const float* scale,
@@ -749,13 +735,11 @@
 __global__ __launch_bounds__(256) void cfg_euler_kernel(EulerArgs a, TO* ypad) {
   int64_t i = (int64_t)blockIdx.x * blockDim.x + threadIdx.x;
   const int64_t total = (int64_t)a.B * a.N * a.mel;
-  const int k = a.kstep ? __hip_atomic_load(a.kstep, __ATOMIC_RELAXED, __HIP_MEMORY_SCOPE_AGENT) : 0;
+  const int k = a.kstep ? step_index(a.kstep) : 0;
   if (a.kstep && a.next_dst) {
-    if (k + 1 < a.nfe) {
-      const float4* src = reinterpret_cast<const float4*>(a.next_src + (int64_t)(k + 1) * a.next_stride);
-      float4* dst = reinterpret_cast<float4*>(a.next_dst);
-      for (int64_t j = i; j < a.next_n / 4; j += (int64_t)gridDim.x * blockDim.x) dst[j] = src[j];
-    }
+    if (k + 1 < a.nfe)
+      step_copy_row(a.next_src + (int64_t)(k + 1) * a.next_stride, a.next_dst, a.next_n, i,
+                    (int64_t)gridDim.x * blockDim.x);
   }
   float dt = a.dt;
   float* traj = a.traj;
@@ -769,27 +753,14 @@
     const int64_t bn = i / a.mel;
     const int b = (int)(bn / a.N), n = (int)(bn - (int64_t)b * a.N);
     const float pc = a.p[(int64_t)b * a.p_seq_stride + (int64_t)(a.p_row_off + n) * a.p_ld + c];
-    float v = pc;
-    if (a.use_cfg) {
-      const float pu = a.p[(int64_t)(a.B + b) * a.p_seq_stride + (int64_t)(a.p_row_off + n) * a.p_ld + c];
-      v = add_nc(pc, mul_nc(sub_nc(pc, pu), a.cfg));
-    }
-    const float y = add_nc(a.y[i], mul_nc(dt, v));
+    float pu = 0.f;
+    if (a.use_cfg) pu = a.p[(int64_t)(a.B + b) * a.p_seq_stride + (int64_t)(a.p_row_off + n) * a.p_ld + c];
+    const float y = cfg_euler_value(pc, pu, a.use_cfg != 0, a.cfg, dt, a.y[i]);
     a.y[i] = y;
     if (ypad) ypad[bn * 128 + c] = from_f32<TO>(y);
     if (traj) traj[i] = y;
   }
-  if (a.kstep && a.arrive) {
-    __syncthreads();
-    if (threadIdx.x == 0) {
-      const unsigned old = __hip_atomic_fetch_add(a.arrive, 1u, __ATOMIC_RELAXED, __HIP_MEMORY_SCOPE_AGENT);
-      if (old == gridDim.x - 1) {
-        __hip_atomic_store(a.arrive, 0u, __ATOMIC_RELAXED, __HIP_MEMORY_SCOPE_AGENT);
-        __hip_atomic_store(const_cast<int*>(a.kstep), k + 1, __ATOMIC_RELAXED, __HIP_MEMORY_SCOPE_AGENT);
-        if (a.tick) __hip_atomic_fetch_add(a.tick, 1, __ATOMIC_RELAXED, __HIP_MEMORY_SCOPE_AGENT);
-      }
-    }
-  }
+  if (a.kstep && a.arrive) step_arrive(a.arrive, a.kstep, k, a.tick, gridDim.x);
 }
 hipError_t cfg_euler(const EulerArgs& a, hipStream_t st) {
   const int64_t total = (int64_t)a.B * a.N * a.mel;
diff --git a/f5-tts_amd/csrc/engine.cpp b/f5-tts_amd/csrc/engine.cpp
--- a/f5-tts_amd/csrc/engine.cpp
+++ b/f5-tts_amd/csrc/engine.cpp
@@ -275,7 +275,34 @@
   return 0;
 }
 
-static int backbone_part(Ctx& c, int s0, int ns, hipStream_t st) {
+static int input_proj(Ctx& c, int s0, int ns, hipStream_t st) {
+  f5h_engine* e = c.e;
+  const int d = e->a.dim, BN = c.B * c.N;
+  const size_t no = (size_t)s0 * c.N;
+  GemmArgs g = gargs(c.b.ypad, 128, e->in_x, BN, c.b.h0 + no * d, d);
+  g.bias = nullptr;
+  g.add = c.b.P + no * d;
+  g.ld_add = d;
+  g.dual_rows = ns == 2 * c.B ? BN : 0;
+  KCK(gemm(e->bf, EPI_INPROJ, g, st));
+  return 0;
+}
+
+static int seam_want(const f5h_engine* e, const Ctx& c) {
+  static const bool res32 = [] {
+    const char* v = getenv("F5H_RES32");
+    return v && *v == '1';
+  }();
+  const f5h_arch& a = e->a;
+  if (e->step_seam == 0 || a.backbone != F5H_DIT || !e->bf || res32) return 0;
+  if (c.method != F5H_EULER || !c.use_cfg || c.batch_mask || c.rag_B || a.long_skip_connection) return 0;
+  if (e->split_cfg == 1) return 0;
+  if (!step_seam_fits(a.dim, a.mel_dim) || e->proj_out.Npad != 128 || (e->ada_row & 3)) return 0;
+  if ((uint64_t)c.S * c.N * a.dim * sizeof(float) >= 0xF0000000ull) return 0;
+  return 1;
+}
+
+static int backbone_part(Ctx& c, int s0, int ns, hipStream_t st, bool skip_head = false, bool skip_tail = false) {
   f5h_engine* e = c.e;
   const f5h_arch& a = e->a;
   const int d = a.dim, bf = e->bf, H = a.heads, inner = H * 64;
@@ -310,12 +337,7 @@
   void* o = op(b.o, ro, inner);
   void* f = op(b.f, ro, a.ff_dim);
   {
-    GemmArgs g = gargs(b.ypad, 128, e->in_x, BN, b.h0 + no * d, d);
-    g.bias = nullptr;
-    g.add = b.P + no * d;
-    g.ld_add = d;
-    g.dual_rows = ns == 2 * c.B ? BN : 0;
-    KCK(gemm(bf, EPI_INPROJ, g, st));
+    if (!skip_head) RC(input_proj(c, s0, ns, st));
     ConvArgs cv{};
     cv.S = ns;
     cv.L = c.N;
@@ -558,6 +580,7 @@
       KCK(gemm(bf, epi_resid, g, st));
     }
   }
+  if (skip_tail) return 0;
   if (dit) {
     const float* fin = ada_k + (size_t)a.depth * 6 * d;
     if (hkeep) {
@@ -808,6 +831,7 @@
   key.batch_mask = c.batch_mask + c.isolate;
   key.lnfold = c.lnfold;
   key.store = c.store;
+  key.seam = c.seam;
   key.method = c.method;
   key.rag_B = c.rag_B;
   key.rag_L = c.rag_L;
@@ -835,6 +859,38 @@
 static int enqueue_step(Ctx& c, const f5h_sample_args* a) {
   f5h_engine* e = c.e;
   c.site = 0;
+  if (c.seam) {
+    RC(backbone_part(c, 0, c.S, c.st, true, true));
+    const f5h_arch& ar = e->a;
+    SeamArgs s{};
+    s.h = c.b.h;
+    s.B = c.B;
+    s.N = c.N;
+    s.d = ar.dim;
+    s.mel = ar.mel_dim;
+    s.ada = c.b.ada;
+    s.ada_row = e->ada_row;
+    s.fin_off = (int64_t)ar.depth * 6 * ar.dim;
+    s.wp = e->proj_out.w;
+    s.bp = e->proj_out.b;
+    s.wx = e->in_x.w;
+    s.P = c.b.P;
+    s.h0 = c.b.h0;
+    s.y = c.b.y;
+    s.ypad = c.b.ypad;
+    s.cfg = a->cfg_strength;
+    s.compute = e->bf;
+    s.kstep = c.b.kstep;
+    s.tgrid = c.b.tgrid;
+    s.trajp = c.b.trajp;
+    s.nfe = c.nfe;
+    s.ada_cur = c.b.ada_cur;
+    s.arrive = reinterpret_cast<unsigned*>(c.b.kstep + kArrive);
+    s.tick = e->ptick;
+    KCK(step_seam(s, c.st));
+    e->n_seam.fetch_add(1, std::memory_order_relaxed);
+    return 0;
+  }
   RC(backbone_step(c));
   const bool dit = adaln_bb(e->a);
   auto common = [&](auto& u) {
@@ -967,6 +1023,7 @@
   Ctx c{};
   const CallShape sh{a->B, a->N, a->nt, a->nfe * stages, a->cfg_strength >= 1e-5f, a->use_batch_mask, method, a->nfe};
   RC(call_begin(e, reinterpret_cast<hipStream_t>(stream), sh, workspace, workspace_bytes, rg, c, ticket));
+  c.seam = seam_want(e, c);
   if (rg) {
     std::vector<int32_t> off((size_t)2 * rg->B + 1);
     off[0] = 0;
@@ -1005,6 +1062,7 @@
   HIPCK(ptr_upload(a->trajectory, c.b.trajp, c.st));
   HIPCK(hipMemsetAsync(c.b.kstep, 0, 64 * sizeof(int), c.st));
   RC(step_prep(c));
+  if (c.seam) RC(input_proj(c, 0, c.S, c.st));
   const double h2 = host_ms();
   const double g2 = hp[HP_LOCK] + hp[HP_REAP] + hp[HP_CAPTURE] + hp[HP_INSTANTIATE];
   RC(run_steps(c, a, workspace));
diff --git a/f5-tts_amd/csrc/engine_ctl.cpp b/f5-tts_amd/csrc/engine_ctl.cpp
--- a/f5-tts_amd/csrc/engine_ctl.cpp
+++ b/f5-tts_amd/csrc/engine_ctl.cpp
@@ -111,6 +111,25 @@
   return 0;
 }
 
+int f5h_set_step_seam(f5h_engine* e, int32_t mode) {
+  if (!e) return fail(F5H_EINVAL, "null engine");
+  if (mode < -1 || mode > 1) return fail(F5H_EINVAL, "step seam must be -1 (auto), 0 (off) or 1 (on)");
+  std::lock_guard<std::mutex> g(e->gm);
+  e->step_seam = mode;
+  return 0;
+}
+
+int f5h_step_seam_stats(f5h_engine* e, int32_t* supported, int64_t* launches) {
+  if (!e) return fail(F5H_EINVAL, "null engine");
+  if (supported)
+    *supported = (e->a.backbone == F5H_DIT && e->bf && !e->a.long_skip_connection &&
+                  step_seam_fits(e->a.dim, e->a.mel_dim) && e->proj_out.Npad == 128 && !(e->ada_row & 3))
+                     ? 1
+                     : 0;
+  if (launches) *launches = e->n_seam.load(std::memory_order_relaxed);
+  return 0;
+}
+
 int f5h_set_store_policy(f5h_engine* e, int32_t mode) {
   if (!e) return fail(F5H_EINVAL, "null engine");
   if (mode != -1 && mode != 0 && mode != 1 && (mode < 0x100 || mode > 0x11F))
diff --git a/f5-tts_amd/csrc/engine_internal.h b/f5-tts_amd/csrc/engine_internal.h
--- a/f5-tts_amd/csrc/engine_internal.h
+++ b/f5-tts_amd/csrc/engine_internal.h
@@ -69,6 +69,8 @@
   int32_t drop_text;
   int32_t rag_B, rag_L;
   uint32_t cfg_bits;
+  int32_t seam;
+  int32_t reserved;
 };
 static_assert(std::has_unique_object_representations_v<GraphKey>, "GraphKey is compared as bytes: no padding");
 inline bool operator==(const GraphKey& a, const GraphKey& b) { return std::memcmp(&a, &b, sizeof(GraphKey)) == 0; }
@@ -112,6 +114,8 @@
   std::atomic<int64_t> n_lnfold{0};
   int store_policy = -1;
   std::atomic<int64_t> n_store_wt{0}, n_store_plain{0};
+  int step_seam = -1;
+  std::atomic<int64_t> n_seam{0};
   unsigned* chain_fault = nullptr;
   volatile unsigned* fault_host = nullptr;
   int fault_slot = -1;
@@ -201,6 +205,7 @@
   int chain;
   int lnfold;
   int store;
+  int seam;
   double* hp;
   int rag_B, rag_L;
 };
diff --git a/f5-tts_amd/csrc/engine_ops.cpp b/f5-tts_amd/csrc/engine_ops.cpp
--- a/f5-tts_amd/csrc/engine_ops.cpp
+++ b/f5-tts_amd/csrc/engine_ops.cpp
@@ -615,6 +615,135 @@
   return 0;
 }
 
+int f5h_op_step_seam(void* stream, const f5h_op_seam_args* a, void* workspace, size_t workspace_bytes) {
+  if (!a) return fail(F5H_EINVAL, "op_step_seam: null args");
+  const int compute = a->compute, B = a->B, N = a->N, d = a->d, mel = a->mel;
+  if (compute != F5H_BF16 && compute != F5H_FP16) return fail(F5H_EINVAL, "op_step_seam needs a 16-bit compute mode");
+  if (B <= 0 || N <= 0 || a->nfe <= 0 || a->step < 0 || a->step >= a->nfe)
+    return fail(F5H_EINVAL, "op_step_seam: bad B / N / nfe / step");
+  if (!step_seam_fits(d, mel))
+    return fail(F5H_EINVAL, "op_step_seam needs d % 64 == 0, 64 <= d <= 1024 and 1 <= mel <= 128");
+  if (a->ada_row % 4 || a->fin_off < 0 || a->fin_off % 4 || a->fin_off + 2 * (int64_t)d > a->ada_row)
+    return fail(F5H_EINVAL, "op_step_seam: ada_row / fin_off must be multiples of 4 with fin_off + 2 d <= ada_row");
+  if (!a->h || !a->table || !a->wp || !a->wx || !a->P || !a->t_grid || !a->y || !a->ypad || !a->h0 || !a->ada_cur)
+    return fail(F5H_EINVAL, "op_step_seam: null tensor");
+  if ((uint64_t)2 * B * N * d * sizeof(float) >= 0xF0000000ull) return fail(F5H_EINVAL, "op_step_seam: too many rows");
+  hipStream_t st = reinterpret_cast<hipStream_t>(stream);
+  const int64_t BN = (int64_t)B * N, rows = 2 * BN;
+  const int dpad = (d + 127) / 128 * 128;
+  OpWs ws(workspace, workspace_bytes);
+  void* hop = ws.take((size_t)rows * d * 2);
+  void* wpop = ws.take((size_t)128 * d * 2);
+  void* wxop = ws.take((size_t)dpad * 128 * 2);
+  void* yop = ws.take((size_t)BN * 128 * 2);
+  float* wx32 = reinterpret_cast<float*>(ws.take((size_t)dpad * 128 * 4));
+  float* bias = reinterpret_cast<float*>(ws.take(128 * 4));
+  int* kstep = reinterpret_cast<int*>(ws.take(64 * 4));
+  float** trajp = reinterpret_cast<float**>(ws.take(64));
+  void* aop = a->fused ? nullptr : ws.take((size_t)rows * d * 2);
+  float* p = a->fused ? nullptr : reinterpret_cast<float*>(ws.take((size_t)rows * 128 * 4));
+  OPWS_CHECK(ws, "op_step_seam");
+  HIPCK(f32_to_op(compute, a->h, rows * d, hop, st));
+  HIPCK(hipMemsetAsync(wpop, 0, (size_t)128 * d * 2, st));
+  HIPCK(f32_to_op(compute, a->wp, (int64_t)mel * d, wpop, st));
+  HIPCK(hipMemsetAsync(wx32, 0, (size_t)dpad * 128 * 4, st));
+  HIPCK(hipMemcpy2DAsync(wx32, 128 * 4, a->wx, (size_t)mel * 4, (size_t)mel * 4, d, hipMemcpyDeviceToDevice, st));
+  HIPCK(f32_to_op(compute, wx32, (int64_t)dpad * 128, wxop, st));
+  HIPCK(f32_to_op(compute, a->ypad, BN * 128, yop, st));
+  if (a->bp) {
+    HIPCK(hipMemsetAsync(bias, 0, 128 * 4, st));
+    HIPCK(hipMemcpyAsync(bias, a->bp, (size_t)mel * 4, hipMemcpyDeviceToDevice, st));
+  }
+  HIPCK(hipMemsetAsync(kstep, 0, 64 * 4, st));
+  HIPCK(seg_upload(&a->step, 1, kstep, st));
+  HIPCK(ptr_upload(a->traj, trajp, st));
+  unsigned* arrive = reinterpret_cast<unsigned*>(kstep + 16);
+  if (a->fused) {
+    SeamArgs s{};
+    s.h = hop;
+    s.B = B;
+    s.N = N;
+    s.d = d;
+    s.mel = mel;
+    s.ada = a->table;
+    s.ada_row = a->ada_row;
+    s.fin_off = a->fin_off;
+    s.wp = wpop;
+    s.bp = a->bp ? bias : nullptr;
+    s.wx = wxop;
+    s.P = a->P;
+    s.h0 = a->h0;
+    s.y = a->y;
+    s.ypad = yop;
+    s.cfg = a->cfg;
+    s.compute = compute;
+    s.kstep = kstep;
+    s.tgrid = a->t_grid;
+    s.trajp = trajp;
+    s.nfe = a->nfe;
+    s.ada_cur = a->ada_cur;
+    s.arrive = arrive;
+    HIPCK(step_seam(s, st));
+  } else {
+    const float* fin = a->table + (int64_t)a->step * a->ada_row + a->fin_off;
+    HIPCK(ln_modulate(compute, hop, 1, (int)rows, d, fin + d, fin, aop, st));
+    GemmArgs g{};
+    g.A = aop;
+    g.lda = d;
+    g.W = wpop;
+    g.ldw = d;
+    g.M = (int)rows;
+    g.N = 128;
+    g.K = d;
+    g.bias = a->bp ? bias : nullptr;
+    g.C = p;
+    g.ldc = 128;
+    HIPCK(gemm(compute, EPI_STORE, g, st));
+    EulerArgs u{};
+    u.y = a->y;
+    u.B = B;
+    u.N = N;
+    u.mel = mel;
+    u.p = p;
+    u.p_seq_stride = (int64_t)N * 128;
+    u.p_row_off = 0;
+    u.p_ld = 128;
+    u.use_cfg = 1;
+    u.cfg = a->cfg;
+    u.ypad = yop;
+    u.compute = compute;
+    u.kstep = kstep;
+    u.tgrid = a->t_grid;
+    u.trajp = trajp;
+    u.next_src = a->table;
+    u.next_stride = a->ada_row;
+    u.next_n = (int)a->ada_row;
+    u.next_dst = a->ada_cur;
+    u.nfe = a->nfe;
+    u.arrive = arrive;
+    HIPCK(cfg_euler(u, st));
+    if (a->step + 1 < a->nfe) {
+      GemmArgs x{};
+      x.A = yop;
+      x.lda = 128;
+      x.W = wxop;
+      x.ldw = 128;
+      x.M = (int)BN;
+      x.N = d;
+      x.K = 128;
+      x.C = a->h0;
+      x.ldc = d;
+      x.add = a->P;
+      x.ld_add = d;
+      x.dual_rows = BN;
+      HIPCK(gemm(compute, EPI_INPROJ, x, st));
+    }
+  }
+  HIPCK(op_to_f32(compute, yop, BN * 128, a->ypad, st));
+  if (a->kstep_out) HIPCK(hipMemcpyAsync(a->kstep_out, kstep, sizeof(int), hipMemcpyDeviceToDevice, st));
+  return 0;
+}
+
 int f5h_op_text_upsample(void* stream, int32_t B, int32_t nt, int32_t N, int32_t td, const int64_t* text,
                          const int32_t* seq_len, const float* in, float* out) {
   if (B <= 0 || nt < 0 || N <= 0 || N > 8192 || td <= 0 || td % 4)
diff --git a/f5-tts_amd/csrc/engine_pack.cpp b/f5-tts_amd/csrc/engine_pack.cpp
--- a/f5-tts_amd/csrc/engine_pack.cpp
+++ b/f5-tts_amd/csrc/engine_pack.cpp
@@ -422,6 +422,7 @@
   if (const char* sv = getenv("F5H_SPLIT_CFG")) e->split_cfg = std::min(2, std::max(0, atoi(sv)));
   if (const char* pv = getenv("F5H_NO_PAD_SKIP")) e->pad_skip = (*pv == '1') ? 0 : 1;
   if (const char* cv = getenv("F5H_CHAIN")) e->chain = (*cv == '1') ? 1 : 0;
+  if (const char* mv = getenv("F5H_SEAM")) e->step_seam = (*mv == '0') ? 0 : (*mv == '1') ? 1 : -1;
   {
     hipEvent_t ev = nullptr;
     if (hipEventCreateWithFlags(&ev, hipEventDisableTiming) == hipSuccess) {
diff --git a/f5-tts_amd/csrc/euler_step.h b/f5-tts_amd/csrc/euler_step.h
--- /dev/null
+++ b/f5-tts_amd/csrc/euler_step.h
@@ -0,0 +1,34 @@
+#pragma once
+#include "common.h"
+
+namespace f5h {
+
+F5H_DEV float cfg_euler_value(float pc, float pu, bool use_cfg, float cfg, float dt, float y0) {
+  float v = pc;
+  if (use_cfg) v = add_nc(pc, mul_nc(sub_nc(pc, pu), cfg));
+  return add_nc(y0, mul_nc(dt, v));
+}
+
+F5H_DEV int step_index(const int* kstep) {
+  return __hip_atomic_load(kstep, __ATOMIC_RELAXED, __HIP_MEMORY_SCOPE_AGENT);
+}
+
+F5H_DEV void step_copy_row(const float* src_row, float* dst, int n, int64_t gtid, int64_t gthreads) {
+  const float4* src = reinterpret_cast<const float4*>(src_row);
+  float4* d4 = reinterpret_cast<float4*>(dst);
+  for (int64_t j = gtid; j < n / 4; j += gthreads) d4[j] = src[j];
+}
+
+F5H_DEV void step_arrive(unsigned* arrive, const int* kstep, int k, int* tick, unsigned nblocks) {
+  __syncthreads();
+  if (threadIdx.x == 0) {
+    const unsigned old = __hip_atomic_fetch_add(arrive, 1u, __ATOMIC_RELAXED, __HIP_MEMORY_SCOPE_AGENT);
+    if (old == nblocks - 1) {
+      __hip_atomic_store(arrive, 0u, __ATOMIC_RELAXED, __HIP_MEMORY_SCOPE_AGENT);
+      __hip_atomic_store(const_cast<int*>(kstep), k + 1, __ATOMIC_RELAXED, __HIP_MEMORY_SCOPE_AGENT);
+      if (tick) __hip_atomic_fetch_add(tick, 1, __ATOMIC_RELAXED, __HIP_MEMORY_SCOPE_AGENT);
+    }
+  }
+}
+
+}
diff --git a/f5-tts_amd/csrc/kernels.h b/f5-tts_amd/csrc/kernels.h
--- a/f5-tts_amd/csrc/kernels.h
+++ b/f5-tts_amd/csrc/kernels.h
@@ -176,6 +176,23 @@
   unsigned* arrive; int* tick;
 };
 hipError_t cfg_euler(const EulerArgs& a, hipStream_t st);
+constexpr int kSeamMaxDim = 1024;
+struct SeamArgs {
+  const void* h;
+  int B, N, d, mel;
+  const float* ada; int64_t ada_row;
+  int64_t fin_off;
+  const void* wp; const float* bp;
+  const void* wx;
+  const float* P; float* h0;
+  float* y; void* ypad;
+  float cfg; int compute;
+  int* kstep; const float* tgrid; float* const* trajp; int nfe;
+  float* ada_cur;
+  unsigned* arrive; int* tick;
+};
+bool step_seam_fits(int d, int mel);
+hipError_t step_seam(const SeamArgs& a, hipStream_t st);
 constexpr int kOdeMethods = 3;
 struct OdeTableau {
   int stages;
diff --git a/f5-tts_amd/csrc/lnrow.h b/f5-tts_amd/csrc/lnrow.h
--- a/f5-tts_amd/csrc/lnrow.h
+++ b/f5-tts_amd/csrc/lnrow.h
@@ -74,6 +74,26 @@
   }
 }
 
+constexpr int kLnMaxV = 8;
+template <typename TO, int NV, typename TI>
+F5H_DEV void ln_mod_row_io(const TI* x, int d, const float* shift, const float* scale, int lane, TO* orow) {
+  constexpr bool FIXED = NV > 0;
+  constexpr int V = FIXED ? NV : kLnMaxV;
+  const float4* sh = reinterpret_cast<const float4*>(shift);
+  const float4* sc = reinterpret_cast<const float4*>(scale);
+  const int n4 = FIXED ? 64 * NV : d >> 2;
+  float4 v[V], a[V], b[V];
+#pragma unroll
+  for (int k = 0; k < V; ++k) {
+    const int i = lane + 64 * k;
+    const bool ok = FIXED || i < n4;
+    v[k] = ok ? load4f<TI>(x + 4 * i) : make_float4(0, 0, 0, 0);
+    a[k] = ok ? sc[i] : make_float4(0, 0, 0, 0);
+    b[k] = ok ? sh[i] : make_float4(0, 0, 0, 0);
+  }
+  ln_mod_row<TO, V, FIXED>(v, a, b, lane, n4, d, orow);
+}
+
 template <typename T>
 F5H_DEV void ln16_row(const uint4 (&x)[2], const float4 (&a)[2][2], const float4 (&b)[2][2], uint4 (&o)[2]) {
   typedef typename Op16<T>::v8 v8;
diff --git a/f5-tts_amd/csrc/seam.hip b/f5-tts_amd/csrc/seam.hip
--- /dev/null
+++ b/f5-tts_amd/csrc/seam.hip
@@ -0,0 +1,244 @@
+#include "common.h"
+#include "euler_step.h"
+#include "lnrow.h"
+
+namespace f5h {
+
+namespace {
+
+constexpr int kSeamThreads = 512;
+constexpr int kSeamSlabs = kSeamMaxDim / 32;
+constexpr int kSeamPass = kSeamMaxDim / 128;
+constexpr int kSeamRing = 16;
+constexpr int kSeamPLd = 132;
+constexpr int kSeamYLd = 256 + 16;
+constexpr uint32_t kSeamPast = 0xF0000000u;
+
+F5H_DEV u32x4 seam_load16(__amdgpu_buffer_rsrc_t r, uint32_t off) {
+  return __builtin_bit_cast(u32x4, __builtin_amdgcn_raw_buffer_load_b128(r, off, 0, 0));
+}
+
+}
+
+template <typename T>
+__global__ __launch_bounds__(kSeamThreads) void step_seam_kernel(SeamArgs a) {
+  typedef typename Op16<T>::v8 v8;
+  __shared__ __attribute__((aligned(16))) unsigned char rows_s[32 * (2 * kSeamMaxDim + 16)];
+  __shared__ __attribute__((aligned(16))) float pt[32 * kSeamPLd];
+  __shared__ __attribute__((aligned(16))) unsigned char yt[16 * kSeamYLd];
+
+  const int tid = threadIdx.x, lane = tid & 63, wid = tid >> 6;
+  const int fr = lane & 15, q = lane >> 4;
+  const int d = a.d, N = a.N, mel = a.mel;
+  const int nblk = (N + 15) >> 4;
+  const int b = blockIdx.x / nblk, n0 = (blockIdx.x - b * nblk) * 16;
+  const int k = __builtin_amdgcn_readfirstlane(step_index(a.kstep));
+  const bool last = k + 1 >= a.nfe;
+  const int nk = d >> 5;
+  const int npass = (d + 127) >> 7;
+  const int live = min(16, N - n0);
+  const int64_t BN = (int64_t)a.B * N;
+  const int64_t base = ((int64_t)b * N + n0) * mel;
+
+  const float dt = sub_nc(a.tgrid[k + 1], a.tgrid[k]);
+  float* traj = a.trajp ? *a.trajp : nullptr;
+  if (traj) traj += (int64_t)(k + 1) * (BN * mel);
+  float yv[4];
+#pragma unroll
+  for (int it = 0; it < 4; ++it) {
+    const int i = tid + it * kSeamThreads;
+    yv[it] = a.y[base + (i < live * mel ? i : 0)];
+  }
+  const int colp = wid * 16 + 4 * q;
+  float4 bias = make_float4(0, 0, 0, 0);
+  if (a.bp) bias = *reinterpret_cast<const float4*>(a.bp + colp);
+
+  if (tid < 16 * kSeamYLd / 16) reinterpret_cast<uint4*>(yt)[tid] = make_uint4(0, 0, 0, 0);
+
+  const __amdgpu_buffer_rsrc_t wprs = rsrc_of(a.wp, (uint64_t)128 * d * 2);
+  const uint32_t wv = (uint32_t)((16 * wid + fr) * d * 2 + q * 16);
+  const __amdgpu_buffer_rsrc_t wxrs = rsrc_of(a.wx, (uint64_t)d * 256);
+  const uint32_t xv0 = (uint32_t)((16 * wid + fr) * 256 + q * 16);
+  auto frag = [&](int i) -> u32x4 {
+    if (i < kSeamSlabs) return seam_load16(wprs, i < nk ? wv + i * 64 : kSeamPast);
+    const int j = i - kSeamSlabs;
+    return seam_load16(wxrs, (!last && (j >> 2) < npass) ? xv0 + (uint32_t)((j >> 2) * 128 * 256 + (j & 3) * 64)
+                                                          : kSeamPast);
+  };
+  u32x4 wf[kSeamRing];
+  auto load_first = [&]() {
+    static_for<0, kSeamRing>([&](auto S) {
+      constexpr int s = decltype(S)::value;
+      wf[s] = frag(s);
+    });
+  };
+
+  const int AST = 2 * d + 16;
+  {
+    const float* fin = a.ada + (int64_t)k * a.ada_row + a.fin_off;
+    const float* scale = fin;
+    const float* shift = fin + d;
+    const T* H = reinterpret_cast<const T*>(a.h);
+    auto grow = [&](int r) { return (int64_t)((r >> 4) * a.B + b) * N + n0 + (r & 15); };
+    if (d == 1024) {
+      const float4* sh = reinterpret_cast<const float4*>(shift);
+      const float4* sc = reinterpret_cast<const float4*>(scale);
+      float4 av[2][2], bv[2][2];
+      uint4 xv[4][2];
+#pragma unroll
+      for (int kk = 0; kk < 2; ++kk) {
+        const int c = lane + 64 * kk;
+        av[kk][0] = sc[2 * c];
+        av[kk][1] = sc[2 * c + 1];
+        bv[kk][0] = sh[2 * c];
+        bv[kk][1] = sh[2 * c + 1];
+      }
+#pragma unroll
+      for (int rr = 0; rr < 4; ++rr) {
+        const int r = wid * 4 + rr;
+        const bool ok = n0 + (r & 15) < N;
+        const uint4* x = reinterpret_cast<const uint4*>(H + (ok ? grow(r) : 0) * 1024);
+#pragma unroll
+        for (int kk = 0; kk < 2; ++kk) xv[rr][kk] = x[lane + 64 * kk];
+      }
+      asm volatile("" ::: "memory");
+      load_first();
+      asm volatile("" ::: "memory");
+#pragma unroll
+      for (int rr = 0; rr < 4; ++rr) {
+        const int r = wid * 4 + rr;
+        const bool ok = n0 + (r & 15) < N;
+        uint4 o[2];
+        ln16_row<T>(xv[rr], av, bv, o);
+        uint4* op = reinterpret_cast<uint4*>(rows_s + r * AST);
+#pragma unroll
+        for (int kk = 0; kk < 2; ++kk) op[lane + 64 * kk] = ok ? o[kk] : make_uint4(0, 0, 0, 0);
+      }
+    } else {
+      load_first();
+      asm volatile("" ::: "memory");
+#pragma unroll 1
+      for (int rr = 0; rr < 4; ++rr) {
+        const int r = wid * 4 + rr;
+        T* orow = reinterpret_cast<T*>(rows_s + r * AST);
+        if (n0 + (r & 15) < N) {
+          const T* x = H + grow(r) * d;
+          switch (d) {
+            case 768: ln_mod_row_io<T, 3, T>(x, d, shift, scale, lane, orow); break;
+            case 512: ln_mod_row_io<T, 2, T>(x, d, shift, scale, lane, orow); break;
+            default: ln_mod_row_io<T, 0, T>(x, d, shift, scale, lane, orow);
+          }
+        } else {
+          for (int i = lane; i < d / 8; i += 64) reinterpret_cast<uint4*>(orow)[i] = make_uint4(0, 0, 0, 0);
+        }
+      }
+    }
+  }
+
+  __syncthreads();
+
+  {
+    const unsigned char* a0 = rows_s + fr * AST + q * 16;
+    const unsigned char* a1 = a0 + 16 * AST;
+    f32x4 acc[2] = {f32x4{0.f, 0.f, 0.f, 0.f}, f32x4{0.f, 0.f, 0.f, 0.f}};
+    static_for<0, kSeamSlabs>([&](auto S) {
+      constexpr int s = decltype(S)::value, slot = s % kSeamRing;
+      if (s < nk) {
+        const v8 w = __builtin_bit_cast(v8, wf[slot]);
+        const v8 r0 = *reinterpret_cast<const v8*>(a0 + s * 64);
+        const v8 r1 = *reinterpret_cast<const v8*>(a1 + s * 64);
+        acc[0] = Op16<T>::mma16(w, r0, acc[0]);
+        acc[1] = Op16<T>::mma16(w, r1, acc[1]);
+      }
+      wf[slot] = frag(s + kSeamRing);
+    });
+#pragma unroll
+    for (int mt = 0; mt < 2; ++mt) {
+      f32x4 x = acc[mt];
+      if (a.bp) x = f32x4{add_nc(x[0], bias.x), add_nc(x[1], bias.y), add_nc(x[2], bias.z), add_nc(x[3], bias.w)};
+      *reinterpret_cast<f32x4*>(pt + (16 * mt + fr) * kSeamPLd + colp) = x;
+    }
+  }
+  __syncthreads();
+
+  {
+#pragma unroll
+    for (int it = 0; it < 4; ++it) {
+      const int i = tid + it * kSeamThreads;
+      if (i < live * mel) {
+        const int nl = i / mel, c = i - nl * mel;
+        const float y = cfg_euler_value(pt[nl * kSeamPLd + c], pt[(16 + nl) * kSeamPLd + c], true, a.cfg, dt, yv[it]);
+        a.y[base + i] = y;
+        reinterpret_cast<T*>(yt + nl * kSeamYLd)[c] = from_f32<T>(y);
+        if (traj) traj[base + i] = y;
+      }
+    }
+    __syncthreads();
+    if (tid < live * 16) {
+      const int nl = tid >> 4, ch = tid & 15;
+      const uint4 v = *reinterpret_cast<const uint4*>(yt + nl * kSeamYLd + ch * 16);
+      reinterpret_cast<uint4*>(reinterpret_cast<T*>(a.ypad) + ((int64_t)b * N + n0 + nl) * 128)[ch] = v;
+    }
+  }
+
+  if (!last) {
+    v8 af[4];
+#pragma unroll
+    for (int ks = 0; ks < 4; ++ks) af[ks] = *reinterpret_cast<const v8*>(yt + fr * kSeamYLd + q * 16 + ks * 64);
+    const bool rok = n0 + fr < N;
+    const int64_t rowc = (int64_t)b * N + n0 + fr;
+    const __amdgpu_buffer_rsrc_t prs = rsrc_of(a.P, (uint64_t)2 * BN * d * sizeof(float));
+    f32x4 acc[kSeamPass];
+    u32x4 pcv[kSeamPass], puv[kSeamPass];
+    static_for<0, kSeamPass>([&](auto TT) {
+      constexpr int t = decltype(TT)::value;
+      acc[t] = f32x4{0.f, 0.f, 0.f, 0.f};
+      if (t < npass) {
+#pragma unroll
+        for (int ks = 0; ks < 4; ++ks)
+          acc[t] = Op16<T>::mma16(__builtin_bit_cast(v8, wf[(4 * t + ks) % kSeamRing]), af[ks], acc[t]);
+      }
+      if constexpr (4 * t + kSeamRing < kSeamSlabs) {
+#pragma unroll
+        for (int ks = 0; ks < 4; ++ks) wf[(4 * t + ks) % kSeamRing] = frag(kSeamSlabs + 4 * t + ks + kSeamRing);
+      }
+      const int col = t * 128 + colp;
+      const bool ok = rok && col < d;
+      const uint32_t o = (uint32_t)((rowc * d + col) * sizeof(float));
+      pcv[t] = seam_load16(prs, ok ? o : kSeamPast);
+      puv[t] = seam_load16(prs, ok ? o + (uint32_t)(BN * d * sizeof(float)) : kSeamPast);
+    });
+    static_for<0, kSeamPass>([&](auto TT) {
+      constexpr int t = decltype(TT)::value;
+      const int col = t * 128 + colp;
+      if (rok && col < d) {
+        const f32x4 pc = __builtin_bit_cast(f32x4, pcv[t]), pu = __builtin_bit_cast(f32x4, puv[t]);
+        float* o = a.h0 + rowc * d + col;
+        *reinterpret_cast<float4*>(o) =
+            make_float4(acc[t][0] + pc[0], acc[t][1] + pc[1], acc[t][2] + pc[2], acc[t][3] + pc[3]);
+        *reinterpret_cast<float4*>(o + BN * d) =
+            make_float4(acc[t][0] + pu[0], acc[t][1] + pu[1], acc[t][2] + pu[2], acc[t][3] + pu[3]);
+      }
+    });
+  }
+
+  if (a.ada_cur && !last)
+    step_copy_row(a.ada + (int64_t)(k + 1) * a.ada_row, a.ada_cur, (int)a.ada_row,
+                  (int64_t)blockIdx.x * kSeamThreads + tid, (int64_t)gridDim.x * kSeamThreads);
+  if (a.arrive) step_arrive(a.arrive, a.kstep, k, a.tick, gridDim.x);
+}
+
+bool step_seam_fits(int d, int mel) { return d >= 64 && d % 64 == 0 && d <= kSeamMaxDim && mel >= 1 && mel <= 128; }
+
+hipError_t step_seam(const SeamArgs& a, hipStream_t st) {
+  if (!step_seam_fits(a.d, a.mel) || a.B <= 0 || a.N <= 0 || (a.ada_row & 3) || !a.kstep) return hipErrorInvalidValue;
+  if (a.compute != F5H_C_BF16 && a.compute != F5H_C_FP16) return hipErrorInvalidValue;
+  const unsigned blocks = (unsigned)a.B * (unsigned)((a.N + 15) / 16);
+  if (a.compute == F5H_C_BF16)
+    hipLaunchKernelGGL(step_seam_kernel<bf16>, dim3(blocks), dim3(kSeamThreads), 0, st, a);
+  else
+    hipLaunchKernelGGL(step_seam_kernel<f16>, dim3(blocks), dim3(kSeamThreads), 0, st, a);
+  return hipGetLastError();
+}
+
+}
diff --git a/f5-tts_amd/f5_tts_amd/_lib.py b/f5-tts_amd/f5_tts_amd/_lib.py
--- a/f5-tts_amd/f5_tts_amd/_lib.py
+++ b/f5-tts_amd/f5_tts_amd/_lib.py
@@ -47,6 +47,9 @@
     "f5h_set_store_policy",
     "f5h_store_policy_stats",
     "f5h_store_policy_force",
+    "f5h_set_step_seam",
+    "f5h_step_seam_stats",
+    "f5h_op_step_seam",
     "f5h_op_linear",
     "f5h_op_attention",
     "f5h_op_attention_qlen",
@@ -151,6 +154,20 @@
         ("q_norm_w", ctypes.c_void_p), ("k_norm_w", ctypes.c_void_p), ("qk_norm_eps", ctypes.c_float),
         ("qkv_dst_len", ctypes.c_int32),
         ("seg_off", ctypes.c_void_p), ("n_seq", ctypes.c_int32),
+    ]
+
+
+class OpSeamArgs(ctypes.Structure):
+    _fields_ = [
+        ("compute", ctypes.c_int32), ("fused", ctypes.c_int32),
+        ("B", ctypes.c_int32), ("N", ctypes.c_int32), ("d", ctypes.c_int32), ("mel", ctypes.c_int32),
+        ("nfe", ctypes.c_int32), ("step", ctypes.c_int32),
+        ("ada_row", ctypes.c_int64), ("fin_off", ctypes.c_int64),
+        ("cfg", ctypes.c_float),
+        ("h", ctypes.c_void_p), ("table", ctypes.c_void_p), ("wp", ctypes.c_void_p), ("bp", ctypes.c_void_p),
+        ("wx", ctypes.c_void_p), ("P", ctypes.c_void_p), ("t_grid", ctypes.c_void_p),
+        ("y", ctypes.c_void_p), ("ypad", ctypes.c_void_p), ("h0", ctypes.c_void_p), ("traj", ctypes.c_void_p),
+        ("ada_cur", ctypes.c_void_p), ("kstep_out", ctypes.c_void_p),
     ]
 
 
@@ -284,6 +301,13 @@
         L.f5h_store_policy_stats.restype = ctypes.c_int
         L.f5h_store_policy_force.argtypes = [i32]
         L.f5h_store_policy_force.restype = ctypes.c_int
+    if hasattr(L, "f5h_set_step_seam"):
+        L.f5h_set_step_seam.argtypes = [vp, i32]
+        L.f5h_set_step_seam.restype = ctypes.c_int
+        L.f5h_step_seam_stats.argtypes = [vp, ctypes.POINTER(i32), ctypes.POINTER(i64)]
+        L.f5h_step_seam_stats.restype = ctypes.c_int
+        L.f5h_op_step_seam.argtypes = [vp, ctypes.POINTER(OpSeamArgs), vp, sz]
+        L.f5h_op_step_seam.restype = ctypes.c_int
     if hasattr(L, "f5h_chain_debug_spin_limit"):
         L.f5h_chain_debug_spin_limit.argtypes = [i64]
         L.f5h_chain_debug_spin_limit.restype = ctypes.c_int
@@ -352,6 +376,10 @@
     return hasattr(lib(), "f5h_op_attention_ranges")
 
 
+def has_step_seam() -> bool:
+    return hasattr(lib(), "f5h_set_step_seam")
+
+
 def has_ragged() -> bool:
     return hasattr(lib(), "f5h_vocos_decode_ragged")
 
diff --git a/f5-tts_amd/f5_tts_amd/engine.py b/f5-tts_amd/f5_tts_amd/engine.py
--- a/f5-tts_amd/f5_tts_amd/engine.py
+++ b/f5-tts_amd/f5_tts_amd/engine.py
@@ -204,6 +204,14 @@
     def ln_fold_stats(self):
         sup, n = ctypes.c_int32(), ctypes.c_int64()
         _lib.check(_lib.lib().f5h_ln_fold_stats(self._h, ctypes.byref(sup), ctypes.byref(n)), "ln_fold_stats")
+        return bool(sup.value), int(n.value)
+
+    def set_step_seam(self, mode: int):
+        _lib.check(_lib.lib().f5h_set_step_seam(self._h, int(mode)), "set_step_seam")
+
+    def step_seam_stats(self):
+        sup, n = ctypes.c_int32(), ctypes.c_int64()
+        _lib.check(_lib.lib().f5h_step_seam_stats(self._h, ctypes.byref(sup), ctypes.byref(n)), "step_seam_stats")
         return bool(sup.value), int(n.value)
 
     STORE_CLASS_BITS = {"qkv": 1, "attn": 2, "out": 4, "ffn1": 8, "ffn2": 16}
@@ -549,6 +557,31 @@
                                       int(bool(h16)), M, d, h.data_ptr(), p0.data_ptr(), _lib.ptr(p1),
                                       out.data_ptr(), ws.data_ptr(), ws.numel()), "f5h_op_norm")
     return out
+
+
+def op_step_seam(h, table, fin_off, wp, bp, wx, P, t_grid, y, ypad, h0, traj, ada_cur, step, cfg, B, fused=True,
+                 compute="bf16"):
+    if not _lib.has_step_seam():
+        raise RuntimeError("the loaded libf5h.so has no f5h_op_step_seam (an older build)")
+    dev = h.device
+    rows, d = h.shape
+    BN, mel = y.shape
+    nfe, ada_row = table.shape
+    for t in (h, table, wp, wx, P, t_grid, y, ypad, h0, ada_cur) + tuple(x for x in (bp, traj) if x is not None):
+        assert t.is_contiguous() and t.dtype == torch.float32 and t.device == dev
+    assert rows == 2 * BN and BN % B == 0 and ypad.shape == (BN, 128) and h0.shape == (rows, d)
+    kout = torch.full((1,), -1, dtype=torch.int32, device=dev)
+    a = _lib.OpSeamArgs(compute=_lib.COMPUTE[compute], fused=int(bool(fused)), B=B, N=BN // B, d=d, mel=mel, nfe=nfe,
+                        step=int(step), ada_row=ada_row, fin_off=int(fin_off), cfg=float(cfg), h=h.data_ptr(),
+                        table=table.data_ptr(), wp=wp.data_ptr(), bp=_lib.ptr(bp), wx=wx.data_ptr(), P=P.data_ptr(),
+                        t_grid=t_grid.data_ptr(), y=y.data_ptr(), ypad=ypad.data_ptr(), h0=h0.data_ptr(),
+                        traj=_lib.ptr(traj), ada_cur=ada_cur.data_ptr(), kstep_out=kout.data_ptr())
+    dpad = (d + 127) // 128 * 128
+    need = rows * d * 4 + 128 * d * 2 + dpad * 128 * 6 + BN * 128 * 2 + rows * 128 * 4 + 16 * 256 + 4096
+    ws = torch.empty(need, dtype=torch.uint8, device=dev)
+    _lib.check(_lib.lib().f5h_op_step_seam(_lib.stream_handle(dev), ctypes.byref(a), ws.data_ptr(), ws.numel()),
+               "f5h_op_step_seam")
+    return kout
 
 
 def op_dwconv_ln(x, dw_w, dw_b, ln_w, ln_b, compute="bf16", seq_len=None):
diff --git a/include/f5h.h b/include/f5h.h
--- a/include/f5h.h
+++ b/include/f5h.h
@@ -143,6 +143,8 @@
 int f5h_set_ln_fold(f5h_engine* eng, int32_t enable);
 int f5h_ln_fold_stats(f5h_engine* eng, int32_t* supported, int64_t* passes);
 int f5h_set_store_policy(f5h_engine* eng, int32_t mode);
+int f5h_set_step_seam(f5h_engine* eng, int32_t mode);
+int f5h_step_seam_stats(f5h_engine* eng, int32_t* supported, int64_t* launches);
 int f5h_store_policy_stats(f5h_engine* eng, int64_t* write_through, int64_t* plain);
 int f5h_store_policy_force(int32_t mode);
 int f5h_chain_stats(f5h_engine* eng, int64_t* launches, int32_t* fault, int64_t* refused);
@@ -170,6 +172,26 @@
 int f5h_op_conv_pos(void* stream, int32_t compute, int32_t S, int32_t L, int32_t d, const float* x, const float* w,
                     const float* bias, const uint8_t* rowkeep, int32_t mode, const float* resid, int32_t x_as_f32,
                     int64_t y_seq_stride, int64_t y_row_off, float* y, void* workspace, size_t workspace_bytes);
+typedef struct f5h_op_seam_args {
+  int32_t compute, fused;
+  int32_t B, N, d, mel, nfe, step;
+  int64_t ada_row, fin_off;
+  float cfg;
+  const float* h;
+  const float* table;
+  const float* wp;
+  const float* bp;
+  const float* wx;
+  const float* P;
+  const float* t_grid;
+  float* y;
+  float* ypad;
+  float* h0;
+  float* traj;
+  float* ada_cur;
+  int32_t* kstep_out;
+} f5h_op_seam_args;
+int f5h_op_step_seam(void* stream, const f5h_op_seam_args* a, void* workspace, size_t workspace_bytes);
 int f5h_op_norm(void* stream, int32_t compute, int32_t kind, int32_t h16, int32_t M, int32_t d, const float* h,
                 const float* shift_or_g, const float* scale, float* out, void* workspace, size_t workspace_bytes);
 int f5h_op_dwconv_ln(void* stream, int32_t compute, int32_t S, int32_t L, int32_t C, const float* x,
```
